# hyperplane-lab/RGBManip

Measured on AMD Instinct MI355X. Metric: adapose_poses_per_sec_batch256, higher is better.
Workload: dtype bf16

## Files before the change

### include/rgbm.h

```cpp
#ifndef RGBM_H_
#define RGBM_H_
#include <stddef.h>
#include <stdint.h>

#ifdef __cplusplus
extern "C" {
#endif

#define RGBM_VERSION 100
#define RGBM_F32 0
#define RGBM_BF16 1
#define RGBM_F16 2
#define RGBM_BF16X3 3

int rgbm_version(void);
const char* rgbm_last_error(void);

typedef struct rgbm_weight_desc {
  const char* name;
  const float* data;
  int ndim;
  const int64_t* shape;
} rgbm_weight_desc;

typedef struct rgbm_adapose rgbm_adapose_t;

typedef struct rgbm_adapose_out {
  float *view1_nocs, *view2_nocs;
  float *view1_depth, *view2_depth;
  float *view1_r, *view2_r;
  float *view1_t, *view2_t;
  float *view1_s, *view2_s;
} rgbm_adapose_out;

int rgbm_adapose_create(rgbm_adapose_t** h, int device, const rgbm_weight_desc* w, int n_w, int dtype, int norm_mode);
int rgbm_adapose_destroy(rgbm_adapose_t* h);
int rgbm_adapose_set_chunk(rgbm_adapose_t* h, int max_chunk_views);
int rgbm_adapose_set_option(rgbm_adapose_t* h, const char* key, int value);
int rgbm_adapose_workspace_bytes(rgbm_adapose_t* h, int B, size_t* bytes);
int rgbm_adapose_set_dropout(rgbm_adapose_t* h, float p, uint64_t seed);
int rgbm_adapose_dropout_masks(rgbm_adapose_t* h, int B, float* out_dev);
int rgbm_adapose_set_dropout_masks(rgbm_adapose_t* h, int B, const float* masks_dev);
int rgbm_adapose_forward(rgbm_adapose_t* h, int B, const float* img1, const float* img2, const int32_t* choose1,
                         const int32_t* choose2, const float* P1, const float* P2, const float* depths, void* workspace,
                         size_t workspace_bytes, const rgbm_adapose_out* out, void* stream);

int rgbm_adapose_postprocess(int B, int P, int img_size, const float* nocs1, const float* depth1, const float* r1,
                             const int32_t* choose1, const double* Kcrop, const double* E1, double* bbox_world, double* ts,
                             int32_t* valid, void* stream);
int rgbm_adapose_postprocess_scratch_bytes(int B, size_t* bytes);
int rgbm_adapose_postprocess_ws(int B, int P, int img_size, const float* nocs1, const float* depth1, const float* r1,
                                const int32_t* choose1, const double* Kcrop, const double* E1, double* bbox_world, double* ts,
                                int32_t* valid, void* scratch, size_t scratch_bytes, void* stream);

int rgbm_adapose_postprocess_ransac(int B, int P, int img_size, uint32_t seed, const float* nocs1, const float* depth1,
                                    const int32_t* choose1, const double* Kcrop, const double* E1, double* bbox_world, double* srt,
                                    int32_t* valid, void* stream);
int rgbm_adapose_postprocess_pnp(int B, int P, uint32_t seed, const float* nocs1, const float* pts2d1, const float* nocs2,
                                 const float* pts2d2, const double* K, const double* E1, const double* E2, double* bbox_out,
                                 double* srt_out, int32_t* info_out, int32_t* valid_out, void* stream);

int rgbm_prepare_inputs(const float* rgb_dev, const uint8_t* mask_dev, const double* K_dev, int N, int H, int W, int S, int P,
                        uint32_t seed, float* img_out, int32_t* choose_out, float* pts2d_out, double* Kcrop_out,
                        int32_t* window_out, int32_t* valid_out, uint8_t* scratch, void* stream);

int rgbm_prepare_inputs_indexed(const float* rgb_dev, const uint8_t* mask_dev, const double* K_dev, const int32_t* frame_map_dev,
                                int N, int H, int W, int S, int P, uint32_t seed, float* img_out, int32_t* choose_out,
                                float* pts2d_out, double* Kcrop_out, int32_t* window_out, int32_t* valid_out, uint8_t* scratch,
                                void* stream);
int rgbm_prepare_inputs_ex(const float* rgb_dev, const uint8_t* mask_dev, const double* K_dev, const int32_t* frame_map_dev,
                           int frame0, int N, int H, int W, int S, int P, uint32_t seed, float* img_out, int32_t* choose_out,
                           float* pts2d_out, double* Kcrop_out, int32_t* window_out, int32_t* valid_out, uint8_t* scratch,
                           void* stream);

int rgbm_projection(const double* Kcrop_dev, const double* E_dev, float* P_dev, int N, void* stream);
int rgbm_mask_extent(const uint8_t* mask_dev, int N, int H, int W, int32_t* ext_out, int32_t* count_out, void* stream);

int rgbm_lookat_quat(const double* dir_dev, int N, int batch_zero, double* quat_dev, void* stream);
int rgbm_control_action_to_pose(const float* action_dev, int lda, const double* pose_mid, const double* pose_min,
                                const double* pose_max, int N, double* pose_dev, void* stream);
typedef struct rgbm_control_reward_args {
  const float* action;
  const double* cam_pose;
  const double* target;
  const float* move_success;
  const double* bbox;
  const double* avail;
  const double* gt_bbox;
  const double* pred_bbox;
  const double* pose_cur;
  const double* pose_prev;
  const double* robot_pose;
  const double* success;
  double* reward;
  double* terms;
  double coef[14];
  double proper_pos[3];
  double precision2;
  int N, T, lda, pots, first;
  int pad_;
} rgbm_control_reward_args;
int rgbm_control_reward(const rgbm_control_reward_args* args, void* stream);
int rgbm_control_grasp_frame(const double* est_dev, int N, double* center_dev, double* direction_dev, void* stream);

typedef struct rgbm_synth_scene {
  const double* cam_pose;
  const double* robot_pose;
  const double* box;
  double fx, fy, cx, cy;
  int N, H, W, env0;
} rgbm_synth_scene;
int rgbm_synth_camera(const rgbm_synth_scene* scene, double* K_dev, double* E_dev, double* rays_dev, void* stream);
int rgbm_synth_render(const rgbm_synth_scene* scene, const double* rays_dev, float* color_dev, uint8_t* mask_dev, void* stream);

int rgbm_gae(int T, int N, const float* rewards, const uint8_t* dones, const float* values, const float* last_values,
             float gamma, float lam, float* returns, float* adv, double* sums, void* stream);
int rgbm_adv_normalise(int64_t n_local, float* adv, const double* sums, double count_total, void* stream);

typedef struct rgbm_policy_layout {
  int dims[5];
  int log_std;
  int w[2][4];
  int b[2][4];
  int total;
} rgbm_policy_layout;
int rgbm_policy_forward(const float* params, const rgbm_policy_layout* L, int n, int mode, const float* obs, const float* noise,
                        float* actions, float* logp, float* value, float* mu, void* stream);
int rgbm_ppo_partial_floats(const rgbm_policy_layout* L, int n, size_t* count);
int rgbm_ppo_minibatch_fwd_bwd(const float* params, const rgbm_policy_layout* L, int n, const float* obs, const float* actions,
                               const float* old_logp, const float* adv, const float* returns, const float* old_values,
                               const float* old_mu, const float* old_log_std, float clip, float vcoef, float ecoef,
                               float* partial_scratch, float* grads_flat, void* stream);
int rgbm_ppo_clip_adam(float* params, const float* grads_flat, float* exp_avg, float* exp_avg_sq, void* opt_state,
                       const rgbm_policy_layout* L, float inv_world, float max_norm, float desired_kl, float lr_min,
                       float lr_max, int adaptive, void* stream);

int rgbm_conv_nd(int dtype, const void* in_dev, int N, int D, int H, int W, int Cin, int Cin_pad, const float* w_host,
                 int Cout, int Cout_pad, int KD, int KH, int KW, int stride_d, int stride_hw, int pad_d, int pad_hw,
                 int dil_hw, int transposed, const float* bias_host, const float* bn_scale_host, const float* bn_shift_host,
                 const void* res_dev, int res_mode, int act, float slope, void* out_dev, void* stream);
int rgbm_bn_per_sample_scratch_bytes(int V, size_t* bytes);
int rgbm_bn_per_sample(int dtype, void* y_dev, const void* res_dev, const float* gamma_dev, const float* beta_dev, void* scratch_dev,
                       int V, int64_t nvox, int C, int relu, void* stream);
int rgbm_conv3d_tile(int layer, int dtype, const void* in_dev, int N, int D, int H, int W, const float* w_host,
                     const float* bn_scale_host, const float* bn_shift_host, const void* res_dev, void* out_dev, void* stream);
int rgbm_upsample_conv3x3(int dtype, const void* in_dev, int V, int h, int w, int Cin, const float* w_host, int Cout,
                          const float* bias_host, int act, float slope, void* z_scratch_dev, void* out_dev, void* stream);
int rgbm_upsample_conv3x3_final(int dtype, const void* in_dev, int V, int h, int w, const float* w3_host, const float* b3_host,
                                float slope, const float* wf_host, const float* bf_host, void* out_dev, int out_f32, void* stream);
int rgbm_stem(int dtype, const float* img1_dev, const float* img2_dev, const float* w_host, void* out_dev, int B, int S, void* stream);
int rgbm_maxpool3x3s2(int dtype, const void* in_dev, void* out_dev, int V, int H, int W, int C, void* stream);
int rgbm_resize_bilinear_ac(int dtype, const void* in_dev, void* out_dev, int V, int Hs, int Ws, int C, int Ho, int Wo,
                            void* stream);
int rgbm_adaptive_avgpool(int dtype, const void* in_dev, void* out_dev, int V, int H, int W, int C, int S, void* stream);
int rgbm_build_volume(int dtype, const void* feat_dev, const float* P_views_dev, const float* depths_dev, float* homog_scratch,
                      void* vol_dev, int V, int B, int D, int H, int W, void* stream);
int rgbm_conv0_sweep(const void* feat_dev, const float* P_views_dev, const float* depths_dev, float* homog_scratch,
                     const float* w_host, const float* bn_scale_host, const float* bn_shift_host, void* out_dev,
                     int V, int B, int D, int H, int W, void* stream);
int rgbm_conv0_sweep_dt(int dtype, const void* feat_dev, const float* P_views_dev, const float* depths_dev, float* homog_scratch,
                        const float* w_host, const float* bn_scale_host, const float* bn_shift_host, void* out_dev,
                        int V, int B, int D, int H, int W, void* stream);
int rgbm_conv0_sweep_f16feat(const void* feat_f16_dev, const float* P_views_dev, const float* depths_dev, float* homog_scratch,
                             const float* w_host, const float* bn_scale_host, const float* bn_shift_host, void* out_bf16_dev,
                             int V, int B, int D, int H, int W, void* stream);
int rgbm_adapose_forward_ex(rgbm_adapose_t* h, int B, const float* img1, const float* img2, const int32_t* choose1,
                            const int32_t* choose2, const float* P1, const float* P2, const float* depths, void* workspace,
                            size_t workspace_bytes, const rgbm_adapose_out* out, int stop_after, void* stream);
int rgbm_adapose_forward_graph(rgbm_adapose_t* h, int B, const float* img1, const float* img2, const int32_t* choose1,
                               const int32_t* choose2, const float* P1, const float* P2, const float* depths, void* workspace,
                               size_t workspace_bytes, const rgbm_adapose_out* out, void* stream, int32_t* n_nodes, int32_t* captured);
int rgbm_adapose_graph_clear(rgbm_adapose_t* h);
int rgbm_adapose_fetch(rgbm_adapose_t* h, int B, void* workspace, const char* name, float* out_dev, size_t capacity,
                       size_t* n_elems, void* stream);

#define RGBM_PROF_ROWS 42
int rgbm_debug_flags(int flags);
int rgbm_set_tuning(const char* key, long long value);
int rgbm_microbench_mfma_scratch_floats(int* n);
int rgbm_microbench_mfma(float* scratch, int iters, int random_operands, double* flops, void* stream);
int rgbm_microbench_copy(const void* src, void* dst, size_t bytes, void* stream);
int rgbm_prof_rows(void);
int rgbm_prof_start(void);
int rgbm_prof_stop(double* stats);
int rgbm_prof_select(int row);

#ifdef __cplusplus
}
#endif
#endif
```

### rgbmanip_amd/_lib.py

```python
from __future__ import annotations

import ctypes as C
import os

_HERE = os.path.dirname(os.path.abspath(__file__))
LIB_PATH = os.environ.get("RGBM_HIP_LIB") or os.path.join(_HERE, "librgbm_hip.so")

F32, BF16, F16, BF16X3 = 0, 1, 2, 3
ACT_NONE, ACT_RELU, ACT_PRELU, ACT_TANH = 0, 1, 2, 3
RES_NONE, RES_PRE_ACT, RES_POST_ACT = 0, 1, 2


PROF_ROWS = 42
PROF_KERNELS = [
    ("conv_igemm_glds_kernel<float, 16, 256>", "fp32"), ("conv_igemm_glds_kernel<float, 32, 256>", "fp32"),
    ("conv_igemm_glds_kernel<float, 64, 256>", "fp32"), ("conv_igemm_glds_kernel<float, 128, 128>", "fp32"),
    ("conv_igemm_glds_kernel<unsigned short, 16, 256>", "bf16"), ("conv_igemm_glds_kernel<unsigned short, 32, 256>", "bf16"),
    ("conv_igemm_glds_kernel<unsigned short, 64, 256>", "bf16"), ("conv_igemm_glds_kernel<unsigned short, 128, 128>", "bf16"),
    ("conv3d_tile_kernel<float, ...> (conv1..conv11)", "fp32"), ("conv3d_tile_kernel<unsigned short, ...> (conv1..conv11)", "bf16"),
    ("conv3d_tile_kernel<float, 32, 16, 4, 8, 8, 1, false, true> (conv0 + fused plane sweep)", "fp32"),
    ("conv3d_tile_kernel<unsigned short, 32, 16, 4, 8, 8, 1, false, true> (conv0 + fused plane sweep)", "bf16"),
    ("conv_igemm_ws_kernel<float, ...>", "fp32"), ("conv_igemm_ws_kernel<unsigned short, false, false> (128 channels x 256 pixels)", "bf16"),
    ("conv0_sweep_persistent_kernel<unsigned short> (conv0 + fused plane sweep of bf16 nets; sweep_f16 = 0 / fp16 nets: conv0_sweep_kernel)", "bf16"), ("conv_igemm_ws64_kernel", "bf16"),
    ("conv3d_tile_kernel<unsigned short, 32, 16, 6, 8, 8, 1, false, false> (conv0 on a materialised volume)", "bf16"),
    ("conv3d_tile_kernel<unsigned short, 8, 16, 2, 8, 8, 2, false, false> (conv1)", "bf16"),
    ("conv3d_tile_kernel<unsigned short, 16, 16, 4, 8, 8, 1, false, false> (conv2)", "bf16"),
    ("conv3d_tile_kernel<unsigned short, 16, 32, 2, 8, 8, 2, false, false> (conv3)", "bf16"),
    ("conv3d_tile_kernel<unsigned short, 32, 32, 2, 8, 8, 1, false, false> (conv4)", "bf16"),
    ("conv3d_tile_kernel<unsigned short, 32, 64, 1, 8, 8, 2, false, false> (conv5)", "bf16"),
    ("conv3d_tile_kernel<unsigned short, 64, 64, 1, 8, 8, 1, false, false> (conv6)", "bf16"),
    ("conv3d_tile_kernel<unsigned short, 64, 32, 1, 8, 8, 1, true, false> (conv7)", "bf16"),
    ("conv3d_tile_kernel<unsigned short, 32, 16, 2, 8, 8, 1, true, false> (conv9)", "bf16"),
    ("conv3d_tile_kernel<unsigned short, 16, 16, 4, 8, 8, 1, true, false> (conv11)", "bf16"),
] + [("conv_igemm_glds_kernel<bx3_t, ...> (all channel tiles)", "bf16x3"), ("conv3d_tile_kernel<bx3_t, ...> (conv1..conv11)", "bf16x3"),
     ("conv0 + fused plane sweep <bx3_t>", "bf16x3"), ("conv_igemm_ws_kernel<rgbm::bx3_t, false, false> (128 channels x 256 pixels)", "bf16x3"),
     ("unused (conv_igemm_w256_kernel of rounds 2-5)", "bf16"),
     ("conv_igemm_m32_kernel<unsigned short, 256, 256> (256 channels x 256 pixels, 32x32x16 MFMAs; gemm_kernel = 0: conv_igemm_ws_kernel<unsigned short, true, false>, 256 x 128)", "bf16"),
     ("unused (row-halo ws tile of rounds 2-5)", "bf16"),
     ("conv_igemm_m32_kernel<rgbm::bx3_t, 256, 256> (256 channels x 256 pixels, 32x32x16 MFMAs; gemm_kernel = 0: conv_igemm_ws_kernel<rgbm::bx3_t, true, false>, 256 x 128)", "bf16x3"),
     ("conv_igemm_ws_kernel<rgbm::bx3_t, false, false, true> (64 channels x 256 pixels, four multiply waves)", "bf16x3"),
     ("conv_igemm_ws_kernel<unsigned short, false, false, true> (64 channels x 256 pixels, four multiply waves)", "bf16"),
     ("conv_igemm_ws_kernel<float, false, false, true> (64 channels x 256 pixels, four multiply waves)", "fp32"),
     ("upconv_combine_kernel<16-bit> (PSPUpsample tap combination)", "bf16"), ("upconv_combine_kernel<4-byte> (PSPUpsample tap combination)", "bf16x3"),
     ("upconv_final_kernel (up_3 + final in one kernel; either storage width)", "bf16"),
     ("conv_igemm_m32_kernel<unsigned short, 128, 64 / 128 / 256> (128-pixel tiles: tail and small-batch launches of the 256-channel GEMM)", "bf16"),
     ("conv_igemm_m32_kernel<rgbm::bx3_t, 128, 64 / 128 / 256> (128-pixel tiles: tail and small-batch launches of the 256-channel GEMM)", "bf16x3")]
assert len(PROF_KERNELS) == PROF_ROWS


class RgbmError(RuntimeError):
    pass


class WeightDesc(C.Structure):
    _fields_ = [("name", C.c_char_p), ("data", C.c_void_p), ("ndim", C.c_int), ("shape", C.POINTER(C.c_int64))]


class PolicyLayout(C.Structure):
    _fields_ = [("dims", C.c_int * 5), ("log_std", C.c_int), ("w", (C.c_int * 4) * 2), ("b", (C.c_int * 4) * 2), ("total", C.c_int)]


class AdaposeOut(C.Structure):
    _fields_ = [(n, C.c_void_p) for n in ("view1_nocs", "view2_nocs", "view1_depth", "view2_depth", "view1_r", "view2_r",
                                           "view1_t", "view2_t", "view1_s", "view2_s")]


class ControlRewardArgs(C.Structure):
    _fields_ = [(n, C.c_void_p) for n in ("action", "cam_pose", "target", "move_success", "bbox", "avail", "gt_bbox", "pred_bbox",
                                           "pose_cur", "pose_prev", "robot_pose", "success", "reward", "terms")] + [
        ("coef", C.c_double * 14), ("proper_pos", C.c_double * 3), ("precision2", C.c_double),
        ("N", C.c_int), ("T", C.c_int), ("lda", C.c_int), ("pots", C.c_int), ("first", C.c_int), ("pad_", C.c_int)]


class SynthScene(C.Structure):
    _fields_ = [("cam_pose", C.c_void_p), ("robot_pose", C.c_void_p), ("box", C.c_void_p),
                ("fx", C.c_double), ("fy", C.c_double), ("cx", C.c_double), ("cy", C.c_double),
                ("N", C.c_int), ("H", C.c_int), ("W", C.c_int), ("env0", C.c_int)]


_vp, _i, _f, _d, _sz, _i64 = C.c_void_p, C.c_int, C.c_float, C.c_double, C.c_size_t, C.c_int64

SIGNATURES = {
    "rgbm_version": (_i, []),
    "rgbm_last_error": (C.c_char_p, []),
    "rgbm_adapose_create": (_i, [C.POINTER(_vp), _i, C.POINTER(WeightDesc), _i, _i, _i]),
    "rgbm_adapose_destroy": (_i, [_vp]),
    "rgbm_adapose_set_chunk": (_i, [_vp, _i]),
    "rgbm_adapose_set_option": (_i, [_vp, C.c_char_p, _i]),
    "rgbm_adapose_workspace_bytes": (_i, [_vp, _i, C.POINTER(_sz)]),
    "rgbm_adapose_set_dropout": (_i, [_vp, _f, C.c_uint64]),
    "rgbm_adapose_dropout_masks": (_i, [_vp, _i, _vp]),
    "rgbm_adapose_set_dropout_masks": (_i, [_vp, _i, _vp]),
    "rgbm_adapose_forward": (_i, [_vp, _i, _vp, _vp, _vp, _vp, _vp, _vp, _vp, _vp, _sz, C.POINTER(AdaposeOut), _vp]),
    "rgbm_adapose_forward_ex": (_i, [_vp, _i, _vp, _vp, _vp, _vp, _vp, _vp, _vp, _vp, _sz, C.POINTER(AdaposeOut), _i, _vp]),
    "rgbm_adapose_forward_graph": (_i, [_vp, _i, _vp, _vp, _vp, _vp, _vp, _vp, _vp, _vp, _sz, C.POINTER(AdaposeOut), _vp, C.POINTER(C.c_int32),
                                        C.POINTER(C.c_int32)]),
    "rgbm_adapose_graph_clear": (_i, [_vp]),
    "rgbm_adapose_fetch": (_i, [_vp, _i, _vp, C.c_char_p, _vp, _sz, C.POINTER(_sz), _vp]),
    "rgbm_adapose_postprocess": (_i, [_i, _i, _i, _vp, _vp, _vp, _vp, _vp, _vp, _vp, _vp, _vp, _vp]),
    "rgbm_adapose_postprocess_scratch_bytes": (_i, [_i, C.POINTER(_sz)]),
    "rgbm_adapose_postprocess_ws": (_i, [_i, _i, _i, _vp, _vp, _vp, _vp, _vp, _vp, _vp, _vp, _vp, _vp, _sz, _vp]),
    "rgbm_adapose_postprocess_ransac": (_i, [_i, _i, _i, C.c_uint32, _vp, _vp, _vp, _vp, _vp, _vp, _vp, _vp, _vp]),
    "rgbm_adapose_postprocess_pnp": (_i, [_i, _i, C.c_uint32, _vp, _vp, _vp, _vp, _vp, _vp, _vp, _vp, _vp, _vp, _vp, _vp]),
    "rgbm_gae": (_i, [_i, _i, _vp, _vp, _vp, _vp, _f, _f, _vp, _vp, _vp, _vp]),
    "rgbm_adv_normalise": (_i, [_i64, _vp, _vp, _d, _vp]),
    "rgbm_policy_forward": (_i, [_vp, _vp, _i, _i, _vp, _vp, _vp, _vp, _vp, _vp, _vp]),
    "rgbm_ppo_partial_floats": (_i, [_vp, _i, C.POINTER(_sz)]),
    "rgbm_ppo_minibatch_fwd_bwd": (_i, [_vp, _vp, _i, _vp, _vp, _vp, _vp, _vp, _vp, _vp, _vp, _f, _f, _f, _vp, _vp, _vp]),
    "rgbm_ppo_clip_adam": (_i, [_vp, _vp, _vp, _vp, _vp, _vp, _f, _f, _f, _f, _f, _i, _vp]),
    "rgbm_conv_nd": (_i, [_i, _vp, _i, _i, _i, _i, _i, _i, _vp, _i, _i, _i, _i, _i, _i, _i, _i, _i, _i, _i, _vp, _vp, _vp,
                          _vp, _i, _i, _f, _vp, _vp]),
    "rgbm_bn_per_sample_scratch_bytes": (_i, [_i, C.POINTER(_sz)]),
    "rgbm_bn_per_sample": (_i, [_i, _vp, _vp, _vp, _vp, _vp, _i, _i64, _i, _i, _vp]),
    "rgbm_conv3d_tile": (_i, [_i, _i, _vp, _i, _i, _i, _i, _vp, _vp, _vp, _vp, _vp, _vp]),
    "rgbm_upsample_conv3x3": (_i, [_i, _vp, _i, _i, _i, _i, _vp, _i, _vp, _i, _f, _vp, _vp, _vp]),
    "rgbm_upsample_conv3x3_final": (_i, [_i, _vp, _i, _i, _i, _vp, _vp, _f, _vp, _vp, _vp, _i, _vp]),
    "rgbm_stem": (_i, [_i, _vp, _vp, _vp, _vp, _i, _i, _vp]),
    "rgbm_maxpool3x3s2": (_i, [_i, _vp, _vp, _i, _i, _i, _i, _vp]),
    "rgbm_resize_bilinear_ac": (_i, [_i, _vp, _vp, _i, _i, _i, _i, _i, _i, _vp]),
    "rgbm_adaptive_avgpool": (_i, [_i, _vp, _vp, _i, _i, _i, _i, _i, _vp]),
    "rgbm_build_volume": (_i, [_i, _vp, _vp, _vp, _vp, _vp, _i, _i, _i, _i, _i, _vp]),
    "rgbm_conv0_sweep": (_i, [_vp, _vp, _vp, _vp, _vp, _vp, _vp, _vp, _i, _i, _i, _i, _i, _vp]),
    "rgbm_conv0_sweep_dt": (_i, [_i, _vp, _vp, _vp, _vp, _vp, _vp, _vp, _vp, _i, _i, _i, _i, _i, _vp]),
    "rgbm_conv0_sweep_f16feat": (_i, [_vp, _vp, _vp, _vp, _vp, _vp, _vp, _vp, _i, _i, _i, _i, _i, _vp]),
    "rgbm_prepare_inputs": (_i, [_vp, _vp, _vp, _i, _i, _i, _i, _i, C.c_uint32, _vp, _vp, _vp, _vp, _vp, _vp, _vp, _vp]),
    "rgbm_prepare_inputs_indexed": (_i, [_vp, _vp, _vp, _vp, _i, _i, _i, _i, _i, C.c_uint32, _vp, _vp, _vp, _vp, _vp, _vp, _vp, _vp]),
    "rgbm_prepare_inputs_ex": (_i, [_vp, _vp, _vp, _vp, _i, _i, _i, _i, _i, _i, C.c_uint32, _vp, _vp, _vp, _vp, _vp, _vp, _vp, _vp]),
    "rgbm_projection": (_i, [_vp, _vp, _vp, _i, _vp]),
    "rgbm_mask_extent": (_i, [_vp, _i, _i, _i, _vp, _vp, _vp]),
    "rgbm_lookat_quat": (_i, [_vp, _i, _i, _vp, _vp]),
    "rgbm_control_action_to_pose": (_i, [_vp, _i, C.POINTER(C.c_double), C.POINTER(C.c_double), C.POINTER(C.c_double), _i, _vp, _vp]),
    "rgbm_control_reward": (_i, [C.POINTER(ControlRewardArgs), _vp]),
    "rgbm_control_grasp_frame": (_i, [_vp, _i, _vp, _vp, _vp]),
    "rgbm_synth_camera": (_i, [C.POINTER(SynthScene), _vp, _vp, _vp, _vp]),
    "rgbm_synth_render": (_i, [C.POINTER(SynthScene), _vp, _vp, _vp, _vp]),
    "rgbm_debug_flags": (_i, [_i]),
    "rgbm_set_tuning": (_i, [C.c_char_p, _i64]),
    "rgbm_prof_rows": (_i, []),
    "rgbm_microbench_mfma_scratch_floats": (_i, [C.POINTER(C.c_int)]),
    "rgbm_microbench_mfma": (_i, [_vp, _i, _i, C.POINTER(C.c_double), _vp]),
    "rgbm_microbench_copy": (_i, [_vp, _vp, C.c_size_t, _vp]),
    "rgbm_prof_start": (_i, []),
    "rgbm_prof_select": (_i, [_i]),
    "rgbm_prof_stop": (_i, [C.POINTER(C.c_double)]),
}

_lib = None


def load():
    global _lib
    if _lib is not None:
        return _lib
    if not os.path.exists(LIB_PATH):
        raise RgbmError(f"{LIB_PATH} not found: build it with rgbmanip_amd/csrc/build.sh "
                        f"(or `python -c 'import __graft_entry__ as g; g.build()'`). There is no CPU fallback.")
    lib = C.CDLL(LIB_PATH)
    for name, (res, args) in SIGNATURES.items():
        fn = getattr(lib, name)
        fn.restype = res
        fn.argtypes = args
    if lib.rgbm_prof_rows() != PROF_ROWS:
        raise RgbmError(f"{LIB_PATH}: rgbm_prof_rows() = {lib.rgbm_prof_rows()}, this binding expects {PROF_ROWS} (stale build?)")
    _lib = lib
    return lib


def check(rc: int, what: str = ""):
    if rc != 0:
        msg = load().rgbm_last_error()
        raise RgbmError(f"{what} failed (code {rc}): {msg.decode() if msg else ''}")


def stream_ptr(stream=None):
    import torch
    s = stream if stream is not None else torch.cuda.current_stream()
    return C.c_void_p(s.cuda_stream)


def ptr(t):
    return C.c_void_p(t.data_ptr()) if t is not None else C.c_void_p(0)
```

### rgbmanip_amd/csrc/adapose.cpp

```cpp
#include "adapose.h"

#include <math.h>
#include <string.h>

namespace rgbm {

static const int kLayerPlanes[4] = {64, 128, 256, 512};
static const int kLayerBlocks[4] = {3, 4, 6, 3};
static const int kLayerStride[4] = {1, 2, 1, 1};
static const int kLayerDil[4] = {1, 1, 2, 4};
static const int kPspBins[4] = {1, 2, 3, 6};
static const int kPspSmallViews = 32;


static const HostTensor* find(const StateDict& sd, const std::string& name) {
  auto it = sd.find(name);
  return it == sd.end() ? nullptr : &it->second;
}

#define GET(var, name)                                               \
  const HostTensor* var = find(sd, name);                            \
  RGBM_REQUIRE(var != nullptr, std::string("missing weight ") + (name))

static int init_conv2d(ConvLayer& L, int dtype, const StateDict& sd, const std::string& wname, const char* bname, int Cin,
                       int Cout, int k, int stride, int pad, int dil, int act, float slope, int Cin_pad) {
  GET(w, wname);
  RGBM_REQUIRE(w->numel() == (long long)Cout * Cin * k * k, "weight shape " + wname);
  const float* b = nullptr;
  if (bname) { GET(bt, std::string(bname)); b = bt->data; }
  ConvGeom g;
  g.Cin = Cin; g.Cout = Cout; g.KH = g.KW = k; g.sh = g.sw = stride; g.ph = g.pw = pad; g.dilh = g.dilw = dil;
  g.act = act; g.slope = slope;
  return L.init(dtype, g, w->data, b, nullptr, nullptr, Cin_pad, Cout);
}

static int bn_fold(const StateDict& sd, const std::string& p, int C, std::vector<float>& scale, std::vector<float>& shift) {
  GET(gm, p + "weight"); GET(bt, p + "bias"); GET(mu, p + "running_mean"); GET(var, p + "running_var");
  RGBM_REQUIRE(gm->numel() == C && bt->numel() == C && mu->numel() == C && var->numel() == C, "bn shape " + p);
  scale.resize(C); shift.resize(C);
  for (int i = 0; i < C; ++i) {
    const float inv = 1.0f / sqrtf(var->data[i] + 1e-5f);
    scale[i] = gm->data[i] * inv;
    shift[i] = bt->data[i] - mu->data[i] * scale[i];
  }
  return 0;
}

static int init_conv3d_bn(ConvLayer& L, int dtype, const StateDict& sd, const std::string& p, int Cin, int Cout, int stride,
                          bool transposed) {
  GET(w, p + "conv.weight");
  RGBM_REQUIRE(w->numel() == (long long)Cout * Cin * 27, "weight shape " + p);
  std::vector<float> scale, shift;
  if (int rc = bn_fold(sd, p + "bn.", Cout, scale, shift)) return rc;
  ConvGeom g;
  g.Cin = Cin; g.Cout = Cout; g.KD = g.KH = g.KW = 3; g.sd = g.sh = g.sw = stride; g.pd = g.ph = g.pw = 1;
  g.transposed = transposed; g.act = ACT_RELU;
  return L.init(dtype, g, w->data, nullptr, scale.data(), shift.data(), Cin, Cout);
}

static int init_linear(ConvLayer& L, const StateDict& sd, const std::string& p, int Cin, int Cout, int act, int Cin_pad,
                       int Cout_pad, const float* w_override = nullptr, int ldtype = F32) {
  GET(w, p + ".weight"); GET(b, p + ".bias");
  ConvGeom g;
  g.Cin = Cin; g.Cout = Cout; g.act = act;
  return L.init(ldtype, g, w_override ? w_override : w->data, b->data, nullptr, nullptr, Cin_pad, Cout_pad);
}

int AdaPose::create(const StateDict& sd, int dtype_, int norm_mode_) {
  dtype = dtype_;
  norm_mode = norm_mode_;
  const int E = dtype_chunk(dtype);
  img_cpad = E;
  const std::string fe = "img_extractor.feats.";
  if (int rc = init_conv2d(conv1, dtype, sd, fe + "conv1.weight", nullptr, 3, 64, 7, 2, 3, 1, ACT_RELU, 0.f, img_cpad)) return rc;
  if (dtype != F32) {
    GET(w1, fe + "conv1.weight");
    RGBM_REQUIRE(w1->numel() == 64 * 3 * 7 * 7, "conv1 shape");
    std::vector<float> pk;
    stem_pack(w1->data, pk);
    if (int rc = upload_packed(pk, dtype, &stem_w)) return rc;
    stem = 1;
  }
  int inpl = 64, nb = 0;
  for (int li = 0; li < 4; ++li) {
    for (int b = 0; b < kLayerBlocks[li]; ++b) {
      Block& blk = blocks[nb++];
      const int planes = kLayerPlanes[li];
      const int cin = b == 0 ? inpl : planes;
      const int stride = b == 0 ? kLayerStride[li] : 1;
      const int dil = b == 0 ? 1 : kLayerDil[li];
      const std::string p = fe + "layer" + std::to_string(li + 1) + "." + std::to_string(b) + ".";
      if (int rc = init_conv2d(blk.c1, dtype, sd, p + "conv1.weight", nullptr, cin, planes, 3, stride, dil, dil, ACT_RELU, 0.f, cin)) return rc;
      if (int rc = init_conv2d(blk.c2, dtype, sd, p + "conv2.weight", nullptr, planes, planes, 3, 1, dil, dil, ACT_RELU, 0.f, planes)) return rc;
      blk.has_ds = find(sd, p + "downsample.0.weight") != nullptr;
      if (blk.has_ds)
        if (int rc = init_conv2d(blk.ds, dtype, sd, p + "downsample.0.weight", nullptr, cin, planes, 1, stride, 0, 1, ACT_NONE, 0.f, cin)) return rc;
      blk.stride = stride; blk.planes = planes;
    }
    inpl = kLayerPlanes[li];
  }
  n_blocks = nb;
  for (int i = 0; i < 4; ++i)
    if (int rc = init_conv2d(psp[i], dtype, sd, "img_extractor.psp.stages." + std::to_string(i) + ".1.weight", nullptr, 512, 128, 1, 1, 0, 1, ACT_RELU, 0.f, 512)) return rc;
  struct { ConvLayer* L; const char* nm; int cin, cout; } ups[3] = {{&up1, "up_1", 1024, 256}, {&up2, "up_2", 256, 64}, {&up3, "up_3", 64, 64}};
  for (auto& u : ups) {
    const std::string p = std::string("img_extractor.") + u.nm + ".conv.";
    GET(sl, p + "1.weight");
    const std::string bn = p + "0.bias";
    if (int rc = init_conv2d(*u.L, dtype, sd, p + "0.weight", bn.c_str(), u.cin, u.cout, 3, 1, 1, 1, ACT_PRELU, sl->data[0], u.cin)) return rc;
    UpConvLayer* uc = u.L == &up1 ? &up1c : u.L == &up2 ? &up2c : nullptr;
    if (uc) {
      GET(w, p + "0.weight"); GET(b, bn);
      if (int rc = uc->init(dtype, u.cin, u.cout, w->data, b->data, ACT_PRELU, sl->data[0])) return rc;
    }
  }
  if (int rc = init_conv2d(fin, dtype, sd, "img_extractor.final.weight", "img_extractor.final.bias", 64, 32, 1, 1, 0, 1, ACT_NONE, 0.f, 64)) return rc;
  if (dtype != F32) {
    GET(w3, "img_extractor.up_3.conv.0.weight"); GET(b3, "img_extractor.up_3.conv.0.bias"); GET(s3, "img_extractor.up_3.conv.1.weight");
    GET(wf, "img_extractor.final.weight"); GET(bfin, "img_extractor.final.bias");
    if (int rc = tail.init(dtype, w3->data, b3->data, s3->data[0], wf->data, bfin->data)) return rc;
  }


  const std::string cr = "cost_regularization.";
  const int crc[8] = {32, 8, 16, 16, 32, 32, 64, 64};
  const int crs[7] = {1, 2, 1, 2, 1, 2, 1};
  for (int i = 0; i < 7; ++i)
    if (int rc = init_conv3d_bn(c3d[i], dtype, sd, cr + "conv" + std::to_string(i) + ".", crc[i], crc[i + 1], crs[i], false)) return rc;
  if (int rc = init_conv3d_bn(dc[0], dtype, sd, cr + "conv7.", 64, 32, 2, true)) return rc;
  if (int rc = init_conv3d_bn(dc[1], dtype, sd, cr + "conv9.", 32, 16, 2, true)) return rc;
  if (int rc = init_conv3d_bn(dc[2], dtype, sd, cr + "conv11.", 16, 8, 2, true)) return rc;
  if (norm_mode == 1) {
    const char* nm[10] = {"conv0", "conv1", "conv2", "conv3", "conv4", "conv5", "conv6", "conv7", "conv9", "conv11"};
    for (int i = 0; i < 10; ++i) {
      const bool tr = i >= 7;
      const int cin = tr ? (i == 7 ? 64 : i == 8 ? 32 : 16) : crc[i], cout = tr ? cin / 2 : crc[i + 1];
      const std::string p = cr + nm[i] + ".";
      GET(w, p + "conv.weight"); GET(gm, p + "bn.weight"); GET(bt, p + "bn.bias");
      RGBM_REQUIRE(w->numel() == (long long)cout * cin * 27 && gm->numel() == cout && bt->numel() == cout, "weight shape " + p);
      ConvGeom g;
      g.Cin = cin; g.Cout = cout; g.KD = g.KH = g.KW = 3; g.sd = g.sh = g.sw = tr ? 2 : crs[i]; g.pd = g.ph = g.pw = 1;
      g.transposed = tr; g.act = ACT_NONE;
      ConvLayer& L = tr ? dc_raw[i - 7] : c3d_raw[i];
      if (int rc = L.init(dtype, g, w->data, nullptr, nullptr, nullptr, cin, cout)) return rc;
      if (upload_f32(gm->data, cout, &bn_gamma[i])) return -2;
      if (upload_f32(bt->data, cout, &bn_beta[i])) return -2;
    }
  }
  {
    const char* nm[10] = {"conv0", "conv1", "conv2", "conv3", "conv4", "conv5", "conv6", "conv7", "conv9", "conv11"};
    const int cin[10] = {32, 8, 16, 16, 32, 32, 64, 64, 32, 16};
    const int cout[10] = {8, 16, 16, 32, 32, 64, 64, 32, 16, 8};
    for (int i = 0; i < 10; ++i) {
      const std::string p = cr + nm[i] + ".";
      GET(w, p + "conv.weight");
      std::vector<float> scale, shift, packed;
      if (int rc = bn_fold(sd, p + "bn.", cout[i], scale, shift)) return rc;
      const int coutp = cout[i] < 16 ? 16 : cout[i];
      conv3d_tile_pack(w->data, scale.data(), cin[i], cout[i], coutp, i >= 7, dtype, packed);
      t3d[i].Cin = cin[i]; t3d[i].Cout = cout[i];
      if (upload_packed(packed, dtype, &t3d[i].w)) return -2;
      std::vector<float> bpad(coutp, 0.f);
      for (int o = 0; o < cout[i]; ++o) bpad[o] = shift[o];
      if (upload_f32(bpad.data(), bpad.size(), &t3d[i].bias)) return -2;
      if (i == 9 && dtype != F32) {
        std::vector<float> pt;
        prob_sparse_pack(w->data, scale.data(), pt);
        if (dtype == BF16X3) { if (conv0_sweep_x3_upload(pt, &w11_taps)) return -2; }
        else if (upload_packed(pt, dtype, &w11_taps)) return -2;
      }
      if (i == 9 && dtype == BF16X3) {
        std::vector<float> p16;
        conv3d_tile_pack(w->data, scale.data(), cin[i], cout[i], coutp, true, BF16, p16);
        if (conv0_sweep_x3_upload(p16, &w11_x3)) return -2;
      }
      if (i == 0 && dtype != F32) {
        conv0_sweep_pack(w->data, scale.data(), packed);
        if (dtype == BF16X3) { if (conv0_sweep_x3_upload(packed, &sweep_w)) return -2; }
        else if (upload_packed(packed, dtype, &sweep_w)) return -2;
        if (dtype == BF16 && weights_fit_f16(packed) && upload_packed(packed, F16, &sweep_w_f16)) return -2;
      }
    }
  }
  {
    GET(w, cr + "prob.weight");
    RGBM_REQUIRE(w->numel() == 8 * 27, "prob weight shape");
    std::vector<float> wp(27 * 8);
    for (int c = 0; c < 8; ++c) for (int t = 0; t < 27; ++t) wp[t * 8 + c] = w->data[c * 27 + t];
    if (upload_f32(wp.data(), wp.size(), &wprob)) return -2;
  }
  if (int rc = init_linear(inst, sd, "instance_color.0", 32, 64, ACT_RELU, 32, 64)) return rc;
  if (int rc = init_linear(nh[0], sd, "nocs_head.0", 64, 128, ACT_RELU, 64, 128)) return rc;
  if (int rc = init_linear(nh[1], sd, "nocs_head.2", 128, 64, ACT_RELU, 128, 64)) return rc;
  if (int rc = init_linear(nh[2], sd, "nocs_head.4", 64, 3, ACT_TANH, 64, 4)) return rc;
  if (int rc = init_linear(npm[0], sd, "nocs_pts_mlp.0", 3, 32, ACT_RELU, 4, 32)) return rc;
  if (int rc = init_linear(npm[1], sd, "nocs_pts_mlp.2", 32, 64, ACT_RELU, 32, 64)) return rc;
  {
    static const char* const names[6] = {"instance_color.0", "nocs_head.0", "nocs_head.2", "nocs_head.4", "nocs_pts_mlp.0", "nocs_pts_mlp.2"};
    static const int cin[6] = {32, 64, 128, 64, 3, 32}, cout[6] = {64, 128, 64, 3, 32, 64};
    const float* w[6]; const float* b[6];
    for (int l = 0; l < 6; ++l) {
      GET(wt, std::string(names[l]) + ".weight"); GET(bt, std::string(names[l]) + ".bias");
      RGBM_REQUIRE(wt->numel() == (long long)cin[l] * cout[l] && bt->numel() == cout[l], std::string("point MLP shape ") + names[l]);
      w[l] = wt->data; b[l] = bt->data;
    }
    std::vector<float> table((size_t)point_mlp_table_floats());
    point_mlp_pack(w, b, table.data());
    if (upload_f32(table.data(), table.size(), &pmlp_table)) return -2;
  }
  if (int rc = init_linear(pm1[0], sd, "pose_mlp1.0", 96, 128, ACT_RELU, 96, 128, nullptr, pose_dtype())) return rc;
  if (int rc = init_linear(pm1[1], sd, "pose_mlp1.2", 128, 128, ACT_RELU, 128, 128, nullptr, pose_dtype())) return rc;
  {
    GET(w, "pose_mlp2.0.weight"); GET(b, "pose_mlp2.0.bias");
    RGBM_REQUIRE(w->numel() == 256 * 256, "pose_mlp2.0 shape");
    std::vector<float> wl(256 * 128);
    for (int o = 0; o < 256; ++o) for (int i = 0; i < 128; ++i) wl[o * 128 + i] = w->data[o * 256 + i];
    if (int rc = init_linear(pm2[0], sd, "pose_mlp2.0", 128, 256, ACT_RELU, 128, 256, wl.data(), pose_dtype())) return rc;
    if (upload_f32(w->data, 256 * 256, &pm2_0_wfull)) return -2;
    if (upload_f32(b->data, 256, &pm2_0_bias)) return -2;
  }
  if (int rc = init_linear(pm2[1], sd, "pose_mlp2.2", 256, 256, ACT_RELU, 256, 256, nullptr, pose_dtype())) return rc;
  const char* hn[3] = {"rotation_estimator", "translation_estimator", "size_estimator"};
  const int hout[3] = {6, 3, 3};
  for (int h = 0; h < 3; ++h) {
    const int dims[4] = {256, 256, 128, hout[h]};
    for (int l = 0; l < 3; ++l) {
      GET(w, std::string(hn[h]) + "." + std::to_string(2 * l) + ".weight");
      GET(b, std::string(hn[h]) + "." + std::to_string(2 * l) + ".bias");
      RGBM_REQUIRE(w->numel() == (long long)dims[l] * dims[l + 1], "head weight shape");
      if (upload_f32(w->data, w->numel(), &head_w[h][l])) return -2;
      if (upload_f32(b->data, b->numel(), &head_b[h][l])) return -2;
    }
  }
  return 0;
}

void AdaPose::destroy() {
  conv1.destroy();
  if (stem_w) (void)hipFree(stem_w);
  stem_w = nullptr;
  for (int i = 0; i < n_blocks; ++i) { blocks[i].c1.destroy(); blocks[i].c2.destroy(); if (blocks[i].has_ds) blocks[i].ds.destroy(); }
  for (auto& l : psp) l.destroy();
  up1.destroy(); up2.destroy(); up3.destroy(); fin.destroy();
  up1c.destroy(); up2c.destroy(); tail.destroy();
  if (drop_masks) (void)hipFree(drop_masks);
  if (drop_state) (void)hipFree(drop_state);
  drop_masks = nullptr; drop_state = nullptr; drop_cap_views = 0; drop_p = 0.f; drop_explicit = 0; drop_last_B = 0;
  for (auto& l : c3d) l.destroy();
  for (auto& l : dc) l.destroy();
  for (auto& l : c3d_raw) l.destroy();
  for (auto& l : dc_raw) l.destroy();
  for (int i = 0; i < 10; ++i) { if (bn_gamma[i]) (void)hipFree(bn_gamma[i]); if (bn_beta[i]) (void)hipFree(bn_beta[i]); bn_gamma[i] = bn_beta[i] = nullptr; }
  inst.destroy();
  for (auto& l : nh) l.destroy();
  for (auto& l : npm) l.destroy();
  for (auto& l : pm1) l.destroy();
  for (auto& l : pm2) l.destroy();
  for (auto& t : t3d) { if (t.w) (void)hipFree(t.w); if (t.bias) (void)hipFree(t.bias); t.w = nullptr; t.bias = nullptr; }
  if (sweep_w) (void)hipFree(sweep_w);
  sweep_w = nullptr;
  if (sweep_w_f16) (void)hipFree(sweep_w_f16);
  sweep_w_f16 = nullptr;
  if (w11_x3) (void)hipFree(w11_x3);
  w11_x3 = nullptr;
  if (w11_taps) (void)hipFree(w11_taps);
  w11_taps = nullptr;
  if (wprob) (void)hipFree(wprob);
  if (pm2_0_wfull) (void)hipFree(pm2_0_wfull);
  if (pmlp_table) { (void)hipFree(pmlp_table); pmlp_table = nullptr; }
  if (pm2_0_bias) (void)hipFree(pm2_0_bias);
  for (int h = 0; h < 3; ++h) for (int l = 0; l < 3; ++l) { if (head_w[h][l]) (void)hipFree(head_w[h][l]); if (head_b[h][l]) (void)hipFree(head_b[h][l]); }
}

bool AdaPose::feat_f32_only() const {
  return dtype == BF16X3 && cost_impl == 3 && sweep_w != nullptr && norm_mode == 0 && !(g_debug_flags & 4096);
}

bool AdaPose::feat_f16() const {
  return dtype == BF16 && sweep_f16 != 0 && cost_impl == 3 && sweep_w_f16 != nullptr && norm_mode == 0 && !(g_debug_flags & 4096) && (upconv & 4) &&
         tail.ready() && tail.f16_ready();
}

bool AdaPose::sparse_active() const {
  const bool b16 = dtype_size(dtype) == 2;
  return sparse_dec != 0 && norm_mode == 0 && cost_impl == 3 && (b16 || (dtype == BF16X3 && w11_x3)) && sparse_tail && sweep_w != nullptr &&
         !(g_debug_flags & 4096);
}

int AdaPose::chunk_views(int V) const {
  const int cap = norm_mode == 1 && max_chunk > 32 ? 32 : max_chunk;
  return V < cap ? V : cap;
}

int AdaPose::plan(int B, Arena& A, Buffers& bf) const {
  const int V = 2 * B, P = n_pts, S = img;
  const size_t es = dtype_size(dtype);
  const size_t VP = (size_t)V * P;
  bf.Pviews = (float*)A.alloc((size_t)V * 16 * 4);
  bf.homog = (float*)A.alloc((size_t)V * 12 * 4);
  bf.choose = (int*)A.alloc(VP * 4);
  bf.masks = (unsigned char*)A.alloc((size_t)V * sparse_mask_bytes_per_view(img));
  bf.sweep_list = (int*)A.alloc((size_t)V * ((img + 11) / 12) * ((img + 15) / 16) * 4);
  bf.sweep_count = (int*)A.alloc((size_t)(V + 64) * 4);
  bf.feat = A.alloc((size_t)V * S * S * 32 * es);
  bf.featf = dtype == BF16X3 ? (float*)A.alloc((size_t)V * S * S * 32 * 4) : nullptr;
  bf.X0 = (float*)A.alloc(VP * 32 * 4);
  bf.X1 = (float*)A.alloc(VP * 64 * 4);
  bf.H128 = (float*)A.alloc(VP * 128 * 4);
  bf.H64 = (float*)A.alloc(VP * 64 * 4);
  bf.nocs4 = (float*)A.alloc(VP * 4 * 4);
  bf.N32 = (float*)A.alloc(VP * 32 * 4);
  bf.PF96 = (float*)A.alloc(VP * 96 * 4);
  bf.PF96h = pose_dtype() == F16 ? A.alloc(VP * 96 * 2) : nullptr;
  bf.prob = (float*)A.alloc(VP * n_depth * 4);
  bf.depth = (float*)A.alloc(VP * 4);
  bf.Q128a = (float*)A.alloc(VP * 128 * 4);
  bf.Q128b = (float*)A.alloc(VP * 128 * 4);
  bf.G256a = (float*)A.alloc(VP * 256 * 4);
  bf.G256b = (float*)A.alloc(VP * 256 * 4);
  bf.glob = (float*)A.alloc((size_t)V * 128 * 4);
  bf.vbias = (float*)A.alloc((size_t)V * 256 * 4);
  bf.pf2 = (float*)A.alloc((size_t)V * 256 * 4);
  bf.h1 = (float*)A.alloc((size_t)V * 256 * 4);
  bf.h2 = (float*)A.alloc((size_t)V * 128 * 4);
  bf.r6 = (float*)A.alloc((size_t)V * 8 * 4);
  bf.R = (float*)A.alloc((size_t)V * 9 * 4);
  bf.tv = (float*)A.alloc((size_t)V * 4 * 4);
  bf.sv = (float*)A.alloc((size_t)V * 4 * 4);
  const size_t m0 = A.mark();
  bf.imgpad = A.alloc((size_t)V * S * S * img_cpad * es);
  bf.c1 = A.alloc((size_t)V * (S / 2) * (S / 2) * 64 * es);
  const size_t lbuf = (size_t)V * ((size_t)(S / 4) * (S / 4) * 64 > (size_t)(S / 8) * (S / 8) * 512 ? (size_t)(S / 4) * (S / 4) * 64 : (size_t)(S / 8) * (S / 8) * 512) * es;
  for (int i = 0; i < 4; ++i) bf.lb[i] = A.alloc(lbuf);
  for (int i = 0; i < 4; ++i) {
    bf.pooled[i] = A.alloc((size_t)V * kPspBins[i] * kPspBins[i] * 512 * es);
    bf.stage[i] = A.alloc((size_t)V * kPspBins[i] * kPspBins[i] * 128 * es);
  }
  const size_t f8 = (size_t)(S / 8) * (S / 8), f4 = (size_t)(S / 4) * (S / 4), f2 = (size_t)(S / 2) * (S / 2), f1 = (size_t)S * S;
  bf.cat = A.alloc((size_t)V * f8 * 1024 * es);
  bf.ups = A.alloc((size_t)V * f4 * 1024 * es);
  bf.u1 = A.alloc((size_t)V * f4 * 256 * es);
  bf.u2 = A.alloc((size_t)V * f2 * 64 * es);
  bf.u3 = A.alloc((size_t)V * f1 * 64 * es);
  A.release(m0);
  const int Vc = chunk_views(V);
  const int D = n_depth;
  const size_t vox = (size_t)D * S * S;
  bf.vol = (cost_impl >= 2 && norm_mode == 0) ? nullptr : A.alloc((size_t)Vc * vox * 32 * es);
  bf.bn_scratch = norm_mode == 1 ? A.alloc(bn_scratch_bytes(Vc)) : nullptr;
  bf.c[0] = A.alloc((size_t)Vc * vox * 8 * es);
  bf.c[1] = A.alloc((size_t)Vc * (vox / 8) * 16 * es);
  bf.c[2] = A.alloc((size_t)Vc * (vox / 8) * 16 * es);
  bf.c[3] = A.alloc((size_t)Vc * (vox / 64) * 32 * es);
  bf.c[4] = A.alloc((size_t)Vc * (vox / 64) * 32 * es);
  bf.c[5] = A.alloc((size_t)Vc * (vox / 512) * 64 * es);
  bf.c[6] = A.alloc((size_t)Vc * (vox / 512) * 64 * es);
  bf.u7 = A.alloc((size_t)Vc * (vox / 64) * 32 * es);
  bf.u9 = A.alloc((size_t)Vc * (vox / 8) * 16 * es);
  bf.u11 = A.alloc((size_t)Vc * vox * 8 * es);
  A.release(m0);
  return 0;
}

size_t AdaPose::workspace_bytes(int B) const {
  Arena A(nullptr, 0);
  Buffers bf;
  plan(B, A, bf);
  return A.peak + 256;
}

int AdaPose::pspnet(const Buffers& bf, int V, const float* img1, const float* img2, hipStream_t s, const float* drop) const {
  const int S = img;
  int H = S / 2, W = S / 2;
  if (stem && stem_w) {
    if (int rc = launch_stem(dtype, img1, img2, stem_w, bf.lb[0], V / 2, V, S, s)) return rc;
  } else {
    const size_t es = dtype_size(dtype);
    const int B = V / 2;
    if (int rc = launch_nchw_to_nhwc_pad(dtype, img1, bf.imgpad, B, 3, S, S, img_cpad, s)) return rc;
    if (int rc = launch_nchw_to_nhwc_pad(dtype, img2, (char*)bf.imgpad + (size_t)B * S * S * img_cpad * es, B, 3, S, S, img_cpad, s)) return rc;
    if (int rc = conv1.run(bf.imgpad, bf.c1, V, 1, S, S, 64, nullptr, 0, nullptr, 0, s)) return rc;
    if (int rc = launch_maxpool3x3s2(dtype, bf.c1, bf.lb[0], V, H, W, 64, s)) return rc;
  }
  H = S / 4; W = S / 4;
  int xi = 0;
  for (int i = 0; i < n_blocks; ++i) {
    const Block& blk = blocks[i];
    void* x = bf.lb[xi];
    void* t = bf.lb[(xi + 1) & 3];
    void* r = bf.lb[(xi + 2) & 3];
    void* y = bf.lb[(xi + 3) & 3];
    int Do, Ho, Wo;
    blk.c1.out_dims(1, H, W, Do, Ho, Wo);
    if (int rc = blk.c1.run(x, t, V, 1, H, W, blk.planes, nullptr, 0, nullptr, 0, s)) return rc;
    const void* res = x;
    if (blk.has_ds) {
      if (int rc = blk.ds.run(x, r, V, 1, H, W, blk.planes, nullptr, 0, nullptr, 0, s)) return rc;
      res = r;
    }
    if (int rc = blk.c2.run(t, y, V, 1, Ho, Wo, blk.planes, res, RES_PRE_ACT, nullptr, 0, s)) return rc;
    H = Ho; W = Wo;
    xi = (xi + 3) & 3;
  }
  const void* f = bf.lb[xi];
  last_f_index = xi;
  RGBM_REQUIRE(H == S / 8 && W == S / 8, "feature stride");
  if (g_debug_flags & 1024) {
    if (int rc = launch_copy_channels(dtype, f, bf.cat, (long long)V * H * W, 512, 1024, 0, s)) return rc;
    {
      void* outs[4] = {bf.pooled[0], bf.pooled[1], bf.pooled[2], bf.pooled[3]};
      if (int rc = launch_adaptive_avgpool_multi(dtype, f, outs, kPspBins, 4, V, H, W, 512, s)) return rc;
    }
    for (int i = 0; i < 4; ++i) {
      const int Sb = kPspBins[i];
      if (int rc = psp[i].run(bf.pooled[i], bf.stage[i], V, 1, Sb, Sb, 128, nullptr, 0, nullptr, 0, s)) return rc;
      if (int rc = launch_resize_bilinear_ac(dtype, bf.stage[i], bf.cat, V, Sb, Sb, 128, H, W, 1024, 512 + 128 * i, s)) return rc;
    }
  } else {
    bool small = V <= kPspSmallViews;
    for (int i = 0; i < 4; ++i)
      small = small && psp[i].packs.size() == 1 && psp[i].packs[0].Kpad == 512 && psp[i].Cout_pad == 128 && psp[i].bias == nullptr;
    if (small) {
      const void* w[4] = {psp[0].packs[0].w, psp[1].packs[0].w, psp[2].packs[0].w, psp[3].packs[0].w};
      void* outs[4] = {bf.stage[0], bf.stage[1], bf.stage[2], bf.stage[3]};
      if (int rc = launch_psp_pool_conv(dtype, f, 512, w, outs, kPspBins, V, H, W, psp[0].g.act, psp[0].g.slope, s)) return rc;
    } else {
      void* outs[4] = {bf.pooled[0], bf.pooled[1], bf.pooled[2], bf.pooled[3]};
      if (int rc = launch_adaptive_avgpool_multi(dtype, f, outs, kPspBins, 4, V, H, W, 512, s)) return rc;
      for (int i = 0; i < 4; ++i)
        if (int rc = psp[i].run(bf.pooled[i], bf.stage[i], V, 1, kPspBins[i], kPspBins[i], 128, nullptr, 0, nullptr, 0, s)) return rc;
    }
    const void* stages[4] = {bf.stage[0], bf.stage[1], bf.stage[2], bf.stage[3]};
    if (int rc = launch_psp_resize_cat(dtype, f, stages, kPspBins, bf.cat, V, H, W, s)) return rc;
  }
  RGBM_REQUIRE(drop == nullptr || (upconv & 3) == 3, "dropout needs option upconv bits 0 and 1 (up_1 / up_2 through the tap combination)");
  if (upconv & 1) {
    if (int rc = up1c.run(bf.cat, bf.ups, bf.u1, V, H, W, 256, s, drop)) return rc;
  } else {
    if (int rc = launch_resize_bilinear_ac(dtype, bf.cat, bf.ups, V, H, W, 1024, 2 * H, 2 * W, 1024, 0, s)) return rc;
    if (int rc = up1.run(bf.ups, bf.u1, V, 1, 2 * H, 2 * W, 256, nullptr, 0, nullptr, 0, s)) return rc;
  }
  if (upconv & 2) {
    if (int rc = up2c.run(bf.u1, bf.ups, bf.u2, V, 2 * H, 2 * W, 64, s, drop ? drop + 256 : nullptr)) return rc;
  } else {
    if (int rc = launch_resize_bilinear_ac(dtype, bf.u1, bf.ups, V, 2 * H, 2 * W, 256, 4 * H, 4 * W, 256, 0, s)) return rc;
    if (int rc = up2.run(bf.ups, bf.u2, V, 1, 4 * H, 4 * W, 64, nullptr, 0, nullptr, 0, s)) return rc;
  }
  fin.out_plain_f32 = feat_f32_only();
  if ((upconv & 4) && tail.ready())
    return tail.run(bf.u2, fin.out_plain_f32 ? (void*)bf.featf : bf.feat, fin.out_plain_f32 ? 1 : feat_f16() ? 2 : 0, V, 4 * H, 4 * W, s);
  if (int rc = launch_resize_bilinear_ac(dtype, bf.u2, bf.ups, V, 4 * H, 4 * W, 64, 8 * H, 8 * W, 64, 0, s)) return rc;
  fin.out_plain_f32 = feat_f32_only();
  if (int rc = up3.run_then_1x1(fin, bf.ups, bf.u3, 64, fin.out_plain_f32 ? (void*)bf.featf : bf.feat, 32, V, 1, 8 * H, 8 * W, fuse_final != 0, nullptr, s)) return rc;
  return 0;
}

int AdaPose::cost_volume(const Buffers& bf, int V, int B, const float* depths, hipStream_t s) const {
  const int S = img, D = n_depth, P = n_pts;
  const int Vh = view2_heads ? V : B;
  const int Vc0 = chunk_views(V);
  const bool b16 = dtype_size(dtype) == 2;
  bool sweep_sparse = false;
  auto tile = [&](int layer, const void* in, void* out, const void* res, int Vc, int Di, int Hi, int Wi, int Do, int Ho,
                  int Wo, bool transposed, int v0, const unsigned char* tmask = nullptr) -> int {
    const int li = layer == 10 ? 0 : layer;
    Conv3dTileDesc d;
    memset(&d, 0, sizeof(d));
    d.in = in; d.wgt = t3d[li].w; d.out = out; d.bias = t3d[li].bias; d.res = res;
    d.N = Vc; d.Di = Di; d.Hi = Hi; d.Wi = Wi; d.Do = Do; d.Ho = Ho; d.Wo = Wo;
    d.Dq = transposed ? Di : Do; d.Hq = transposed ? Hi : Ho; d.Wq = transposed ? Wi : Wo;
    d.Cout = t3d[li].Cout; d.relu = 1;
    d.feat = bf.feat; d.homog = bf.homog; d.depths = depths; d.v0 = v0; d.V = V; d.B = B;
    d.out_classmajor = layer == 9 ? 1 : 0;
    d.tile_mask = tmask;
    d.tile_mask_stride = sparse_mask_bytes_per_view(S);
    if (layer == 10 && sweep_sparse) { d.tile_list = bf.sweep_list; d.tile_count = bf.sweep_count; }
    d.prof_variant = dtype == BF16X3 ? (layer == 10 ? 28 : 27) : layer == 10 ? 10 + (dtype != F32 ? 1 : 0) : (dtype != F32 ? 16 + layer : 8);
    d.algo_flops = 2.0 * Vc * (double)(transposed ? Di * Hi * Wi : Do * Ho * Wo) * t3d[li].Cout * 27.0 * t3d[li].Cin;
    d.algo_bytes = ((layer == 10 ? (double)Vc * Hi * Wi * t3d[li].Cin : (double)Vc * Di * Hi * Wi * t3d[li].Cin) +
                    (double)Vc * Do * Ho * Wo * t3d[li].Cout * (res ? 2 : 1)) * (double)dtype_size(dtype);
    if (layer == 10 && cost_impl == 3 && b16 && sweep_w && !(g_debug_flags & 4096)) {
      d.wgt = sweep_w;
      if (feat_f16()) { d.wgt = sweep_w_f16; d.feat_f16 = 1; }
      return launch_conv0_sweep(d, dtype, s);
    }
    if (layer == 10 && cost_impl == 3 && dtype == BF16X3 && sweep_w && !(g_debug_flags & 4096)) {
      d.wgt = sweep_w;
      d.feat = bf.featf;
      return launch_conv0_sweep_x3(d, s);
    }
    return launch_conv3d_tile(layer, dtype, d, s);
  };
  const bool sparse_ok = sparse_active();
  for (int v0 = 0; norm_mode == 0 && cost_impl >= 1 && v0 < Vh; v0 += Vc0) {
    const int Vc = Vh - v0 < Vc0 ? Vh - v0 : Vc0;
    const unsigned char* mk[10] = {nullptr, nullptr, nullptr, nullptr, nullptr, nullptr, nullptr, nullptr, nullptr, nullptr};
    sweep_sparse = false;
    if (sparse_ok) {
      int td, th, tw;
      for (int L : {1, 2, 3, 4, 5, 7, 8}) RGBM_REQUIRE(!conv3d_tile_dims(L, dtype, &td, &th, &tw) && th == 8 && tw == 8, "sparse cost regularisation: 8 x 8 tiles expected");
      if (int rc = launch_sparse_masks(bf.choose, v0, Vc, P, S, bf.masks, bf.sweep_list, bf.sweep_count, s)) return rc;
      for (int L : {7, 8}) mk[L] = bf.masks + sparse_mask_offset(S, L);
      if (sparse_dec >= 2) {
        for (int L : {1, 2, 3, 4, 5}) mk[L] = bf.masks + sparse_mask_offset(S, L);
        sweep_sparse = true;
      }
    }
    if (cost_impl == 1) {
      if (int rc = launch_build_volume(dtype, bf.feat, bf.homog, depths, bf.vol, v0, Vc, V, B, D, S, S, s)) return rc;
      if (int rc = tile(0, bf.vol, bf.c[0], nullptr, Vc, D, S, S, D, S, S, false, v0)) return rc;
    } else {
      if (int rc = tile(10, nullptr, bf.c[0], nullptr, Vc, D, S, S, D, S, S, false, v0)) return rc;
    }
    if (int rc = tile(1, bf.c[0], bf.c[1], nullptr, Vc, D, S, S, D / 2, S / 2, S / 2, false, v0, mk[1])) return rc;
    if (int rc = tile(2, bf.c[1], bf.c[2], nullptr, Vc, D / 2, S / 2, S / 2, D / 2, S / 2, S / 2, false, v0, mk[2])) return rc;
    if (int rc = tile(3, bf.c[2], bf.c[3], nullptr, Vc, D / 2, S / 2, S / 2, D / 4, S / 4, S / 4, false, v0, mk[3])) return rc;
    if (int rc = tile(4, bf.c[3], bf.c[4], nullptr, Vc, D / 4, S / 4, S / 4, D / 4, S / 4, S / 4, false, v0, mk[4])) return rc;
    if (int rc = tile(5, bf.c[4], bf.c[5], nullptr, Vc, D / 4, S / 4, S / 4, D / 8, S / 8, S / 8, false, v0, mk[5])) return rc;
    if (cost_impl == 3 && (b16 || dtype == BF16X3) && igemm_conv6) {
      if (int rc = c3d[6].run(bf.c[5], bf.c[6], Vc, D / 8, S / 8, S / 8, 64, nullptr, RES_NONE, nullptr, 0, s)) return rc;
    } else {
      if (int rc = tile(6, bf.c[5], bf.c[6], nullptr, Vc, D / 8, S / 8, S / 8, D / 8, S / 8, S / 8, false, v0)) return rc;
    }
    if (int rc = tile(7, bf.c[6], bf.u7, bf.c[4], Vc, D / 8, S / 8, S / 8, D / 4, S / 4, S / 4, true, v0, mk[7])) return rc;
    if (int rc = tile(8, bf.u7, bf.u9, bf.c[2], Vc, D / 4, S / 4, S / 4, D / 2, S / 2, S / 2, true, v0, mk[8])) return rc;
    if (cost_impl == 3 && (b16 || (dtype == BF16X3 && w11_x3)) && sparse_tail) {
      if (int rc = launch_prob_sparse(bf.u9, bf.c[0], dtype == BF16X3 ? w11_x3 : t3d[9].w, t3d[9].bias, wprob, bf.choose, depths, bf.prob,
                                      bf.depth, v0, Vc, B, P, D, S, S, dtype, s, w11_taps)) return rc;
      continue;
    }
    if (int rc = tile(9, bf.u9, bf.u11, bf.c[0], Vc, D / 2, S / 2, S / 2, D, S, S, true, v0)) return rc;
    if (int rc = launch_prob_softmax_depth(dtype, bf.u11, wprob, bf.choose, depths, bf.prob, bf.depth, v0, Vc, B, P, D, S, S, 1, s)) return rc;
  }
  for (int v0 = 0; norm_mode == 1 && v0 < Vh; v0 += Vc0) {
    const int Vc = Vh - v0 < Vc0 ? Vh - v0 : Vc0;
    if (int rc = launch_build_volume(dtype, bf.feat, bf.homog, depths, bf.vol, v0, Vc, V, B, D, S, S, s)) return rc;
    auto layer = [&](int i, const void* in, void* out, const void* res, int Di, int Hi, int Wi, int C) -> int {
      const ConvLayer& L = i >= 7 ? dc_raw[i - 7] : c3d_raw[i];
      int Do, Ho, Wo;
      L.out_dims(Di, Hi, Wi, Do, Ho, Wo);
      if (int rc = L.run(in, out, Vc, Di, Hi, Wi, C, nullptr, RES_NONE, nullptr, 0, s)) return rc;
      return launch_bn_per_sample(dtype, out, res, bn_gamma[i], bn_beta[i], bf.bn_scratch, Vc, (long long)Do * Ho * Wo, C, 1, s);
    };
    if (int rc = layer(0, bf.vol, bf.c[0], nullptr, D, S, S, 8)) return rc;
    if (int rc = layer(1, bf.c[0], bf.c[1], nullptr, D, S, S, 16)) return rc;
    if (int rc = layer(2, bf.c[1], bf.c[2], nullptr, D / 2, S / 2, S / 2, 16)) return rc;
    if (int rc = layer(3, bf.c[2], bf.c[3], nullptr, D / 2, S / 2, S / 2, 32)) return rc;
    if (int rc = layer(4, bf.c[3], bf.c[4], nullptr, D / 4, S / 4, S / 4, 32)) return rc;
    if (int rc = layer(5, bf.c[4], bf.c[5], nullptr, D / 4, S / 4, S / 4, 64)) return rc;
    if (int rc = layer(6, bf.c[5], bf.c[6], nullptr, D / 8, S / 8, S / 8, 64)) return rc;
    if (int rc = layer(7, bf.c[6], bf.u7, bf.c[4], D / 8, S / 8, S / 8, 32)) return rc;
    if (int rc = layer(8, bf.u7, bf.u9, bf.c[2], D / 4, S / 4, S / 4, 16)) return rc;
    if (int rc = layer(9, bf.u9, bf.u11, bf.c[0], D / 2, S / 2, S / 2, 8)) return rc;
    if (int rc = launch_prob_softmax_depth(dtype, bf.u11, wprob, bf.choose, depths, bf.prob, bf.depth, v0, Vc, B, P, D, S, S, 0, s)) return rc;
  }
  if (norm_mode == 1) return 0;
  for (int v0 = 0; cost_impl == 0 && v0 < Vh; v0 += Vc0) {
    const int Vc = Vh - v0 < Vc0 ? Vh - v0 : Vc0;
    if (int rc = launch_build_volume(dtype, bf.feat, bf.homog, depths, bf.vol, v0, Vc, V, B, D, S, S, s)) return rc;
    if (int rc = c3d[0].run(bf.vol, bf.c[0], Vc, D, S, S, 8, nullptr, 0, nullptr, 0, s)) return rc;
    if (int rc = c3d[1].run(bf.c[0], bf.c[1], Vc, D, S, S, 16, nullptr, 0, nullptr, 0, s)) return rc;
    if (int rc = c3d[2].run(bf.c[1], bf.c[2], Vc, D / 2, S / 2, S / 2, 16, nullptr, 0, nullptr, 0, s)) return rc;
    if (int rc = c3d[3].run(bf.c[2], bf.c[3], Vc, D / 2, S / 2, S / 2, 32, nullptr, 0, nullptr, 0, s)) return rc;
    if (int rc = c3d[4].run(bf.c[3], bf.c[4], Vc, D / 4, S / 4, S / 4, 32, nullptr, 0, nullptr, 0, s)) return rc;
    if (int rc = c3d[5].run(bf.c[4], bf.c[5], Vc, D / 4, S / 4, S / 4, 64, nullptr, 0, nullptr, 0, s)) return rc;
    if (int rc = c3d[6].run(bf.c[5], bf.c[6], Vc, D / 8, S / 8, S / 8, 64, nullptr, 0, nullptr, 0, s)) return rc;
    if (int rc = dc[0].run(bf.c[6], bf.u7, Vc, D / 8, S / 8, S / 8, 32, bf.c[4], RES_POST_ACT, nullptr, 0, s)) return rc;
    if (int rc = dc[1].run(bf.u7, bf.u9, Vc, D / 4, S / 4, S / 4, 16, bf.c[2], RES_POST_ACT, nullptr, 0, s)) return rc;
    if (int rc = dc[2].run(bf.u9, bf.u11, Vc, D / 2, S / 2, S / 2, 8, bf.c[0], RES_POST_ACT, nullptr, 0, s)) return rc;
    if (int rc = launch_prob_softmax_depth(dtype, bf.u11, wprob, bf.choose, depths, bf.prob, bf.depth, v0, Vc, B, P, D, S, S, 0, s)) return rc;
  }
  return 0;
}

int AdaPose::forward(int B, const float* img1, const float* img2, const int* choose1, const int* choose2, const float* P1,
                     const float* P2, const float* depths, void* workspace, size_t workspace_size, const Outputs& out,
                     hipStream_t s, int stop_after) const {
  RGBM_REQUIRE(B > 0, "batch");
  RGBM_REQUIRE(((uintptr_t)workspace & 255) == 0, "workspace must be 256-byte aligned");
  RGBM_REQUIRE(n_depth % 8 == 0 && img % 8 == 0, "depth/img must be multiples of 8");
  const size_t need = workspace_bytes(B);
  RGBM_REQUIRE(workspace_size >= need, "workspace too small: need " + std::to_string(need));
  Arena A(workspace, workspace_size);
  Buffers bf;
  plan(B, A, bf);
  const int V = 2 * B, P = n_pts, S = img, D = n_depth;
  const size_t VP = (size_t)V * P;

  if (int rc = launch_stage_in(P1, P2, choose1, choose2, bf.Pviews, bf.choose, B, P, s)) return rc;
  const float* drop = nullptr;
  if (drop_active()) {
    RGBM_REQUIRE(V <= drop_cap_views && drop_masks && (drop_explicit || drop_state), "dropout: mask buffer smaller than the batch");
    RGBM_REQUIRE((upconv & 3) == 3, "dropout needs option upconv bits 0 and 1 (up_1 / up_2 through the tap combination)");
    if (drop_explicit) {
      RGBM_REQUIRE(drop_explicit == B, "dropout: the masks set for the next forward are for batch " + std::to_string(drop_explicit));
      drop_explicit = 0;
    } else {
      if (int rc = launch_dropout_masks(drop_masks, drop_state, B, drop_p, drop_seed, drop_no_advance ? 0 : 1, s)) return rc;
    }
    drop = drop_masks;
    drop_last_B = B;
  }
  if (int rc = pspnet(bf, V, img1, img2, s, drop)) return rc;
  if (int rc = launch_homography(bf.Pviews, bf.homog, V, B, s)) return rc;
  const void* featg = bf.feat;
  int fdt = dtype;
  if (dtype == BF16X3) {
    if (!feat_f32_only())
      if (int rc = launch_bx3_to_f32(bf.feat, bf.featf, (long long)V * S * S * 32, s)) return rc;
    featg = bf.featf; fdt = F32;
  }
  if (feat_f16()) fdt = F16;
  if (stop_after == 1) return 0;

  const int Vh = view2_heads ? V : B;
  if (pmlp_table != nullptr && !(g_debug_flags & 2048) && ((long long)Vh * P) % 64 == 0) {
    PointMlpDesc pd{};
    pd.table = pmlp_table; pd.feat = featg; pd.choose = bf.choose; pd.nocs4 = bf.nocs4; pd.pf = bf.PF96 + 32; pd.ldpf = 96; pd.P = P; pd.HW = S * S;
    pd.N = (long long)Vh * P;
    if (int rc = launch_point_mlp(fdt, pd, s)) return rc;
  } else {
    if (int rc = launch_gather_points(fdt, featg, bf.choose, bf.X0, Vh, P, S * S, 32, s)) return rc;
    if (int rc = inst.run(bf.X0, bf.X1, Vh, 1, 1, P, 64, nullptr, 0, nullptr, 0, s)) return rc;
    if (int rc = nh[0].run(bf.X1, bf.H128, Vh, 1, 1, P, 128, nullptr, 0, nullptr, 0, s)) return rc;
    if (int rc = nh[1].run(bf.H128, bf.H64, Vh, 1, 1, P, 64, nullptr, 0, nullptr, 0, s)) return rc;
    if (int rc = nh[2].run(bf.H64, bf.nocs4, Vh, 1, 1, P, 4, nullptr, 0, nullptr, 0, s)) return rc;
    if (int rc = npm[0].run(bf.nocs4, bf.N32, Vh, 1, 1, P, 32, nullptr, 0, nullptr, 0, s)) return rc;
    if (int rc = npm[1].run(bf.N32, bf.PF96 + 32, Vh, 1, 1, P, 96, nullptr, 0, nullptr, 0, s)) return rc;
  }

  if (int rc = cost_volume(bf, V, B, depths, s)) return rc;
  if (stop_after == 2) return 0;

  if (int rc = launch_fuse_points(fdt, featg, bf.homog, depths, bf.choose, bf.prob, bf.PF96, V, B, P, D, S, S, 96, 0, s, Vh)) return rc;
  const int pdt = pose_dtype();
  const void* pf_in = bf.PF96;
  if (pdt == F16) {
    if (int rc = launch_f32_to_f16(bf.PF96, bf.PF96h, (long long)Vh * P * 96, s)) return rc;
    pf_in = bf.PF96h;
  } else if (pdt == BF16X3) {
    if (int rc = launch_f32_to_bx3(bf.PF96, bf.PF96, (long long)Vh * P * 96, s)) return rc;
  }
  if (int rc = pm1[0].run(pf_in, bf.Q128a, Vh, 1, 1, P, 128, nullptr, 0, nullptr, 0, s)) return rc;
  if (int rc = pm1[1].run(bf.Q128a, bf.Q128b, Vh, 1, 1, P, 128, nullptr, 0, nullptr, 0, s)) return rc;
  if (int rc = launch_mean_points_partial(pdt, bf.Q128b, (float*)bf.Q128a, Vh, P, 128, s)) return rc;
  if (int rc = launch_view_linear_mean((const float*)bf.Q128a, P, bf.glob, pm2_0_wfull, pm2_0_bias, bf.vbias, Vh, 128, 256, 256, 128, 0, s)) return rc;
  if (int rc = pm2[0].run(bf.Q128b, bf.G256a, Vh, 1, 1, P, 256, nullptr, 0, bf.vbias, 256, s)) return rc;
  if (int rc = pm2[1].run(bf.G256a, bf.G256b, Vh, 1, 1, P, 256, nullptr, 0, nullptr, 0, s)) return rc;
  if (int rc = launch_mean_points_partial(pdt, bf.G256b, (float*)bf.G256a, Vh, P, 256, s)) return rc;
  float* hout[3] = {bf.r6, bf.tv, bf.sv};
  const int hdim[3] = {6, 3, 3};
  if (int rc = launch_pose_heads_mean((const float*)bf.G256a, P, bf.pf2, bf.R, head_w, head_b, hout, hdim, Vh, s)) return rc;

  {
    float* const on[2] = {out.nocs1, out.nocs2};
    float* const od[2] = {out.depth1, out.depth2};
    float* const orr[2] = {out.r1, out.r2};
    float* const ot[2] = {out.t1, out.t2};
    float* const os[2] = {out.s1, out.s2};
    if (int rc = launch_stage_out(bf.nocs4, bf.depth, bf.R, bf.tv, bf.sv, on, od, orr, ot, os, B, P, view2_heads, s)) return rc;
  }
  (void)VP;
  return 0;
}

}
```

### rgbmanip_amd/csrc/adapose.h

```cpp
#pragma once
#include "kernels.h"
#include "layers.h"

namespace rgbm {

struct Arena {
  char* base; size_t off; size_t cap; size_t peak;
  explicit Arena(void* b, size_t c) : base((char*)b), off(0), cap(c), peak(0) {}
  void* alloc(size_t bytes) {
    off = align_up(off, 256);
    void* p = base ? base + off : nullptr;
    off += bytes;
    if (off > peak) peak = off;
    return p;
  }
  size_t mark() const { return off; }
  void release(size_t m) { off = m; }
};

struct AdaPose {
  int dtype = F32;
  int pose_dtype() const { return dtype == BF16 ? F16 : (dtype == BF16X3 && pose_x3) ? BF16X3 : F32; }
  int pose_x3 = 1;
  int img = 224, n_pts = 1024, n_depth = 24;
  int img_cpad = 4;
  int max_chunk = 512;

  struct Block { ConvLayer c1, c2, ds; bool has_ds = false; int stride = 1, planes = 0; };
  ConvLayer conv1;
  Block blocks[16];
  int n_blocks = 0;
  ConvLayer psp[4], up1, up2, up3, fin;
  UpConvLayer up1c, up2c;
  int sparse_dec = 2;
  void* stem_w = nullptr;
  int stem = 0;
  UpConvFinal tail;
  int upconv = 7;
  ConvLayer c3d[7], dc[3];
  int norm_mode = 0;
  ConvLayer c3d_raw[7], dc_raw[3];
  float* bn_gamma[10] = {nullptr};
  float* bn_beta[10] = {nullptr};
  struct Tile3d { void* w = nullptr; float* bias = nullptr; int Cin = 0, Cout = 0; };
  Tile3d t3d[10];
  int igemm_conv6 = 1;
  int fuse_final = 1;
  int view2_heads = 1;
  int sparse_tail = 1;
  int sweep_f16 = 1;
  void* w11_taps = nullptr;
  void* sweep_w_f16 = nullptr;
  void* sweep_w = nullptr;
  int cost_impl = 3;
  void* w11_x3 = nullptr;
  float* wprob = nullptr;
  ConvLayer inst, nh[3], npm[2], pm1[2], pm2[2];
  float* pm2_0_wfull = nullptr;
  float* pmlp_table = nullptr;
  float* pm2_0_bias = nullptr;
  float* head_w[3][3] = {{nullptr}};
  float* head_b[3][3] = {{nullptr}};

  float drop_p = 0.f;
  unsigned long long drop_seed = 0;
  float* drop_masks = nullptr;
  unsigned long long* drop_state = nullptr;
  int drop_cap_views = 0;
  mutable int drop_explicit = 0;
  mutable int drop_last_B = 0;
  int drop_no_advance = 0;
  bool drop_active() const { return drop_p > 0.f || drop_explicit > 0; }

  struct Buffers {
    float *Pviews, *homog; int* choose; void* feat;
    unsigned char* masks;
    int *sweep_list, *sweep_count;
    float* featf;
    float *X0, *X1, *H128, *H64, *nocs4, *N32, *PF96, *prob, *depth, *Q128a, *Q128b, *G256a, *G256b;
    void* PF96h;
    float *glob, *vbias, *pf2, *h1, *h2, *r6, *R, *tv, *sv;
    void *imgpad, *c1, *lb[4], *pooled[4], *stage[4], *cat, *ups, *u1, *u2, *u3;
    void *vol, *c[7], *u7, *u9, *u11;
    void* bn_scratch;
  };
  struct Outputs {
    float *nocs1, *nocs2;
    float *depth1, *depth2;
    float *r1, *r2;
    float *t1, *t2, *s1, *s2;
  };

  int create(const StateDict& sd, int dtype, int norm_mode = 0);
  void destroy();
  size_t workspace_bytes(int B) const;
  int forward(int B, const float* img1, const float* img2, const int* choose1, const int* choose2, const float* P1,
              const float* P2, const float* depths, void* workspace, size_t workspace_size, const Outputs& out,
              hipStream_t s, int stop_after = 0) const;
  mutable int last_f_index = 0;

  int plan(int B, Arena& A, Buffers& bf) const;
  int pspnet(const Buffers& bf, int V, const float* img1, const float* img2, hipStream_t s, const float* drop = nullptr) const;
  int cost_volume(const Buffers& bf, int V, int B, const float* depths, hipStream_t s) const;
  int chunk_views(int V) const;
  bool feat_f32_only() const;
  bool feat_f16() const;
  bool sparse_active() const;
};

const char* last_error_cstr();

}
```

### rgbmanip_amd/csrc/capi.cpp

```cpp
#include "../../include/rgbm.h"

#include <string.h>

#include <algorithm>
#include <string>
#include <vector>

#include "adapose.h"
#include "control.h"
#include "prof.h"

using namespace rgbm;

struct ForwardGraph {
  int B = 0;
  const void* in[7] = {nullptr};
  void* ws = nullptr;
  size_t ws_bytes = 0;
  rgbm_adapose_out out;
  int opt_version = 0;
  int tuning_version = 0;
  hipGraph_t graph = nullptr;
  hipGraphExec_t exec = nullptr;
  size_t nodes = 0;
  unsigned long long last_use = 0;
};

struct rgbm_adapose {
  AdaPose net;
  int device;
  int opt_version = 0;
  unsigned long long tick = 0;
  std::vector<ForwardGraph> graphs;
};
static const size_t kMaxGraphs = 8;

static int ensure_dropout_capacity(rgbm_adapose* h, int B) {
  AdaPose& n = h->net;
  if (2 * B <= n.drop_cap_views) return 0;
  const int views = std::max(2 * B, 2 * n.drop_cap_views);
  float* m = nullptr;
  RGBM_CHECK_HIP(hipMalloc(&m, (size_t)views * kDropoutPerView * sizeof(float)));
  if (n.drop_masks) {
    (void)hipDeviceSynchronize();
    (void)hipFree(n.drop_masks);
  }
  n.drop_masks = m;
  n.drop_cap_views = views;
  ++h->opt_version;
  return 0;
}

static void drop_graph(ForwardGraph& g) {
  if (g.exec) (void)hipGraphExecDestroy(g.exec);
  if (g.graph) (void)hipGraphDestroy(g.graph);
  g.exec = nullptr; g.graph = nullptr;
}


extern "C" {

int rgbm_version(void) { return RGBM_VERSION; }
const char* rgbm_last_error(void) { return last_error_cstr(); }

int rgbm_adapose_create(rgbm_adapose_t** h, int device, const rgbm_weight_desc* w, int n_w, int dtype, int norm_mode) {
  RGBM_REQUIRE(h != nullptr && w != nullptr && n_w > 0, "create arguments");
  RGBM_REQUIRE(dtype == RGBM_F32 || dtype == RGBM_BF16 || dtype == RGBM_F16 || dtype == RGBM_BF16X3, "dtype must be 0 (fp32), 1 (bf16), 2 (fp16) or 3 (bf16x3)");
  RGBM_REQUIRE(norm_mode == 0 || norm_mode == 1, "norm_mode: 0 = eval-mode (folded) BatchNorm3d, 1 = per-sample statistics");
  RGBM_CHECK_HIP(hipSetDevice(device));
  StateDict sd;
  for (int i = 0; i < n_w; ++i) {
    std::string name = w[i].name;
    if (name.rfind("module.", 0) == 0) name = name.substr(7);
    HostTensor t;
    t.data = w[i].data;
    for (int d = 0; d < w[i].ndim; ++d) t.shape.push_back(w[i].shape[d]);
    sd[name] = t;
  }
  rgbm_adapose* obj = new rgbm_adapose();
  obj->device = device;
  int rc = obj->net.create(sd, dtype, norm_mode);
  if (rc) { obj->net.destroy(); delete obj; return rc; }
  *h = obj;
  return 0;
}

int rgbm_adapose_destroy(rgbm_adapose_t* h) {
  if (!h) return 0;
  for (auto& g : h->graphs) drop_graph(g);
  h->net.destroy();
  delete h;
  return 0;
}

int rgbm_adapose_set_chunk(rgbm_adapose_t* h, int max_chunk_views) {
  RGBM_REQUIRE(h && max_chunk_views > 0, "set_chunk arguments");
  h->net.max_chunk = max_chunk_views;
  ++h->opt_version;
  return 0;
}

int rgbm_adapose_set_option(rgbm_adapose_t* h, const char* key, int value) {
  RGBM_REQUIRE(h && key, "set_option arguments");
  const std::string k = key;
  if (k == "max_chunk") { RGBM_REQUIRE(value > 0, "max_chunk"); h->net.max_chunk = value; }
  else if (k == "igemm_conv6") { RGBM_REQUIRE(value == 0 || value == 1, "igemm_conv6"); h->net.igemm_conv6 = value; }
  else if (k == "fuse_final") { RGBM_REQUIRE(value == 0 || value == 1, "fuse_final"); h->net.fuse_final = value; }
  else if (k == "sparse_tail") { RGBM_REQUIRE(value == 0 || value == 1, "sparse_tail"); h->net.sparse_tail = value; }
  else if (k == "upconv") { RGBM_REQUIRE(value >= 0 && value <= 7, "upconv"); h->net.upconv = value; }
  else if (k == "sparse_dec") { RGBM_REQUIRE(value >= 0 && value <= 2, "sparse_dec"); h->net.sparse_dec = value; }
  else if (k == "stem") { RGBM_REQUIRE(value == 0 || value == 1, "stem"); h->net.stem = value; }
  else if (k == "view2_heads") { RGBM_REQUIRE(value == 0 || value == 1, "view2_heads"); h->net.view2_heads = value; }
  else if (k == "sweep_f16") { RGBM_REQUIRE(value == 0 || value == 1, "sweep_f16"); h->net.sweep_f16 = value; }
  else if (k == "cost_impl") { RGBM_REQUIRE(value >= 0 && value <= 3, "cost_impl"); h->net.cost_impl = value; }
  else { set_error("unknown option " + k); return -1; }
  ++h->opt_version;
  return 0;
}

int rgbm_adapose_set_dropout(rgbm_adapose_t* h, float p, uint64_t seed) {
  RGBM_REQUIRE(h && (p == 0.f || (p > 0.f && p < 1.f)), "set_dropout: p must be 0 (off) or lie in (0, 1)");
  RGBM_CHECK_HIP(hipSetDevice(h->device));
  if (!h->net.drop_state) RGBM_CHECK_HIP(hipMalloc(&h->net.drop_state, 2 * sizeof(unsigned long long)));
  RGBM_CHECK_HIP(hipDeviceSynchronize());
  RGBM_CHECK_HIP(hipMemset(h->net.drop_state, 0, 2 * sizeof(unsigned long long)));
  RGBM_CHECK_HIP(hipDeviceSynchronize());
  h->net.drop_p = p;
  h->net.drop_seed = (unsigned long long)seed;
  ++h->opt_version;
  return 0;
}

int rgbm_adapose_dropout_masks(rgbm_adapose_t* h, int B, float* out_dev) {
  RGBM_REQUIRE(h && out_dev && B > 0, "dropout_masks arguments");
  RGBM_REQUIRE(h->net.drop_last_B == B && h->net.drop_masks, "dropout_masks: the last forward with dropout had batch " +
               std::to_string(h->net.drop_last_B) + ", not " + std::to_string(B));
  RGBM_CHECK_HIP(hipSetDevice(h->device));
  RGBM_CHECK_HIP(hipDeviceSynchronize());
  RGBM_CHECK_HIP(hipMemcpy(out_dev, h->net.drop_masks, (size_t)2 * B * kDropoutPerView * sizeof(float), hipMemcpyDeviceToDevice));
  return 0;
}

int rgbm_adapose_set_dropout_masks(rgbm_adapose_t* h, int B, const float* masks_dev) {
  RGBM_REQUIRE(h && masks_dev && B > 0, "set_dropout_masks arguments");
  RGBM_CHECK_HIP(hipSetDevice(h->device));
  if (int rc = ensure_dropout_capacity(h, B)) return rc;
  RGBM_CHECK_HIP(hipDeviceSynchronize());
  RGBM_CHECK_HIP(hipMemcpy(h->net.drop_masks, masks_dev, (size_t)2 * B * kDropoutPerView * sizeof(float), hipMemcpyDeviceToDevice));
  h->net.drop_explicit = B;
  return 0;
}

int rgbm_adapose_workspace_bytes(rgbm_adapose_t* h, int B, size_t* bytes) {
  RGBM_REQUIRE(h && bytes && B > 0, "workspace_bytes arguments");
  *bytes = h->net.workspace_bytes(B);
  return 0;
}

static AdaPose::Outputs to_out(const rgbm_adapose_out* o) {
  AdaPose::Outputs r;
  r.nocs1 = o->view1_nocs; r.nocs2 = o->view2_nocs; r.depth1 = o->view1_depth; r.depth2 = o->view2_depth;
  r.r1 = o->view1_r; r.r2 = o->view2_r; r.t1 = o->view1_t; r.t2 = o->view2_t; r.s1 = o->view1_s; r.s2 = o->view2_s;
  return r;
}

int rgbm_adapose_forward_ex(rgbm_adapose_t* h, int B, const float* img1, const float* img2, const int32_t* choose1,
                            const int32_t* choose2, const float* P1, const float* P2, const float* depths, void* workspace,
                            size_t workspace_bytes, const rgbm_adapose_out* out, int stop_after, void* stream) {
  RGBM_REQUIRE(h && img1 && img2 && choose1 && choose2 && P1 && P2 && depths && workspace && out, "forward arguments");
  if (h->net.drop_p > 0.f && B > 0)
    if (int rc = ensure_dropout_capacity(h, B)) return rc;
  return h->net.forward(B, img1, img2, choose1, choose2, P1, P2, depths, workspace, workspace_bytes, to_out(out),
                        (hipStream_t)stream, stop_after);
}

int rgbm_adapose_forward(rgbm_adapose_t* h, int B, const float* img1, const float* img2, const int32_t* choose1,
                         const int32_t* choose2, const float* P1, const float* P2, const float* depths, void* workspace,
                         size_t workspace_bytes, const rgbm_adapose_out* out, void* stream) {
  return rgbm_adapose_forward_ex(h, B, img1, img2, choose1, choose2, P1, P2, depths, workspace, workspace_bytes, out, 0, stream);
}

int rgbm_adapose_graph_clear(rgbm_adapose_t* h) {
  RGBM_REQUIRE(h, "graph_clear arguments");
  for (auto& g : h->graphs) drop_graph(g);
  h->graphs.clear();
  return 0;
}

int rgbm_adapose_forward_graph(rgbm_adapose_t* h, int B, const float* img1, const float* img2, const int32_t* choose1,
                               const int32_t* choose2, const float* P1, const float* P2, const float* depths, void* workspace,
                               size_t workspace_bytes, const rgbm_adapose_out* out, void* stream, int32_t* n_nodes, int32_t* captured) {
  RGBM_REQUIRE(h && img1 && img2 && choose1 && choose2 && P1 && P2 && depths && workspace && out, "forward_graph arguments");
  hipStream_t s = (hipStream_t)stream;
  if (n_nodes) *n_nodes = 0;
  if (captured) *captured = 0;
  if (h->net.drop_p > 0.f && B > 0)
    if (int rc = ensure_dropout_capacity(h, B)) return rc;
  if (prof_enabled() || h->net.drop_explicit) {
    if (captured) *captured = -1;
    return h->net.forward(B, img1, img2, choose1, choose2, P1, P2, depths, workspace, workspace_bytes, to_out(out), s, 0);
  }
  RGBM_REQUIRE(s != nullptr, "forward_graph: stream capture is not allowed on the default (null) stream; pass a created stream");
  const void* in[7] = {img1, img2, choose1, choose2, P1, P2, depths};
  ForwardGraph* hit = nullptr;
  for (size_t i = 0; i < h->graphs.size();) {
    ForwardGraph& g = h->graphs[i];
    if (g.opt_version != h->opt_version || g.tuning_version != g_tuning_version) {
      drop_graph(g);
      h->graphs.erase(h->graphs.begin() + i);
      continue;
    }
    if (g.B == B && !memcmp(g.in, in, sizeof(in)) && g.ws == workspace && g.ws_bytes == workspace_bytes &&
        !memcmp(&g.out, out, sizeof(*out))) hit = &g;
    ++i;
  }
  if (!hit) {
    h->net.drop_no_advance = 1;
    const int rw = h->net.forward(B, img1, img2, choose1, choose2, P1, P2, depths, workspace, workspace_bytes, to_out(out), s, 0);
    h->net.drop_no_advance = 0;
    if (rw) return rw;
    ForwardGraph g;
    g.B = B; memcpy(g.in, in, sizeof(in)); g.ws = workspace; g.ws_bytes = workspace_bytes; g.out = *out;
    g.opt_version = h->opt_version; g.tuning_version = g_tuning_version;
    RGBM_CHECK_HIP(hipStreamBeginCapture(s, hipStreamCaptureModeThreadLocal));
    const int rc = h->net.forward(B, img1, img2, choose1, choose2, P1, P2, depths, workspace, workspace_bytes, to_out(out), s, 0);
    const hipError_t ee = hipStreamEndCapture(s, &g.graph);
    if (rc) { if (g.graph) (void)hipGraphDestroy(g.graph); return rc; }
    if (ee != hipSuccess || !g.graph) { set_error(std::string("hipStreamEndCapture: ") + hipGetErrorString(ee)); return -2; }
    if (hipGraphGetNodes(g.graph, nullptr, &g.nodes) != hipSuccess) g.nodes = 0;
    const hipError_t ei = hipGraphInstantiate(&g.exec, g.graph, nullptr, nullptr, 0);
    if (ei != hipSuccess) { (void)hipGraphDestroy(g.graph); set_error(std::string("hipGraphInstantiate: ") + hipGetErrorString(ei)); return -2; }
    if (h->graphs.size() >= kMaxGraphs) {
      size_t lru = 0;
      for (size_t i = 1; i < h->graphs.size(); ++i) if (h->graphs[i].last_use < h->graphs[lru].last_use) lru = i;
      drop_graph(h->graphs[lru]);
      h->graphs.erase(h->graphs.begin() + lru);
    }
    h->graphs.push_back(g);
    hit = &h->graphs.back();
    if (captured) *captured = 1;
  }
  hit->last_use = ++h->tick;
  if (n_nodes) *n_nodes = (int32_t)hit->nodes;
  RGBM_CHECK_HIP(hipGraphLaunch(hit->exec, s));
  return 0;
}

int rgbm_adapose_fetch(rgbm_adapose_t* h, int B, void* workspace, const char* name, float* out_dev, size_t capacity,
                       size_t* n_elems, void* stream) {
  RGBM_REQUIRE(h && workspace && name && out_dev && n_elems, "fetch arguments");
  const AdaPose& n = h->net;
  Arena A(workspace, 0);
  AdaPose::Buffers bf;
  n.plan(B, A, bf);
  const size_t V = 2 * (size_t)B, S = n.img, P = n.n_pts, D = n.n_depth;
  const size_t Vc = n.chunk_views((int)V);
  const std::string nm = name;
  const void* src = nullptr; size_t cnt = 0; int dt = n.dtype;
  if (nm == "imgpad") { src = bf.imgpad; cnt = V * S * S * n.img_cpad; }
  else if (nm == "conv1") { src = bf.c1; cnt = V * (S / 2) * (S / 2) * 64; }
  else if (nm == "layer4") { src = bf.lb[n.last_f_index]; cnt = V * (S / 8) * (S / 8) * 512; }
  else if (nm == "cat") { src = bf.cat; cnt = V * (S / 8) * (S / 8) * 1024; }
  else if (nm == "u1") { src = bf.u1; cnt = V * (S / 4) * (S / 4) * 256; }
  else if (nm == "u2") { src = bf.u2; cnt = V * (S / 2) * (S / 2) * 64; }
  else if (nm == "u3") { src = bf.u3; cnt = V * S * S * 64; }
  else if (nm == "feat") { src = bf.feat; cnt = V * S * S * 32; if (n.feat_f32_only()) { src = bf.featf; dt = F32; } else if (n.feat_f16()) dt = F16; }
  else if (nm == "vol") { src = bf.vol; cnt = Vc * D * S * S * 32; }
  else if (nm == "c0") { src = bf.c[0]; cnt = Vc * D * S * S * 8; }
  else if (nm == "c2") { src = bf.c[2]; cnt = Vc * (D / 2) * (S / 2) * (S / 2) * 16; }
  else if (nm == "c4") { src = bf.c[4]; cnt = Vc * (D / 4) * (S / 4) * (S / 4) * 32; }
  else if (nm == "c6") { src = bf.c[6]; cnt = Vc * (D / 8) * (S / 8) * (S / 8) * 64; }
  else if (nm == "u7") { src = bf.u7; cnt = Vc * (D / 4) * (S / 4) * (S / 4) * 32; }
  else if (nm == "u9") { src = bf.u9; cnt = Vc * (D / 2) * (S / 2) * (S / 2) * 16; }
  else if (nm == "u11") { src = bf.u11; cnt = Vc * D * S * S * 8; }
  else if (nm == "homog") { src = bf.homog; cnt = V * 12; dt = F32; }
  else if (nm == "prob") { src = bf.prob; cnt = V * P * D; dt = F32; }
  else if (nm == "pf96") { src = bf.PF96; cnt = V * P * 96; dt = n.pose_dtype() == BF16X3 ? BF16X3 : F32; }
  else if (nm == "pf2") { src = bf.pf2; cnt = V * 256; dt = F32; }
  else if (nm == "r6") { src = bf.r6; cnt = V * 6; dt = F32; }
  RGBM_REQUIRE(src != nullptr, "unknown intermediate name: " + nm);
  const bool tap3d = nm == "c0" || nm == "c2" || nm == "c4" || nm == "c6" || nm == "u7" || nm == "u9";
  RGBM_REQUIRE(!(tap3d && n.sparse_active()), "tap '" + nm + "' needs a dense cost regularisation: set option sparse_dec = 0 before the forward "
               "(the default computes it only inside the chosen pixels' dependency cones)");
  *n_elems = cnt;
  RGBM_REQUIRE(cnt <= capacity, "fetch capacity too small");
  return launch_to_f32(dt, src, out_dev, (long long)cnt, (hipStream_t)stream);
}

int rgbm_adapose_postprocess(int B, int P, int img_size, const float* nocs1, const float* depth1, const float* r1,
                             const int32_t* choose1, const double* Kcrop, const double* E1, double* bbox_world, double* ts,
                             int32_t* valid, void* stream) {
  RGBM_REQUIRE(B > 0 && nocs1 && depth1 && r1 && choose1 && Kcrop && E1 && bbox_world && ts && valid, "postprocess arguments");
  return launch_postprocess(nocs1, depth1, r1, choose1, Kcrop, E1, bbox_world, ts, valid, B, P, img_size, (hipStream_t)stream);
}

int rgbm_adapose_postprocess_scratch_bytes(int B, size_t* bytes) {
  RGBM_REQUIRE(B > 0 && bytes, "postprocess_scratch_bytes arguments");
  *bytes = postprocess_slices(B) > 1 ? postprocess_scratch_bytes(B) : 0;
  return 0;
}

int rgbm_adapose_postprocess_ws(int B, int P, int img_size, const float* nocs1, const float* depth1, const float* r1,
                                const int32_t* choose1, const double* Kcrop, const double* E1, double* bbox_world, double* ts,
                                int32_t* valid, void* scratch, size_t scratch_bytes, void* stream) {
  RGBM_REQUIRE(B > 0 && nocs1 && depth1 && r1 && choose1 && Kcrop && E1 && bbox_world && ts && valid, "postprocess arguments");
  return launch_postprocess(nocs1, depth1, r1, choose1, Kcrop, E1, bbox_world, ts, valid, B, P, img_size, (hipStream_t)stream,
                            scratch, scratch_bytes);
}

int rgbm_adapose_postprocess_ransac(int B, int P, int img_size, uint32_t seed, const float* nocs1, const float* depth1,
                                    const int32_t* choose1, const double* Kcrop, const double* E1, double* bbox_world, double* srt,
                                    int32_t* valid, void* stream) {
  return launch_umeyama_ransac(nocs1, depth1, choose1, Kcrop, E1, bbox_world, srt, valid, B, P, img_size, seed, (hipStream_t)stream);
}

int rgbm_gae(int T, int N, const float* rewards, const uint8_t* dones, const float* values, const float* last_values,
             float gamma, float lam, float* returns, float* adv, double* sums, void* stream) {
  RGBM_REQUIRE(rewards && dones && values && last_values && returns && adv && sums, "gae arguments");
  return launch_gae(T, N, rewards, dones, values, last_values, gamma, lam, returns, adv, sums, (hipStream_t)stream);
}

int rgbm_adv_normalise(int64_t n_local, float* adv, const double* sums, double count_total, void* stream) {
  RGBM_REQUIRE(adv && sums && n_local > 0 && count_total > 1.0, "adv_normalise arguments");
  return launch_adv_normalise(n_local, adv, sums, count_total, (hipStream_t)stream);
}

int rgbm_conv_nd(int dtype, const void* in_dev, int N, int D, int H, int W, int Cin, int Cin_pad, const float* w_host,
                 int Cout, int Cout_pad, int KD, int KH, int KW, int stride_d, int stride_hw, int pad_d, int pad_hw,
                 int dil_hw, int transposed, const float* bias_host, const float* bn_scale_host, const float* bn_shift_host,
                 const void* res_dev, int res_mode, int act, float slope, void* out_dev, void* stream) {
  RGBM_REQUIRE(in_dev && w_host && out_dev, "conv arguments");
  ConvGeom g;
  g.Cin = Cin; g.Cout = Cout; g.KD = KD; g.KH = KH; g.KW = KW;
  g.sd = stride_d; g.sh = g.sw = stride_hw; g.pd = pad_d; g.ph = g.pw = pad_hw;
  g.dild = 1; g.dilh = g.dilw = dil_hw; g.transposed = transposed != 0; g.act = act; g.slope = slope;
  ConvLayer L;
  int rc = L.init(dtype, g, w_host, bias_host, bn_scale_host, bn_shift_host, Cin_pad, Cout_pad);
  if (!rc) rc = L.run(in_dev, out_dev, N, D, H, W, Cout_pad, res_dev, res_mode, nullptr, 0, (hipStream_t)stream);
  if (!rc) { hipError_t e = hipStreamSynchronize((hipStream_t)stream); if (e != hipSuccess) { set_error(hipGetErrorString(e)); rc = -2; } }
  L.destroy();
  return rc;
}

int rgbm_upsample_conv3x3(int dtype, const void* in_dev, int V, int h, int w, int Cin, const float* w_host, int Cout,
                          const float* bias_host, int act, float slope, void* z_scratch_dev, void* out_dev, void* stream) {
  RGBM_REQUIRE(in_dev && w_host && z_scratch_dev && out_dev, "upsample_conv3x3 arguments");
  UpConvLayer L;
  int rc = L.init(dtype, Cin, Cout, w_host, bias_host, act, slope);
  if (!rc) rc = L.run(in_dev, z_scratch_dev, out_dev, V, h, w, Cout, (hipStream_t)stream);
  if (!rc) { hipError_t e = hipStreamSynchronize((hipStream_t)stream); if (e != hipSuccess) { set_error(hipGetErrorString(e)); rc = -2; } }
  L.destroy();
  return rc;
}

int rgbm_upsample_conv3x3_final(int dtype, const void* in_dev, int V, int h, int w, const float* w3_host, const float* b3_host,
                                float slope, const float* wf_host, const float* bf_host, void* out_dev, int out_f32, void* stream) {
  RGBM_REQUIRE(in_dev && w3_host && b3_host && wf_host && bf_host && out_dev, "upsample_conv3x3_final arguments");
  UpConvFinal L;
  int rc = L.init(dtype, w3_host, b3_host, slope, wf_host, bf_host);
  if (!rc) rc = L.run(in_dev, out_dev, out_f32, V, h, w, (hipStream_t)stream);
  if (!rc) { hipError_t e = hipStreamSynchronize((hipStream_t)stream); if (e != hipSuccess) { set_error(hipGetErrorString(e)); rc = -2; } }
  L.destroy();
  return rc;
}

int rgbm_stem(int dtype, const float* img1_dev, const float* img2_dev, const float* w_host, void* out_dev, int B, int S, void* stream) {
  RGBM_REQUIRE(img1_dev && img2_dev && w_host && out_dev && B > 0, "stem arguments");
  std::vector<float> pk;
  stem_pack(w_host, pk);
  void* wd = nullptr;
  int rc = upload_packed(pk, dtype, &wd);
  if (!rc) rc = launch_stem(dtype, img1_dev, img2_dev, wd, out_dev, B, 2 * B, S, (hipStream_t)stream);
  if (!rc) { hipError_t e = hipStreamSynchronize((hipStream_t)stream); if (e != hipSuccess) { set_error(hipGetErrorString(e)); rc = -2; } }
  if (wd) (void)hipFree(wd);
  return rc;
}

int rgbm_bn_per_sample_scratch_bytes(int V, size_t* bytes) {
  RGBM_REQUIRE(V > 0 && bytes, "bn_per_sample_scratch_bytes arguments");
  *bytes = bn_scratch_bytes(V);
  return 0;
}
int rgbm_bn_per_sample(int dtype, void* y_dev, const void* res_dev, const float* gamma_dev, const float* beta_dev, void* scratch_dev,
                       int V, int64_t nvox, int C, int relu, void* stream) {
  RGBM_REQUIRE(y_dev && gamma_dev && beta_dev && scratch_dev, "bn_per_sample arguments");
  return launch_bn_per_sample(dtype, y_dev, res_dev, gamma_dev, beta_dev, scratch_dev, V, (long long)nvox, C, relu, (hipStream_t)stream);
}
int rgbm_maxpool3x3s2(int dtype, const void* in_dev, void* out_dev, int V, int H, int W, int C, void* stream) {
  return launch_maxpool3x3s2(dtype, in_dev, out_dev, V, H, W, C, (hipStream_t)stream);
}
int rgbm_resize_bilinear_ac(int dtype, const void* in_dev, void* out_dev, int V, int Hs, int Ws, int C, int Ho, int Wo,
                            void* stream) {
  return launch_resize_bilinear_ac(dtype, in_dev, out_dev, V, Hs, Ws, C, Ho, Wo, C, 0, (hipStream_t)stream);
}
int rgbm_adaptive_avgpool(int dtype, const void* in_dev, void* out_dev, int V, int H, int W, int C, int S, void* stream) {
  return launch_adaptive_avgpool(dtype, in_dev, out_dev, V, H, W, C, S, (hipStream_t)stream);
}
int rgbm_build_volume(int dtype, const void* feat_dev, const float* P_views_dev, const float* depths_dev, float* homog_scratch,
                      void* vol_dev, int V, int B, int D, int H, int W, void* stream) {
  if (int rc = launch_homography(P_views_dev, homog_scratch, V, B, (hipStream_t)stream)) return rc;
  return launch_build_volume(dtype, feat_dev, homog_scratch, depths_dev, vol_dev, 0, V, V, B, D, H, W, (hipStream_t)stream);
}

}

#include "prof.h"
extern "C" {
int rgbm_prof_rows(void) { return rgbm::kProfVariants; }
int rgbm_microbench_mfma_scratch_floats(int* n) {
  RGBM_REQUIRE(n, "microbench_mfma_scratch_floats arguments");
  return rgbm::microbench_mfma_scratch_floats(n);
}
int rgbm_microbench_mfma(float* scratch, int iters, int random_operands, double* flops, void* stream) {
  return rgbm::launch_microbench_mfma(scratch, iters, random_operands, flops, (hipStream_t)stream);
}
int rgbm_microbench_copy(const void* src, void* dst, size_t bytes, void* stream) {
  return rgbm::launch_microbench_copy(src, dst, bytes, (hipStream_t)stream);
}
int rgbm_prof_start(void) { return rgbm::prof_start(); }
int rgbm_prof_select(int row) {
  RGBM_REQUIRE(row >= -1 && row < rgbm::kProfVariants, "prof_select: row out of range");
  return rgbm::prof_select(row);
}
int rgbm_prof_stop(double* stats) {
  RGBM_REQUIRE(stats != nullptr, "prof_stop arguments");
  return rgbm::prof_stop(stats, rgbm::kProfVariants);
}
}

extern "C" int rgbm_conv3d_tile(int layer, int dtype, const void* in_dev, int N, int D, int H, int W, const float* w_host,
                                const float* bn_scale_host, const float* bn_shift_host, const void* res_dev, void* out_dev,
                                void* stream) {
  static const int cin[10] = {32, 8, 16, 16, 32, 32, 64, 64, 32, 16};
  static const int cout[10] = {8, 16, 16, 32, 32, 64, 64, 32, 16, 8};
  static const int stride[10] = {1, 2, 1, 2, 1, 2, 1, 1, 1, 1};
  RGBM_REQUIRE(layer >= 0 && layer < 10 && in_dev && w_host && bn_scale_host && bn_shift_host && out_dev, "conv3d_tile arguments");
  const bool tr = layer >= 7;
  const int coutp = cout[layer] < 16 ? 16 : cout[layer];
  std::vector<float> packed;
  conv3d_tile_pack(w_host, bn_scale_host, cin[layer], cout[layer], coutp, tr, dtype, packed);
  void* wdev = nullptr; float* bdev = nullptr;
  if (upload_packed(packed, dtype, &wdev)) return -2;
  std::vector<float> bpad(coutp, 0.f);
  for (int o = 0; o < cout[layer]; ++o) bpad[o] = bn_shift_host[o];
  if (upload_f32(bpad.data(), bpad.size(), &bdev)) return -2;
  Conv3dTileDesc d;
  memset(&d, 0, sizeof(d));
  d.in = in_dev; d.wgt = wdev; d.out = out_dev; d.bias = bdev; d.res = res_dev;
  d.N = N; d.Di = D; d.Hi = H; d.Wi = W;
  if (tr) { d.Do = 2 * D; d.Ho = 2 * H; d.Wo = 2 * W; d.Dq = D; d.Hq = H; d.Wq = W; }
  else {
    const int s = stride[layer];
    d.Do = (D + 2 - 3) / s + 1; d.Ho = (H + 2 - 3) / s + 1; d.Wo = (W + 2 - 3) / s + 1;
    d.Dq = d.Do; d.Hq = d.Ho; d.Wq = d.Wo;
  }
  d.Cout = cout[layer]; d.relu = 1; d.prof_variant = -1;
  int rc = launch_conv3d_tile(layer, dtype, d, (hipStream_t)stream);
  if (!rc) { hipError_t e = hipStreamSynchronize((hipStream_t)stream); if (e != hipSuccess) { set_error(hipGetErrorString(e)); rc = -2; } }
  (void)hipFree(wdev); (void)hipFree(bdev);
  return rc;
}

static int conv0_sweep_entry(int dtype, int feat_f16, const void* feat_dev, const float* P_views_dev, const float* depths_dev,
                             float* homog_scratch, const float* w_host, const float* bn_scale_host, const float* bn_shift_host,
                             void* out_dev, int V, int B, int D, int H, int W, void* stream) {
  RGBM_REQUIRE(feat_dev && P_views_dev && depths_dev && homog_scratch && w_host && bn_scale_host && bn_shift_host && out_dev,
               "conv0_sweep arguments");
  RGBM_REQUIRE(dtype == BF16 || dtype == F16 || dtype == BF16X3, "conv0_sweep: 16-bit storage types or bf16x3 (fp32 features in, split-pair c0 out)");
  if (int rc = launch_homography(P_views_dev, homog_scratch, V, B, (hipStream_t)stream)) return rc;
  std::vector<float> packed;
  conv0_sweep_pack(w_host, bn_scale_host, packed);
  void* wdev = nullptr; float* bdev = nullptr;
  if (dtype == BF16X3) { if (conv0_sweep_x3_upload(packed, &wdev)) return -2; }
  else if (upload_packed(packed, feat_f16 ? (int)F16 : dtype, &wdev)) return -2;
  std::vector<float> bpad(16, 0.f);
  for (int o = 0; o < 8; ++o) bpad[o] = bn_shift_host[o];
  if (upload_f32(bpad.data(), bpad.size(), &bdev)) return -2;
  Conv3dTileDesc d;
  memset(&d, 0, sizeof(d));
  d.wgt = wdev; d.out = out_dev; d.bias = bdev;
  d.N = V; d.Di = D; d.Hi = H; d.Wi = W; d.Do = D; d.Ho = H; d.Wo = W; d.Dq = D; d.Hq = H; d.Wq = W;
  d.Cout = 8; d.relu = 1; d.prof_variant = -1;
  d.feat = feat_dev; d.homog = homog_scratch; d.depths = depths_dev; d.v0 = 0; d.V = V; d.B = B;
  d.feat_f16 = feat_f16;
  int rc = dtype == BF16X3 ? launch_conv0_sweep_x3(d, (hipStream_t)stream) : launch_conv0_sweep(d, dtype, (hipStream_t)stream);
  if (!rc) { hipError_t e = hipStreamSynchronize((hipStream_t)stream); if (e != hipSuccess) { set_error(hipGetErrorString(e)); rc = -2; } }
  (void)hipFree(wdev); (void)hipFree(bdev);
  return rc;
}

extern "C" int rgbm_conv0_sweep_dt(int dtype, const void* feat_dev, const float* P_views_dev, const float* depths_dev,
                                   float* homog_scratch, const float* w_host, const float* bn_scale_host, const float* bn_shift_host,
                                   void* out_dev, int V, int B, int D, int H, int W, void* stream) {
  return conv0_sweep_entry(dtype, 0, feat_dev, P_views_dev, depths_dev, homog_scratch, w_host, bn_scale_host, bn_shift_host, out_dev, V, B, D,
                           H, W, stream);
}

extern "C" int rgbm_conv0_sweep_f16feat(const void* feat_f16_dev, const float* P_views_dev, const float* depths_dev,
                                        float* homog_scratch, const float* w_host, const float* bn_scale_host,
                                        const float* bn_shift_host, void* out_bf16_dev, int V, int B, int D, int H, int W, void* stream) {
  return conv0_sweep_entry(BF16, 1, feat_f16_dev, P_views_dev, depths_dev, homog_scratch, w_host, bn_scale_host, bn_shift_host, out_bf16_dev,
                           V, B, D, H, W, stream);
}

extern "C" int rgbm_conv0_sweep(const void* feat_dev, const float* P_views_dev, const float* depths_dev, float* homog_scratch,
                                const float* w_host, const float* bn_scale_host, const float* bn_shift_host, void* out_dev,
                                int V, int B, int D, int H, int W, void* stream) {
  return rgbm_conv0_sweep_dt(BF16, feat_dev, P_views_dev, depths_dev, homog_scratch, w_host, bn_scale_host, bn_shift_host, out_dev,
                             V, B, D, H, W, stream);
}

extern "C" int rgbm_prepare_inputs(const float* rgb_dev, const uint8_t* mask_dev, const double* K_dev, int N, int H, int W, int S,
                                   int P, uint32_t seed, float* img_out, int32_t* choose_out, float* pts2d_out, double* Kcrop_out,
                                   int32_t* window_out, int32_t* valid_out, uint8_t* scratch, void* stream) {
  return launch_prepare_inputs(rgb_dev, mask_dev, K_dev, nullptr, N, H, W, S, P, seed, img_out, choose_out, pts2d_out, Kcrop_out,
                               window_out, valid_out, scratch, (hipStream_t)stream);
}

extern "C" int rgbm_prepare_inputs_indexed(const float* rgb_dev, const uint8_t* mask_dev, const double* K_dev,
                                           const int32_t* frame_map_dev, int N, int H, int W, int S, int P, uint32_t seed,
                                           float* img_out, int32_t* choose_out, float* pts2d_out, double* Kcrop_out,
                                           int32_t* window_out, int32_t* valid_out, uint8_t* scratch, void* stream) {
  RGBM_REQUIRE(frame_map_dev, "prepare_inputs_indexed frame_map");
  return launch_prepare_inputs(rgb_dev, mask_dev, K_dev, frame_map_dev, N, H, W, S, P, seed, img_out, choose_out, pts2d_out,
                               Kcrop_out, window_out, valid_out, scratch, (hipStream_t)stream);
}

extern "C" int rgbm_prepare_inputs_ex(const float* rgb_dev, const uint8_t* mask_dev, const double* K_dev, const int32_t* frame_map_dev,
                                      int frame0, int N, int H, int W, int S, int P, uint32_t seed, float* img_out, int32_t* choose_out,
                                      float* pts2d_out, double* Kcrop_out, int32_t* window_out, int32_t* valid_out, uint8_t* scratch,
                                      void* stream) {
  RGBM_REQUIRE(frame0 >= 0, "prepare_inputs_ex frame0");
  return launch_prepare_inputs(rgb_dev, mask_dev, K_dev, frame_map_dev, N, H, W, S, P, seed, img_out, choose_out, pts2d_out,
                               Kcrop_out, window_out, valid_out, scratch, (hipStream_t)stream, frame0);
}

extern "C" int rgbm_adapose_postprocess_pnp(int B, int P, uint32_t seed, const float* nocs1, const float* pts2d1, const float* nocs2,
                                            const float* pts2d2, const double* K, const double* E1, const double* E2, double* bbox_out,
                                            double* srt_out, int32_t* info_out, int32_t* valid_out, void* stream) {
  return launch_pnp_ransac(nocs1, pts2d1, nocs2, pts2d2, K, E1, E2, bbox_out, srt_out, info_out, valid_out, B, P, seed, (hipStream_t)stream);
}

extern "C" int rgbm_projection(const double* Kcrop_dev, const double* E_dev, float* P_dev, int N, void* stream) {
  return launch_projection(Kcrop_dev, E_dev, P_dev, N, (hipStream_t)stream);
}

extern "C" int rgbm_mask_extent(const uint8_t* mask_dev, int N, int H, int W, int32_t* ext_out, int32_t* count_out, void* stream) {
  return launch_mask_extent(mask_dev, N, H, W, ext_out, count_out, (hipStream_t)stream);
}

static_assert(sizeof(rgbm_control_reward_args) == sizeof(rgbm::ControlRewardArgs), "control reward args ABI mismatch");
static_assert(sizeof(rgbm_synth_scene) == sizeof(rgbm::SynthScene), "synth scene ABI mismatch");
extern "C" int rgbm_lookat_quat(const double* dir_dev, int N, int batch_zero, double* quat_dev, void* stream) {
  return rgbm::launch_lookat_quat(dir_dev, quat_dev, N, batch_zero, (hipStream_t)stream);
}
extern "C" int rgbm_control_action_to_pose(const float* action_dev, int lda, const double* pose_mid, const double* pose_min,
                                           const double* pose_max, int N, double* pose_dev, void* stream) {
  return rgbm::launch_control_action(action_dev, lda, pose_mid, pose_min, pose_max, pose_dev, N, (hipStream_t)stream);
}
extern "C" int rgbm_control_reward(const rgbm_control_reward_args* args, void* stream) {
  RGBM_REQUIRE(args, "control_reward args");
  return rgbm::launch_control_reward(*reinterpret_cast<const rgbm::ControlRewardArgs*>(args), (hipStream_t)stream);
}
extern "C" int rgbm_control_grasp_frame(const double* est_dev, int N, double* center_dev, double* direction_dev, void* stream) {
  return rgbm::launch_control_grasp_frame(est_dev, center_dev, direction_dev, N, (hipStream_t)stream);
}
extern "C" int rgbm_synth_camera(const rgbm_synth_scene* scene, double* K_dev, double* E_dev, double* rays_dev, void* stream) {
  RGBM_REQUIRE(scene, "synth_camera scene");
  return rgbm::launch_synth_camera(*reinterpret_cast<const rgbm::SynthScene*>(scene), K_dev, E_dev, rays_dev, (hipStream_t)stream);
}
extern "C" int rgbm_synth_render(const rgbm_synth_scene* scene, const double* rays_dev, float* color_dev, uint8_t* mask_dev,
                                 void* stream) {
  RGBM_REQUIRE(scene, "synth_render scene");
  return rgbm::launch_synth_render(*reinterpret_cast<const rgbm::SynthScene*>(scene), rays_dev, color_dev, mask_dev,
                                   (hipStream_t)stream);
}

extern "C" int rgbm_debug_flags(int flags) { rgbm::g_debug_flags = flags; ++rgbm::g_tuning_version; return 0; }

extern "C" int rgbm_set_tuning(const char* key, long long value) {
  RGBM_REQUIRE(key != nullptr, "set_tuning arguments");
  const std::string k = key;
  if (k == "ws_min_rows") { RGBM_REQUIRE(value >= 0, "ws_min_rows"); rgbm::g_ws_min_rows = value; }
  else if (k == "gemm_kernel") { RGBM_REQUIRE(value >= 0 && value <= 2, "gemm_kernel"); rgbm::g_gemm_kernel = (int)value; }
  else { set_error("unknown tuning key " + k); return -1; }
  ++rgbm::g_tuning_version;
  return 0;
}

static_assert(sizeof(rgbm_policy_layout) == sizeof(rgbm::PolicyLayout), "policy layout ABI mismatch");
static_assert(sizeof(rgbm::PolicyOptState) == 40 || sizeof(rgbm::PolicyOptState) == 48, "opt state size");
extern "C" {
int rgbm_policy_forward(const float* params, const rgbm_policy_layout* L, int n, int mode, const float* obs, const float* noise,
                        float* actions, float* logp, float* value, float* mu, void* stream) {
  RGBM_REQUIRE(params && L && obs && mu, "policy_forward arguments");
  RGBM_REQUIRE(mode == 1 || (logp && value && actions), "policy_forward outputs");
  RGBM_REQUIRE(mode != 0 || noise, "policy_forward: act needs noise");
  return launch_policy_forward(params, *reinterpret_cast<const PolicyLayout*>(L), n, mode, obs, noise, actions, logp, value, mu,
                               (hipStream_t)stream);
}
int rgbm_ppo_partial_floats(const rgbm_policy_layout* L, int n, size_t* count) {
  RGBM_REQUIRE(L && count && n > 0, "ppo_partial_floats arguments");
  *count = (size_t)policy_partial_floats(*reinterpret_cast<const PolicyLayout*>(L), n);
  return 0;
}
int rgbm_ppo_minibatch_fwd_bwd(const float* params, const rgbm_policy_layout* L, int n, const float* obs, const float* actions,
                               const float* old_logp, const float* adv, const float* returns, const float* old_values,
                               const float* old_mu, const float* old_log_std, float clip, float vcoef, float ecoef,
                               float* partial_scratch, float* grads_flat, void* stream) {
  RGBM_REQUIRE(params && L && obs && actions && old_logp && adv && returns && old_values && old_mu && old_log_std &&
               partial_scratch && grads_flat, "ppo_minibatch arguments");
  return launch_ppo_minibatch(params, *reinterpret_cast<const PolicyLayout*>(L), n, obs, actions, old_logp, adv, returns,
                              old_values, old_mu, old_log_std, clip, vcoef, ecoef, partial_scratch, grads_flat, (hipStream_t)stream);
}
int rgbm_ppo_clip_adam(float* params, const float* grads_flat, float* exp_avg, float* exp_avg_sq, void* opt_state,
                       const rgbm_policy_layout* L, float inv_world, float max_norm, float desired_kl, float lr_min,
                       float lr_max, int adaptive, void* stream) {
  RGBM_REQUIRE(params && grads_flat && exp_avg && exp_avg_sq && opt_state && L, "ppo_clip_adam arguments");
  return launch_ppo_adam(params, grads_flat, exp_avg, exp_avg_sq, reinterpret_cast<PolicyOptState*>(opt_state), L->total,
                         inv_world, max_norm, desired_kl, lr_min, lr_max, adaptive, (hipStream_t)stream);
}
}
```

### rgbmanip_amd/csrc/conv3d_tile.hip

```cpp
#include <type_traits>
#include <utility>
#include "common.h"
#include "kernels.h"
#include "prof.h"

namespace rgbm {

template <typename T> struct Mma3;
template <> struct Mma3<unsigned short> {
  __device__ static __forceinline__ void run(const uint4& a, const uint4& b, f32x4& c) {
    c = __builtin_amdgcn_mfma_f32_16x16x32_bf16(__builtin_bit_cast(bf16x8, a), __builtin_bit_cast(bf16x8, b), c, 0, 0, 0);
  }
};
template <> struct Mma3<f16_t> {
  __device__ static __forceinline__ void run(const uint4& a, const uint4& b, f32x4& c) {
    c = __builtin_amdgcn_mfma_f32_16x16x32_f16(__builtin_bit_cast(f16x8, a), __builtin_bit_cast(f16x8, b), c, 0, 0, 0);
  }
};
template <> struct Mma3<float> {
  __device__ static __forceinline__ void run(const uint4& a, const uint4& b, f32x4& c) {
    c = __builtin_amdgcn_mfma_f32_16x16x4f32(__uint_as_float(a.x), __uint_as_float(b.x), c, 0, 0, 0);
    c = __builtin_amdgcn_mfma_f32_16x16x4f32(__uint_as_float(a.y), __uint_as_float(b.y), c, 0, 0, 0);
    c = __builtin_amdgcn_mfma_f32_16x16x4f32(__uint_as_float(a.z), __uint_as_float(b.z), c, 0, 0, 0);
    c = __builtin_amdgcn_mfma_f32_16x16x4f32(__uint_as_float(a.w), __uint_as_float(b.w), c, 0, 0, 0);
  }
};

template <> struct Mma3<bx3_t> {
  __device__ static __forceinline__ void run(const uint4& a, const uint4& b, f32x4& c) { c = mma_bx3_k16(a, b, c); }
};

template <typename T, int CIN, int COUTP, int TD, int TH, int TW, int STRIDE, bool TR, int WC = 1>
struct C3Cfg {
  static constexpr int E = 16 / sizeof(T);
  static constexpr int BPT = CIN * sizeof(T);
  static constexpr int VS = BPT <= 32 ? BPT : BPT + 16;
  static constexpr int CPV = BPT / 16;
  static constexpr int KE = TR ? 2 : 3;
  static constexpr int HD = (TD - 1) * STRIDE + KE, HH = (TH - 1) * STRIDE + KE, HW = (TW - 1) * STRIDE + KE;
  static constexpr int NVH = HD * HH * HW;
  static constexpr int LDS_BYTES = (NVH + 1) * VS;
  static constexpr int NV = TD * TH * TW;
  static constexpr int NF = NV / 64 * WC;
  static constexpr int FM = COUTP / 16 / WC;
  static_assert(4 % WC == 0 && (COUTP / 16) % WC == 0, "the channel tiles must split over WC waves");
  static constexpr int SPT = BPT >= 64 ? BPT / 64 : 1;
  static constexpr int TPS = BPT >= 64 ? 1 : 64 / BPT;
  static constexpr int GPT = 4 / TPS;
  static_assert(NV % 64 == 0, "tile must hold a multiple of 64 voxels");
  static_assert(BPT % 16 == 0, "voxel must be a multiple of 16 bytes");
  static constexpr int kd_of(int p) { return TR ? 1 + ((p >> 2) & 1) : 3; }
  static constexpr int kh_of(int p) { return TR ? 1 + ((p >> 1) & 1) : 3; }
  static constexpr int kw_of(int p) { return TR ? 1 + (p & 1) : 3; }
  static constexpr int taps_of(int p) { return kd_of(p) * kh_of(p) * kw_of(p); }
  static constexpr int steps_of(int p) { return (taps_of(p) + TPS - 1) / TPS * SPT; }
  static constexpr int step0_of(int p) { int s = 0; for (int q = 0; q < p; ++q) s += steps_of(q); return s; }
};

__device__ __forceinline__ void warp_ixy(const float* __restrict__ hm, float x, float y, float depth, int H, int W, float& ix,
                                         float& iy) {
  const float rx = hm[0] * x + hm[1] * y + hm[2];
  const float ry = hm[3] * x + hm[4] * y + hm[5];
  const float rz = hm[6] * x + hm[7] * y + hm[8];
  const float px = rx * depth + hm[9], py = ry * depth + hm[10], pz = rz * depth + hm[11];
  const float u = px / pz, vv = py / pz;
  const float gx = u / ((float)(W - 1) / 2.f) - 1.f;
  const float gy = vv / ((float)(H - 1) / 2.f) - 1.f;
  ix = ((gx + 1.f) * (float)W - 1.f) / 2.f;
  iy = ((gy + 1.f) * (float)H - 1.f) / 2.f;
}

int g_debug_flags = 0;
long long g_ws_min_rows = 0;
int g_tuning_version = 0;

template <int N> struct IC { static constexpr int value = N; };
template <int... I, typename F> __device__ __forceinline__ void static_for_impl(std::integer_sequence<int, I...>, F&& f) { (f(IC<I>{}), ...); }
template <int N, typename F> __device__ __forceinline__ void static_for(F&& f) { static_for_impl(std::make_integer_sequence<int, N>{}, f); }

template <typename T, int CIN, int COUTP, int TD, int TH, int TW, int STRIDE, bool TR, bool WARP, int WC = 1>
__global__ __launch_bounds__(256, 2) void conv3d_tile_kernel(const Conv3dTileDesc d) {
  using Cfg = C3Cfg<T, CIN, COUTP, TD, TH, TW, STRIDE, TR, WC>;
  constexpr int VS = Cfg::VS, CPV = Cfg::CPV, HH = Cfg::HH, HW = Cfg::HW, NVH = Cfg::NVH;
  constexpr int NF = Cfg::NF, FM = Cfg::FM, SPT = Cfg::SPT, TPS = Cfg::TPS, GPT = Cfg::GPT, E = Cfg::E;
  constexpr int ZERO_OFF = NVH * VS;
  extern __shared__ __attribute__((aligned(16))) unsigned char halo[];

  const int tid = threadIdx.x, lane = tid & 63, wave = tid >> 6;
  const int lr = lane & 15, lg = lane >> 4;

  const int nblk = gridDim.x, bq = nblk >> 3, br = nblk & 7, xcd = blockIdx.x & 7, bidx = blockIdx.x >> 3;
  int t = (xcd < br ? xcd * (bq + 1) : br * (bq + 1) + (xcd - br) * bq) + bidx;
  const int tw = t % d.ntw; t /= d.ntw;
  const int th = t % d.nth; t /= d.nth;
  const int td = t % d.ntd; t /= d.ntd;
  const int n = t;
  if (d.tile_mask && !d.tile_mask[(long long)n * (d.tile_mask_stride ? d.tile_mask_stride : d.nth * d.ntw) + th * d.ntw + tw]) return;
  const int q0d = td * TD, q0h = th * TH, q0w = tw * TW;
  const int i0d = TR ? q0d : q0d * STRIDE - 1, i0h = TR ? q0h : q0h * STRIDE - 1, i0w = TR ? q0w : q0w * STRIDE - 1;

  if (tid < VS / 16) reinterpret_cast<uint4*>(halo + ZERO_OFF)[tid] = make_uint4(0u, 0u, 0u, 0u);

  if constexpr (!WARP) {
    const T* __restrict__ in = reinterpret_cast<const T*>(d.in);
    constexpr int TOTAL = NVH * CPV;
    constexpr int ITERS = (TOTAL + 255) / 256;
    constexpr int BATCH = 8;
#pragma unroll 1
    for (int it0 = 0; it0 < ITERS; it0 += BATCH) {
      uint4 v[BATCH];
#pragma unroll
      for (int u = 0; u < BATCH; ++u) {
        const int idx = tid + (it0 + u) * 256;
        v[u] = make_uint4(0u, 0u, 0u, 0u);
        if (it0 + u < ITERS && idx < TOTAL) {
          const int vox = idx / CPV, chunk = idx - vox * CPV;
          const int hw = vox % HW, hh = (vox / HW) % HH, hd = vox / (HW * HH);
          const int gd = i0d + hd, gh = i0h + hh, gw = i0w + hw;
          if ((unsigned)gd < (unsigned)d.Di && (unsigned)gh < (unsigned)d.Hi && (unsigned)gw < (unsigned)d.Wi)
            v[u] = *reinterpret_cast<const uint4*>(in + ((((long long)n * d.Di + gd) * d.Hi + gh) * d.Wi + gw) * CIN + chunk * E);
        }
      }
#pragma unroll
      for (int u = 0; u < BATCH; ++u) {
        const int idx = tid + (it0 + u) * 256;
        if (it0 + u < ITERS && idx < TOTAL) {
          const int vox = idx / CPV, chunk = idx - vox * CPV;
          *reinterpret_cast<uint4*>(halo + vox * VS + chunk * 16) = v[u];
        }
      }
    }
  } else {
    const T* __restrict__ feat = reinterpret_cast<const T*>(d.feat);
    const int vv = d.v0 + n, partner = (vv + d.B) % d.V, bb = vv % d.B;
    const float* hm = d.homog + (long long)vv * 12;
    const T* refb = feat + (long long)vv * d.Hi * d.Wi * CIN;
    const T* srcb = feat + (long long)partner * d.Hi * d.Wi * CIN;
    constexpr int ITERS = (NVH + 255) / 256;
    constexpr int CG = CPV < 4 ? CPV : 4;
#pragma unroll 1
    for (int it = 0; it < ITERS; ++it) {
      const int vox = tid + it * 256;
      if (vox >= NVH) break;
      const int hw = vox % HW, hh = (vox / HW) % HH, hd = vox / (HW * HH);
      const int gd = i0d + hd, gh = i0h + hh, gw = i0w + hw;
      const bool inb = (unsigned)gd < (unsigned)d.Di && (unsigned)gh < (unsigned)d.Hi && (unsigned)gw < (unsigned)d.Wi;
      unsigned char* dst = halo + vox * VS;
      if (!inb) {
#pragma unroll
        for (int c = 0; c < CPV; ++c) *reinterpret_cast<uint4*>(dst + c * 16) = make_uint4(0u, 0u, 0u, 0u);
        continue;
      }
      float ix, iy;
      warp_ixy(hm, (float)gw, (float)gh, d.depths[bb * d.Di + gd], d.Hi, d.Wi, ix, iy);
      const bool fin = isfinite(ix) && isfinite(iy);
      ix = fin ? fminf(fmaxf(ix, -4.f), 1.0e6f) : 0.f;
      iy = fin ? fminf(fmaxf(iy, -4.f), 1.0e6f) : 0.f;
      const float fx = floorf(ix), fy = floorf(iy);
      const int x0 = (int)fx, y0 = (int)fy;
      const float tx = ix - fx, ty = iy - fy;
      const bool xin0 = (unsigned)x0 < (unsigned)d.Wi, xin1 = (unsigned)(x0 + 1) < (unsigned)d.Wi;
      const bool yin0 = (unsigned)y0 < (unsigned)d.Hi, yin1 = (unsigned)(y0 + 1) < (unsigned)d.Hi;
      const int xc0 = min(max(x0, 0), d.Wi - 1), xc1 = min(max(x0 + 1, 0), d.Wi - 1);
      const int yc0 = min(max(y0, 0), d.Hi - 1), yc1 = min(max(y0 + 1, 0), d.Hi - 1);
      const float w00 = (1.f - tx) * (1.f - ty), w01 = tx * (1.f - ty), w10 = (1.f - tx) * ty, w11 = tx * ty;
      const bool m00 = xin0 && yin0, m01 = xin1 && yin0, m10 = xin0 && yin1, m11 = xin1 && yin1;
      const T* p00 = srcb + ((long long)yc0 * d.Wi + xc0) * CIN;
      const T* p01 = srcb + ((long long)yc0 * d.Wi + xc1) * CIN;
      const T* p10 = srcb + ((long long)yc1 * d.Wi + xc0) * CIN;
      const T* p11 = srcb + ((long long)yc1 * d.Wi + xc1) * CIN;
      const T* pr = refb + ((long long)gh * d.Wi + gw) * CIN;
#pragma unroll
      for (int c0 = 0; c0 < CPV; c0 += CG) {
        uint4 r[CG], a[CG], b[CG], c[CG], e[CG];
#pragma unroll
        for (int k = 0; k < CG; ++k) {
          r[k] = *reinterpret_cast<const uint4*>(pr + (c0 + k) * E);
          a[k] = *reinterpret_cast<const uint4*>(p00 + (c0 + k) * E);
          b[k] = *reinterpret_cast<const uint4*>(p01 + (c0 + k) * E);
          c[k] = *reinterpret_cast<const uint4*>(p10 + (c0 + k) * E);
          e[k] = *reinterpret_cast<const uint4*>(p11 + (c0 + k) * E);
        }
#pragma unroll
        for (int k = 0; k < CG; ++k) {
          const uint4 z = make_uint4(0u, 0u, 0u, 0u);
          float fr[E], fa[E], fb[E], fc[E], fe[E], o[E];
          unpack_chunk(r[k], fr, T());
          unpack_chunk(m00 ? a[k] : z, fa, T());
          unpack_chunk(m01 ? b[k] : z, fb, T());
          unpack_chunk(m10 ? c[k] : z, fc, T());
          unpack_chunk(m11 ? e[k] : z, fe, T());
#pragma unroll
          for (int q = 0; q < E; ++q) {
            const float wsum = ((fa[q] * w00 + fb[q] * w01) + fc[q] * w10) + fe[q] * w11;
            o[q] = fin ? fr[q] + wsum : __builtin_nanf("");
          }
          *reinterpret_cast<uint4*>(dst + (c0 + k) * 16) = pack_chunk(o, T());
        }
      }
    }
  }
  __syncthreads();

  int base[NF];
  int qd_[NF], qh_[NF], qw_[NF];
#pragma unroll
  for (int f = 0; f < NF; ++f) {
    const int vt = ((wave / WC) * NF + f) * 16 + lr;
    const int w_ = vt % TW, h_ = (vt / TW) % TH, d_ = vt / (TW * TH);
    base[f] = ((d_ * STRIDE * HH + h_ * STRIDE) * HW + w_ * STRIDE) * VS + (TPS == 1 ? lg * 16 : 0);
    qd_[f] = q0d + d_; qh_[f] = q0h + h_; qw_[f] = q0w + w_;
  }

  const int co0 = (wave % WC) * FM * 16;
  const unsigned char* __restrict__ wg = reinterpret_cast<const unsigned char*>(d.wgt) + (long long)co0 * 64 + lr * 64 + lg * 16;
  T* __restrict__ out = reinterpret_cast<T*>(d.out);
  const T* __restrict__ res = reinterpret_cast<const T*>(d.res);

  float bv[FM][4];
#pragma unroll
  for (int a = 0; a < FM; ++a)
#pragma unroll
    for (int e = 0; e < 4; ++e) bv[a][e] = (co0 + a * 16 + lg * 4 < d.Cout) ? d.bias[co0 + a * 16 + lg * 4 + e] : 0.f;

  auto run_pass = [&](auto pc) {
    constexpr int PASS = decltype(pc)::value;
    constexpr int KH = Cfg::kh_of(PASS), KW = Cfg::kw_of(PASS);
    constexpr int NT = Cfg::taps_of(PASS), NS = Cfg::steps_of(PASS), S0 = Cfg::step0_of(PASS);
    f32x4 acc[FM][NF];
#pragma unroll
    for (int a = 0; a < FM; ++a)
#pragma unroll
      for (int f = 0; f < NF; ++f) acc[a][f] = f32x4{0.f, 0.f, 0.f, 0.f};
    auto step_off = [&](int s, int& so, bool& pad) {
      pad = false;
      if constexpr (TPS == 1) {
        const int tap = s / SPT;
        so = (((tap / (KH * KW)) * HH + (tap / KW) % KH) * HW + tap % KW) * VS + (s % SPT) * 64;
      } else {
        const int tap = s * TPS + lg / GPT;
        pad = tap >= NT;
        so = (((tap / (KH * KW)) * HH + (tap / KW) % KH) * HW + tap % KW) * VS + (lg % GPT) * 16;
      }
    };
    if constexpr (std::is_same<T, bx3_t>::value) {
      {
        constexpr int NP = (NS + 1) / 2;
        uint4 bq0[2][NF], bq1[2][NF], aq0[2][FM], aq1[2][FM];
        auto read_pair = [&](auto PI, uint4 (&d0)[NF], uint4 (&d1)[NF]) {
          constexpr int s = 2 * decltype(PI)::value;
          constexpr bool two = s + 1 < NS;
          int so0, so1 = 0;
          bool pad0, pad1 = false;
          step_off(s, so0, pad0);
          if constexpr (two) step_off(s + 1, so1, pad1);
          constexpr bool mp0 = (TPS > 1) && ((s + 1) * TPS > NT), mp1 = (TPS > 1) && ((s + 2) * TPS > NT);
#pragma unroll
          for (int f = 0; f < NF; ++f) {
            d0[f] = *reinterpret_cast<const uint4*>(halo + ((mp0 && pad0) ? ZERO_OFF : base[f] + so0));
            if constexpr (two) d1[f] = *reinterpret_cast<const uint4*>(halo + ((mp1 && pad1) ? ZERO_OFF : base[f] + so1));
          }
        };
        auto load_pair = [&](auto PI, uint4 (&d0)[FM], uint4 (&d1)[FM]) {
          constexpr int s = 2 * decltype(PI)::value;
#pragma unroll
          for (int a = 0; a < FM; ++a) {
            d0[a] = *reinterpret_cast<const uint4*>(wg + ((long long)(S0 + s) * COUTP + a * 16) * 64);
            if constexpr (s + 1 < NS) d1[a] = *reinterpret_cast<const uint4*>(wg + ((long long)(S0 + s + 1) * COUTP + a * 16) * 64);
          }
        };
        load_pair(IC<0>{}, aq0[0], aq1[0]);
        if constexpr (NP > 1) load_pair(IC<1>{}, aq0[1], aq1[1]);
        read_pair(IC<0>{}, bq0[0], bq1[0]);
        static_for<NP>([&](auto PI) {
          constexpr int pi = decltype(PI)::value;
          constexpr bool two = 2 * pi + 1 < NS;
          uint4 a0[FM], a1[FM];
#pragma unroll
          for (int a = 0; a < FM; ++a) {
            a0[a] = aq0[pi & 1][a];
            if constexpr (two) a1[a] = aq1[pi & 1][a];
          }
          if constexpr (pi + 2 < NP) load_pair(IC<pi + 2>{}, aq0[pi & 1], aq1[pi & 1]);
          if constexpr (pi + 1 < NP) read_pair(IC<pi + 1>{}, bq0[(pi + 1) & 1], bq1[(pi + 1) & 1]);
          __builtin_amdgcn_sched_barrier(0);
          if constexpr (two) {
            uint4 ah[FM], al[FM];
#pragma unroll
            for (int a = 0; a < FM; ++a) bx3_pair(a0[a], a1[a], ah[a], al[a]);
#pragma unroll
            for (int f = 0; f < NF; ++f) {
              uint4 bh, bl;
              bx3_pair(bq0[pi & 1][f], bq1[pi & 1][f], bh, bl);
#pragma unroll
              for (int a = 0; a < FM; ++a) {
                acc[a][f] = __builtin_amdgcn_mfma_f32_16x16x32_bf16(__builtin_bit_cast(bf16x8, al[a]), __builtin_bit_cast(bf16x8, bh), acc[a][f], 0, 0, 0);
                acc[a][f] = __builtin_amdgcn_mfma_f32_16x16x32_bf16(__builtin_bit_cast(bf16x8, ah[a]), __builtin_bit_cast(bf16x8, bl), acc[a][f], 0, 0, 0);
                acc[a][f] = __builtin_amdgcn_mfma_f32_16x16x32_bf16(__builtin_bit_cast(bf16x8, ah[a]), __builtin_bit_cast(bf16x8, bh), acc[a][f], 0, 0, 0);
              }
            }
          } else {
#pragma unroll
            for (int f = 0; f < NF; ++f)
#pragma unroll
              for (int a = 0; a < FM; ++a) Mma3<T>::run(a0[a], bq0[pi & 1][f], acc[a][f]);
          }
          __builtin_amdgcn_sched_barrier(0);
        });
      }
    } else {
    {
      uint4 bq[2][NF];
      auto read_b = [&](int s, uint4 (&dst)[NF]) {
        int so;
        bool pad;
        step_off(s, so, pad);
        const bool maybe_pad = (TPS > 1) && ((s + 1) * TPS > NT);
#pragma unroll
        for (int f = 0; f < NF; ++f) dst[f] = *reinterpret_cast<const uint4*>(halo + ((maybe_pad && pad) ? ZERO_OFF : base[f] + so));
      };
      constexpr int PDA = NS < 4 ? NS : 4;
      uint4 aq[PDA][FM];
      auto load_a = [&](int s, uint4 (&dst)[FM]) {
#pragma unroll
        for (int a = 0; a < FM; ++a) dst[a] = *reinterpret_cast<const uint4*>(wg + ((long long)(S0 + s) * COUTP + a * 16) * 64);
      };
#pragma unroll
      for (int p = 0; p < PDA; ++p) load_a(p, aq[p]);
      read_b(0, bq[0]);
#pragma unroll
      for (int s = 0; s < NS; ++s) {
        uint4 af[FM];
#pragma unroll
        for (int a = 0; a < FM; ++a) af[a] = aq[s % PDA][a];
        if (s + PDA < NS) load_a(s + PDA, aq[s % PDA]);
        if (s + 1 < NS) read_b(s + 1, bq[(s + 1) & 1]);
        __builtin_amdgcn_sched_barrier(0);
#pragma unroll
        for (int f = 0; f < NF; ++f)
#pragma unroll
          for (int a = 0; a < FM; ++a) Mma3<T>::run(af[a], bq[s & 1][f], acc[a][f]);
        __builtin_amdgcn_sched_barrier(0);
      }
    }
    }
    constexpr int pd = TR ? (PASS >> 2) & 1 : 0, ph = TR ? (PASS >> 1) & 1 : 0, pw = TR ? PASS & 1 : 0;
    constexpr int OS = TR ? 2 : 1;
    long long opix[NF];
    bool fok[NF];
    float rv[NF][FM][4];
#pragma unroll
    for (int f = 0; f < NF; ++f) {
      fok[f] = !(qd_[f] >= d.Dq || qh_[f] >= d.Hq || qw_[f] >= d.Wq);
      const long long rpix = (((long long)n * d.Do + (qd_[f] * OS + pd)) * d.Ho + (qh_[f] * OS + ph)) * d.Wo + (qw_[f] * OS + pw);
      opix[f] = (TR && d.out_classmajor) ? ((((long long)PASS * d.N + n) * d.Dq + qd_[f]) * d.Hq + qh_[f]) * d.Wq + qw_[f] : rpix;
#pragma unroll
      for (int a = 0; a < FM; ++a) {
        const int ch = co0 + a * 16 + lg * 4;
#pragma unroll
        for (int e = 0; e < 4; ++e) rv[f][a][e] = 0.f;
        if (res && fok[f] && ch < d.Cout) load4(res + rpix * d.Cout + ch, rv[f][a]);
      }
    }
#pragma unroll
    for (int f = 0; f < NF; ++f) {
      if (!fok[f]) continue;
#pragma unroll
      for (int a = 0; a < FM; ++a) {
        const int ch = co0 + a * 16 + lg * 4;
        if (ch >= d.Cout) continue;
        float v[4] = {acc[a][f][0], acc[a][f][1], acc[a][f][2], acc[a][f][3]};
#pragma unroll
        for (int e = 0; e < 4; ++e) {
          v[e] += bv[a][e];
          if (d.relu) v[e] = v[e] < 0.f ? 0.f : v[e];
          v[e] += rv[f][a][e];
        }
        store4(out + opix[f] * d.Cout + ch, v);
      }
    }
  };
  run_pass(IC<0>{});
  if constexpr (TR) {
    run_pass(IC<1>{}); run_pass(IC<2>{}); run_pass(IC<3>{});
    run_pass(IC<4>{}); run_pass(IC<5>{}); run_pass(IC<6>{}); run_pass(IC<7>{});
  }
}

static inline int c3_steps(int ntaps, int bpt) { return bpt >= 64 ? ntaps * (bpt / 64) : (ntaps + 64 / bpt - 1) / (64 / bpt); }

void conv3d_tile_pack(const float* w, const float* scale, int Cin, int Cout, int coutp, bool transposed, int dtype,
                      std::vector<float>& packed) {
  const int E = dtype_chunk(dtype);
  const int bpt = Cin * (int)dtype_size(dtype);
  const int spt = bpt >= 64 ? bpt / 64 : 1, tps = bpt >= 64 ? 1 : 64 / bpt;
  const int npass = transposed ? 8 : 1;
  int total = 0;
  for (int p = 0; p < npass; ++p) {
    const int nt = transposed ? (1 + ((p >> 2) & 1)) * (1 + ((p >> 1) & 1)) * (1 + (p & 1)) : 27;
    total += c3_steps(nt, bpt);
  }
  packed.assign((size_t)total * coutp * 4 * E, 0.f);
  int step0 = 0;
  for (int p = 0; p < npass; ++p) {
    const int pd = (p >> 2) & 1, ph = (p >> 1) & 1, pw = p & 1;
    const int KD = transposed ? 1 + pd : 3, KH = transposed ? 1 + ph : 3, KW = transposed ? 1 + pw : 3;
    const int nt = KD * KH * KW;
    const int ns = c3_steps(nt, bpt);
    for (int s = 0; s < ns; ++s)
      for (int g = 0; g < 4; ++g) {
        const int tap = spt > 1 ? s / spt : s * tps + g / (4 / tps);
        const int chunk = spt > 1 ? (s % spt) * 4 + g : g % (4 / tps);
        if (tap >= nt) continue;
        const int kd = tap / (KH * KW), kh = (tap / KW) % KH, kw = tap % KW;
        int widx;
        if (!transposed) widx = kd * 9 + kh * 3 + kw;
        else {
          auto kidx = [](int par, int delta) { return par == 0 ? 1 : (delta == 0 ? 2 : 0); };
          widx = kidx(pd, kd) * 9 + kidx(ph, kh) * 3 + kidx(pw, kw);
        }
        for (int o = 0; o < Cout; ++o)
          for (int e = 0; e < E; ++e) {
            const int c = chunk * E + e;
            if (c >= Cin) continue;
            const float val = transposed ? w[((long long)c * Cout + o) * 27 + widx] : w[((long long)o * Cin + c) * 27 + widx];
            packed[(((size_t)(step0 + s) * coutp + o) * 4 + g) * E + e] = val * (scale ? scale[o] : 1.f);
          }
      }
    step0 += ns;
  }
}

template <typename T, int CIN, int COUTP, int TD, int TH, int TW, int STRIDE, bool TR, bool WARP, int WC = 1>
static int launch_c3(Conv3dTileDesc d, hipStream_t s) {
  using Cfg = C3Cfg<T, CIN, COUTP, TD, TH, TW, STRIDE, TR, WC>;
  constexpr size_t LDS = Cfg::LDS_BYTES;
  static_assert(LDS <= 160 * 1024, "tile does not fit LDS");
  d.ntd = (d.Dq + TD - 1) / TD; d.nth = (d.Hq + TH - 1) / TH; d.ntw = (d.Wq + TW - 1) / TW;
  const long long nblk = (long long)d.N * d.ntd * d.nth * d.ntw;
  RGBM_REQUIRE(nblk > 0 && nblk < (1ll << 31), "conv3d grid out of range");
  auto kern = conv3d_tile_kernel<T, CIN, COUTP, TD, TH, TW, STRIDE, TR, WARP, WC>;
  if (int rc = ensure_dynamic_lds(reinterpret_cast<const void*>(kern), (int)LDS)) return rc;
  prof_begin_launch(s, d.prof_variant, d.algo_flops, d.algo_bytes);
  hipLaunchKernelGGL(kern, dim3((unsigned)nblk), dim3(256), LDS, s, d);
  prof_end_launch(s);
  RGBM_CHECK_HIP(hipGetLastError());
  return 0;
}

int conv3d_tile_dims(int layer, int dtype, int* TD, int* TH, int* TW) {
  const bool b16 = dtype == BF16 || dtype == F16;
#define C3_CASE(L, CIN, COUTP, TDB, THB, TWB, TDF, THF, TWF, STRIDE, TR, WARP, WCB, WCF) \
  case L: *TD = b16 ? TDB : TDF; *TH = b16 ? THB : THF; *TW = b16 ? TWB : TWF; return 0;
  switch (layer) {
#include "conv3d_tile_table.h"
    default: break;
  }
#undef C3_CASE
  return -1;
}

int launch_conv3d_tile(int layer, int dtype, const Conv3dTileDesc& d, hipStream_t s) {
#define C3_CASE(L, CIN, COUTP, TDB, THB, TWB, TDF, THF, TWF, STRIDE, TR, WARP, WCB, WCF)                           \
  case L:                                                                                                          \
    return dtype == BF16  ? launch_c3<unsigned short, CIN, COUTP, TDB, THB, TWB, STRIDE, TR, WARP, WCB>(d, s)      \
           : dtype == F16 ? launch_c3<f16_t, CIN, COUTP, TDB, THB, TWB, STRIDE, TR, WARP, WCB>(d, s)               \
           : dtype == BF16X3 ? launch_c3<bx3_t, CIN, COUTP, TDF, THF, TWF, STRIDE, TR, WARP, WCF>(d, s)            \
                          : launch_c3<float, CIN, COUTP, TDF, THF, TWF, STRIDE, TR, WARP, 1>(d, s);
  switch (layer) {
#include "conv3d_tile_table.h"
    default: break;
  }
#undef C3_CASE
  set_error("conv3d_tile: unknown layer id");
  return -1;
}

}
```

### rgbmanip_amd/csrc/kernels.h

```cpp
#pragma once
#include <vector>

#include "common.h"

namespace rgbm {

int launch_nchw_to_nhwc_pad(int dtype, const float* in, void* out, int V, int C, int H, int W, int Cp, hipStream_t s);
int launch_maxpool3x3s2(int dtype, const void* in, void* out, int V, int H, int W, int C, hipStream_t s);
int launch_resize_bilinear_ac(int dtype, const void* in, void* out, int V, int Hs, int Ws, int C, int Ho, int Wo, int ldo,
                              int ch_off, hipStream_t s);
int launch_copy_channels(int dtype, const void* in, void* out, long long npix, int C, int ldo, int ch_off, hipStream_t s);
int launch_adaptive_avgpool(int dtype, const void* in, void* out, int V, int H, int W, int C, int S, hipStream_t s);
int launch_adaptive_avgpool_multi(int dtype, const void* in, void* const* outs, const int* bins, int nb, int V, int H, int W, int C,
                                  hipStream_t s);
int launch_psp_pool_conv(int dtype, const void* in, int ldi, const void* const* w, void* const* outs, const int* bins, int V, int H, int W,
                         int act, float slope, hipStream_t s);
int launch_psp_resize_cat(int dtype, const void* f, const void* const* stages, const int* bins, void* out, int V, int Ho, int Wo, hipStream_t s);
int launch_homography(const float* P_views, float* out, int V, int B, hipStream_t s);
int launch_build_volume(int dtype, const void* feat, const float* homog, const float* depths, void* vol, int v0, int Vc, int V,
                        int B, int D, int H, int W, hipStream_t s);

int launch_upconv_combine(int dtype, const void* z, const float* bias, void* out, int V, int h, int w, int Co, int ldo, int act,
                          float slope, hipStream_t s, const float* drop = nullptr);
int launch_upconv_final(int dtype, const void* x, const void* wz, const float* bias, float slope, const void* wf, const float* biasf,
                        void* out, int out_f32, int V, int h, int w, hipStream_t s, const void* wf_f16 = nullptr);

constexpr int kDropoutPerView = 256 + 64;
unsigned dropout_threshold(float p);
float dropout_scale(float p);
int launch_dropout_masks(float* masks, unsigned long long* state, int B, float p, unsigned long long seed, int advance, hipStream_t s);

size_t bn_scratch_bytes(int V);
int launch_bn_per_sample(int dtype, void* y, const void* res, const float* gamma, const float* beta, void* scratch, int V,
                         long long nvox, int C, int relu, hipStream_t s);

int launch_to_f32(int dtype, const void* in, float* out, long long n, hipStream_t s);

int launch_gather_points(int dtype, const void* feat, const int* choose, float* out, int V, int P, int HW, int C, hipStream_t s);
int launch_prob_softmax_depth(int dtype, const void* u11, const float* wprob, const int* choose, const float* depths,
                              float* prob, float* depth_out, int v0, int Vc, int B, int P, int D, int H, int W, int classmajor,
                              hipStream_t s);
int launch_fuse_points(int dtype, const void* feat, const float* homog, const float* depths, const int* choose,
                       const float* prob, float* out, int V, int B, int P, int D, int H, int W, int ldo, int ch_off,
                       hipStream_t s, int Vn = -1);
int launch_mean_points(int dtype, const void* in, float* out, float* scratch, int V, int P, int C, hipStream_t s);
int launch_f32_to_f16(const float* in, void* out, long long n, hipStream_t s);
void stem_pack(const float* w, std::vector<float>& packed);
int launch_stem(int dtype, const float* img1, const float* img2, const void* wpk, void* out, int B, int V, int S, hipStream_t s);
int launch_f32_to_bx3(const float* in, void* out, long long n, hipStream_t s);
int launch_view_linear(const float* x, const float* W, const float* bias, float* out, int V, int I, int O, int ldw, int i0,
                       int relu, hipStream_t s);
struct PointMlpDesc {
  const float* table;
  const void* feat;
  const int* choose;
  float* nocs4;
  float* pf;
  int ldpf, P, HW;
  long long N;
};
int point_mlp_table_floats();
void point_mlp_pack(const float* const w[6], const float* const b[6], float* table);
int launch_point_mlp(int feat_dtype, const PointMlpDesc& d, hipStream_t s);
int launch_ortho6d(const float* r6, float* R, int V, hipStream_t s);
int launch_mean_points_partial(int dtype, const void* in, float* scratch, int V, int P, int C, hipStream_t s);
int launch_view_linear_mean(const float* partial, int P, float* mean_out, const float* W, const float* bias, float* out, int V, int I, int O,
                            int ldw, int i0, int relu, hipStream_t s);
int launch_pose_heads_mean(const float* partial, int P, float* mean_out, float* R, float* const w[3][3], float* const b[3][3],
                           float* const out[3], const int odim[3], int V, hipStream_t s);
int launch_pose_heads(const float* pf2, float* const w[3][3], float* const b[3][3], float* const out[3], const int odim[3], int V,
                      hipStream_t s);
int launch_stage_in(const float* P1, const float* P2, const int* c1, const int* c2, float* Pviews, int* choose, int B, int P, hipStream_t s);
int launch_stage_out(const float* nocs4, const float* depth, const float* R, const float* tv, const float* sv, float* const nocs[2],
                     float* const dep[2], float* const r[2], float* const t[2], float* const sz[2], int B, int P, int view2, hipStream_t s);
int launch_copy_cols(const float* in, float* out, long long rows, int ldi, int ldo, int n, hipStream_t s);

struct Conv3dTileDesc {
  const void* in; const void* wgt; void* out; const float* bias; const void* res;
  int N, Di, Hi, Wi;
  int Do, Ho, Wo;
  int Dq, Hq, Wq;
  int ntd, nth, ntw;
  int Cout, relu;
  const void* feat; const float* homog; const float* depths; int v0, V, B;
  int prof_variant; double algo_flops, algo_bytes;
  int out_classmajor;
  int feat_f16;
  const int* tile_list; const int* tile_count;
  int tile_mask_stride;
  const unsigned char* tile_mask;
};
extern int g_debug_flags;
extern long long g_ws_min_rows;
extern int g_tuning_version;
extern int g_gemm_kernel;
void conv3d_tile_pack(const float* w, const float* scale, int Cin, int Cout, int coutp, bool transposed, int dtype,
                      std::vector<float>& packed);
int launch_conv3d_tile(int layer, int dtype, const Conv3dTileDesc& d, hipStream_t s);
int sparse_mask_bytes_per_view(int S);
int sparse_mask_offset(int S, int layer);
int launch_sparse_masks(const int* choose, int v0, int Vc, int P, int S, unsigned char* masks, int* sweep_list, int* sweep_count,
                        hipStream_t s);
int conv3d_tile_dims(int layer, int dtype, int* TD, int* TH, int* TW);

void conv0_sweep_pack(const float* w, const float* scale, std::vector<float>& packed);
int launch_conv0_sweep(const Conv3dTileDesc& d, int dtype, hipStream_t s);

int conv0_sweep_x3_upload(const std::vector<float>& packed, void** dev);
int launch_conv0_sweep_x3(const Conv3dTileDesc& d, hipStream_t s);
int launch_bx3_to_f32(const void* in, float* out, long long n, hipStream_t s);

int launch_prob_sparse(const void* u9, const void* c0, const void* w11_packed, const float* bias11, const float* wprob,
                       const int* choose, const float* depths, float* prob, float* depth_out, int v0, int Vc, int B, int P,
                       int D, int H, int W, int dtype, hipStream_t s, const void* w11_taps = nullptr);
void prob_sparse_pack(const float* w, const float* scale, std::vector<float>& packed);

int launch_prepare_inputs(const float* rgb, const unsigned char* mask, const double* K, const int* frame_map, int N, int H, int W, int S, int P,
                          unsigned seed, float* img, int* choose, float* pts2d, double* Kcrop, int* window, int* valid,
                          unsigned char* small_scratch, hipStream_t s, int frame0 = 0);

int launch_umeyama_ransac(const float* nocs, const float* depth, const int* choose, const double* Kc, const double* E1,
                          double* bbox, double* srt, int* valid, int B, int P, int img, unsigned seed, hipStream_t s);

int launch_projection(const double* Kc, const double* E, float* P, int n, hipStream_t s);
int launch_pnp_ransac(const float* nocs1, const float* pts1, const float* nocs2, const float* pts2, const double* K, const double* E1,
                      const double* E2, double* bbox, double* srt, int* info, int* valid, int B, int P, unsigned seed, hipStream_t s);

int launch_mask_extent(const unsigned char* mask, int N, int H, int W, int* ext, int* count, hipStream_t s);

int launch_postprocess(const float* nocs, const float* depth, const float* rot, const int* choose, const double* Kc,
                       const double* E1, double* bbox, double* ts_out, int* valid, int B, int P, int img, hipStream_t s,
                       void* scratch = nullptr, size_t scratch_bytes = 0);
int launch_microbench_mfma(float* scratch, int iters, int random_operands, double* flops, hipStream_t s);
int microbench_mfma_scratch_floats(int* n);
int launch_microbench_copy(const void* src, void* dst, size_t bytes, hipStream_t s);
size_t postprocess_scratch_bytes(int B);
int postprocess_slices(int B);

int launch_gae(int T, int N, const float* rewards, const unsigned char* dones, const float* values, const float* last_values,
               float gamma, float lam, float* returns, float* adv, double* sums, hipStream_t s);
int launch_adv_normalise(long long n_local, float* adv, const double* sums, double count_total, hipStream_t s);

struct PolicyLayout { int dims[5]; int log_std; int w[2][4]; int b[2][4]; int total; };
struct PolicyOptState { int t; int n_updates; float lr; float last_kl; float last_norm; float pad_; double sum_surr; double sum_vloss; };
int launch_policy_forward(const float* params, const PolicyLayout& L, int n, int mode, const float* obs, const float* noise,
                          float* actions, float* logp, float* value, float* mu, hipStream_t s);
int policy_partial_floats(const PolicyLayout& L, int n);
int launch_ppo_minibatch(const float* params, const PolicyLayout& L, int n, const float* obs, const float* actions,
                         const float* old_logp, const float* adv, const float* returns, const float* old_values,
                         const float* old_mu, const float* old_sigma, float clip, float vcoef, float ecoef, float* partial,
                         float* grads, hipStream_t s);
int launch_ppo_adam(float* params, const float* grads, float* m, float* v, PolicyOptState* st, int total, float inv_world,
                    float max_norm, float desired_kl, float lr_min, float lr_max, int adaptive, hipStream_t s);

}
```

Measured before the change: 5835.

## Add persistent depth-column walk for 3D conv tiles with halo reuse and sparse column lists

Adds a persistent conv3d column kernel. Each workgroup walks a depth column of tiles for one (view, h, w) position, reusing the overlapping halo planes between consecutive depth tiles and prefetching the next tile while the current one computes. Weights can sit in LDS when they fit. Sparse tile masks are compacted into a column list by new count and list kernels. It is on by default for layers 1, 5 and 7 when there are enough columns, and it raises LDS use and adds two small launches per layer.

Measured after the change: 5889 (median of 6 runs). About the same (+0.9%).

```diff
diff --git a/include/rgbm.h b/include/rgbm.h
--- a/include/rgbm.h
+++ b/include/rgbm.h
@@ -144,6 +144,9 @@
                        int V, int64_t nvox, int C, int relu, void* stream);
 int rgbm_conv3d_tile(int layer, int dtype, const void* in_dev, int N, int D, int H, int W, const float* w_host,
                      const float* bn_scale_host, const float* bn_shift_host, const void* res_dev, void* out_dev, void* stream);
+int rgbm_conv3d_tile_ex(int layer, int dtype, const void* in_dev, int N, int D, int H, int W, const float* w_host,
+                        const float* bn_scale_host, const float* bn_shift_host, const void* res_dev, void* out_dev,
+                        const void* mask_dev, int mask_stride, int out_classmajor, int mode, int grid, void* stream);
 int rgbm_upsample_conv3x3(int dtype, const void* in_dev, int V, int h, int w, int Cin, const float* w_host, int Cout,
                           const float* bias_host, int act, float slope, void* z_scratch_dev, void* out_dev, void* stream);
 int rgbm_upsample_conv3x3_final(int dtype, const void* in_dev, int V, int h, int w, const float* w3_host, const float* b3_host,
diff --git a/rgbmanip_amd/_lib.py b/rgbmanip_amd/_lib.py
--- a/rgbmanip_amd/_lib.py
+++ b/rgbmanip_amd/_lib.py
@@ -113,6 +113,7 @@
     "rgbm_bn_per_sample_scratch_bytes": (_i, [_i, C.POINTER(_sz)]),
     "rgbm_bn_per_sample": (_i, [_i, _vp, _vp, _vp, _vp, _vp, _i, _i64, _i, _i, _vp]),
     "rgbm_conv3d_tile": (_i, [_i, _i, _vp, _i, _i, _i, _i, _vp, _vp, _vp, _vp, _vp, _vp]),
+    "rgbm_conv3d_tile_ex": (_i, [_i, _i, _vp, _i, _i, _i, _i, _vp, _vp, _vp, _vp, _vp, _vp, _i, _i, _i, _i, _vp]),
     "rgbm_upsample_conv3x3": (_i, [_i, _vp, _i, _i, _i, _i, _vp, _i, _vp, _i, _f, _vp, _vp, _vp]),
     "rgbm_upsample_conv3x3_final": (_i, [_i, _vp, _i, _i, _i, _vp, _vp, _f, _vp, _vp, _vp, _i, _vp]),
     "rgbm_stem": (_i, [_i, _vp, _vp, _vp, _vp, _i, _i, _vp]),
diff --git a/rgbmanip_amd/csrc/adapose.cpp b/rgbmanip_amd/csrc/adapose.cpp
--- a/rgbmanip_amd/csrc/adapose.cpp
+++ b/rgbmanip_amd/csrc/adapose.cpp
@@ -302,6 +302,7 @@
   bf.masks = (unsigned char*)A.alloc((size_t)V * sparse_mask_bytes_per_view(img));
   bf.sweep_list = (int*)A.alloc((size_t)V * ((img + 11) / 12) * ((img + 15) / 16) * 4);
   bf.sweep_count = (int*)A.alloc((size_t)(V + 64) * 4);
+  bf.col_scratch = (int*)A.alloc(((size_t)V * (1 + (size_t)((img / 2 + 7) / 8) * ((img / 2 + 7) / 8)) + 64) * 4);
   bf.feat = A.alloc((size_t)V * S * S * 32 * es);
   bf.featf = dtype == BF16X3 ? (float*)A.alloc((size_t)V * S * S * 32 * 4) : nullptr;
   bf.X0 = (float*)A.alloc(VP * 32 * 4);
@@ -474,6 +475,7 @@
     d.out_classmajor = layer == 9 ? 1 : 0;
     d.tile_mask = tmask;
     d.tile_mask_stride = sparse_mask_bytes_per_view(S);
+    d.col_scratch = bf.col_scratch;
     if (layer == 10 && sweep_sparse) { d.tile_list = bf.sweep_list; d.tile_count = bf.sweep_count; }
     d.prof_variant = dtype == BF16X3 ? (layer == 10 ? 28 : 27) : layer == 10 ? 10 + (dtype != F32 ? 1 : 0) : (dtype != F32 ? 16 + layer : 8);
     d.algo_flops = 2.0 * Vc * (double)(transposed ? Di * Hi * Wi : Do * Ho * Wo) * t3d[li].Cout * 27.0 * t3d[li].Cin;
diff --git a/rgbmanip_amd/csrc/adapose.h b/rgbmanip_amd/csrc/adapose.h
--- a/rgbmanip_amd/csrc/adapose.h
+++ b/rgbmanip_amd/csrc/adapose.h
@@ -76,6 +76,7 @@
     float *Pviews, *homog; int* choose; void* feat;
     unsigned char* masks;
     int *sweep_list, *sweep_count;
+    int* col_scratch;
     float* featf;
     float *X0, *X1, *H128, *H64, *nocs4, *N32, *PF96, *prob, *depth, *Q128a, *Q128b, *G256a, *G256b;
     void* PF96h;
diff --git a/rgbmanip_amd/csrc/capi.cpp b/rgbmanip_amd/csrc/capi.cpp
--- a/rgbmanip_amd/csrc/capi.cpp
+++ b/rgbmanip_amd/csrc/capi.cpp
@@ -428,9 +428,9 @@
 }
 }
 
-extern "C" int rgbm_conv3d_tile(int layer, int dtype, const void* in_dev, int N, int D, int H, int W, const float* w_host,
-                                const float* bn_scale_host, const float* bn_shift_host, const void* res_dev, void* out_dev,
-                                void* stream) {
+static int conv3d_tile_entry(int layer, int dtype, const void* in_dev, int N, int D, int H, int W, const float* w_host,
+                             const float* bn_scale_host, const float* bn_shift_host, const void* res_dev, void* out_dev,
+                             const unsigned char* mask_dev, int mask_stride, int out_classmajor, int mode, int grid, void* stream) {
   static const int cin[10] = {32, 8, 16, 16, 32, 32, 64, 64, 32, 16};
   static const int cout[10] = {8, 16, 16, 32, 32, 64, 64, 32, 16, 8};
   static const int stride[10] = {1, 2, 1, 2, 1, 2, 1, 1, 1, 1};
@@ -455,10 +455,36 @@
     d.Dq = d.Do; d.Hq = d.Ho; d.Wq = d.Wo;
   }
   d.Cout = cout[layer]; d.relu = 1; d.prof_variant = -1;
+  d.tile_mask = mask_dev; d.tile_mask_stride = mask_stride; d.out_classmajor = tr ? out_classmajor : 0;
+  d.col_mode = mode; d.col_grid = grid;
+  int* scratch = nullptr;
+  if (mask_dev) {
+    int td, th, tw;
+    RGBM_REQUIRE(!conv3d_tile_dims(layer, dtype, &td, &th, &tw), "conv3d_tile layer");
+    const size_t cols = (size_t)N * ((d.Hq + th - 1) / th) * ((d.Wq + tw - 1) / tw);
+    if (hipMalloc(&scratch, (1 + N + cols) * sizeof(int)) != hipSuccess) { (void)hipFree(wdev); (void)hipFree(bdev); set_error("hipMalloc"); return -2; }
+    d.col_scratch = scratch;
+  }
   int rc = launch_conv3d_tile(layer, dtype, d, (hipStream_t)stream);
   if (!rc) { hipError_t e = hipStreamSynchronize((hipStream_t)stream); if (e != hipSuccess) { set_error(hipGetErrorString(e)); rc = -2; } }
   (void)hipFree(wdev); (void)hipFree(bdev);
+  if (scratch) (void)hipFree(scratch);
   return rc;
+}
+
+extern "C" int rgbm_conv3d_tile(int layer, int dtype, const void* in_dev, int N, int D, int H, int W, const float* w_host,
+                                const float* bn_scale_host, const float* bn_shift_host, const void* res_dev, void* out_dev,
+                                void* stream) {
+  return conv3d_tile_entry(layer, dtype, in_dev, N, D, H, W, w_host, bn_scale_host, bn_shift_host, res_dev, out_dev, nullptr, 0, 0, 0, 0,
+                           stream);
+}
+
+extern "C" int rgbm_conv3d_tile_ex(int layer, int dtype, const void* in_dev, int N, int D, int H, int W, const float* w_host,
+                                   const float* bn_scale_host, const float* bn_shift_host, const void* res_dev, void* out_dev,
+                                   const void* mask_dev, int mask_stride, int out_classmajor, int mode, int grid, void* stream) {
+  RGBM_REQUIRE(mode >= 0 && mode <= 2 && grid >= 0 && mask_stride >= 0, "conv3d_tile_ex arguments");
+  return conv3d_tile_entry(layer, dtype, in_dev, N, D, H, W, w_host, bn_scale_host, bn_shift_host, res_dev, out_dev,
+                           static_cast<const unsigned char*>(mask_dev), mask_stride, out_classmajor, mode, grid, stream);
 }
 
 static int conv0_sweep_entry(int dtype, int feat_f16, const void* feat_dev, const float* P_views_dev, const float* depths_dev,
diff --git a/rgbmanip_amd/csrc/conv3d_tile.hip b/rgbmanip_amd/csrc/conv3d_tile.hip
--- a/rgbmanip_amd/csrc/conv3d_tile.hip
+++ b/rgbmanip_amd/csrc/conv3d_tile.hip
@@ -55,6 +55,10 @@
   static constexpr int taps_of(int p) { return kd_of(p) * kh_of(p) * kw_of(p); }
   static constexpr int steps_of(int p) { return (taps_of(p) + TPS - 1) / TPS * SPT; }
   static constexpr int step0_of(int p) { int s = 0; for (int q = 0; q < p; ++q) s += steps_of(q); return s; }
+  static constexpr int W_BYTES = step0_of(TR ? 8 : 1) * COUTP * 64;
+  static constexpr int ADV = TR ? TD : TD * STRIDE, OVL = HD - ADV;
+  static constexpr bool WL = W_BYTES <= 32 * 1024;
+  static constexpr int COL_LDS_BYTES = LDS_BYTES + (WL ? W_BYTES : 0);
 };
 
 __device__ __forceinline__ void warp_ixy(const float* __restrict__ hm, float x, float y, float depth, int H, int W, float& ix,
@@ -78,16 +82,228 @@
 template <int... I, typename F> __device__ __forceinline__ void static_for_impl(std::integer_sequence<int, I...>, F&& f) { (f(IC<I>{}), ...); }
 template <int N, typename F> __device__ __forceinline__ void static_for(F&& f) { static_for_impl(std::make_integer_sequence<int, N>{}, f); }
 
+template <int FM, int WC>
+__device__ __forceinline__ void c3_load_bias(const Conv3dTileDesc& d, float (&bv)[FM][4]) {
+  const int lane = threadIdx.x & 63, wave = threadIdx.x >> 6, lg = lane >> 4;
+  const int co0 = (wave % WC) * FM * 16;
+#pragma unroll
+  for (int a = 0; a < FM; ++a)
+#pragma unroll
+    for (int e = 0; e < 4; ++e) bv[a][e] = (co0 + a * 16 + lg * 4 < d.Cout) ? d.bias[co0 + a * 16 + lg * 4 + e] : 0.f;
+}
+
+template <typename T, int CIN, int COUTP, int TD, int TH, int TW, int STRIDE, bool TR, int WC, bool WL, int W_OFF, int HOOK_PASS, typename Hook>
+__device__ __forceinline__ void c3_tile_compute(const Conv3dTileDesc& d, const int n, const int q0d, const int q0h, const int q0w,
+                                                const float (&bv)[C3Cfg<T, CIN, COUTP, TD, TH, TW, STRIDE, TR, WC>::FM][4], Hook&& hook, const int zofs = 0) {
+  using Cfg = C3Cfg<T, CIN, COUTP, TD, TH, TW, STRIDE, TR, WC>;
+  constexpr int VS = Cfg::VS, HH = Cfg::HH, HW = Cfg::HW, NVH = Cfg::NVH;
+  constexpr int NF = Cfg::NF, FM = Cfg::FM, SPT = Cfg::SPT, TPS = Cfg::TPS, GPT = Cfg::GPT;
+  constexpr int ZERO_OFF = NVH * VS;
+  extern __shared__ __attribute__((aligned(16))) unsigned char halo[];
+  const int tid = threadIdx.x, lane = tid & 63, wave = tid >> 6;
+  const int lr = lane & 15, lg = lane >> 4;
+  (void)tid;
+
+  int base[NF];
+  int qd_[NF], qh_[NF], qw_[NF];
+#pragma unroll
+  for (int f = 0; f < NF; ++f) {
+    const int vt = ((wave / WC) * NF + f) * 16 + lr;
+    const int w_ = vt % TW, h_ = (vt / TW) % TH, d_ = vt / (TW * TH);
+    base[f] = ((d_ * STRIDE * HH + h_ * STRIDE) * HW + w_ * STRIDE) * VS + (TPS == 1 ? lg * 16 : 0) + zofs;
+    qd_[f] = q0d + d_; qh_[f] = q0h + h_; qw_[f] = q0w + w_;
+  }
+
+  const int co0 = (wave % WC) * FM * 16;
+  const unsigned char* __restrict__ wg = reinterpret_cast<const unsigned char*>(d.wgt) + (long long)co0 * 64 + lr * 64 + lg * 16 + zofs;
+  int wl[FM];
+#pragma unroll
+  for (int a = 0; a < FM; ++a) {
+    const int r = co0 + a * 16 + lr;
+    wl[a] = W_OFF + r * 64 + ((lg ^ ((r >> 2) & 3)) << 4) + zofs;
+  }
+  T* __restrict__ out = reinterpret_cast<T*>(d.out);
+  const T* __restrict__ res = reinterpret_cast<const T*>(d.res);
+
+  auto run_pass = [&](auto pc) {
+    constexpr int PASS = decltype(pc)::value;
+    constexpr int KH = Cfg::kh_of(PASS), KW = Cfg::kw_of(PASS);
+    constexpr int NT = Cfg::taps_of(PASS), NS = Cfg::steps_of(PASS), S0 = Cfg::step0_of(PASS);
+    f32x4 acc[FM][NF];
+#pragma unroll
+    for (int a = 0; a < FM; ++a)
+#pragma unroll
+      for (int f = 0; f < NF; ++f) acc[a][f] = f32x4{0.f, 0.f, 0.f, 0.f};
+    auto step_off = [&](int s, int& so, bool& pad) {
+      pad = false;
+      if constexpr (TPS == 1) {
+        const int tap = s / SPT;
+        so = (((tap / (KH * KW)) * HH + (tap / KW) % KH) * HW + tap % KW) * VS + (s % SPT) * 64;
+      } else {
+        const int tap = s * TPS + lg / GPT;
+        pad = tap >= NT;
+        so = (((tap / (KH * KW)) * HH + (tap / KW) % KH) * HW + tap % KW) * VS + (lg % GPT) * 16;
+      }
+    };
+    if constexpr (std::is_same<T, bx3_t>::value) {
+      {
+        constexpr int NP = (NS + 1) / 2;
+        uint4 bq0[2][NF], bq1[2][NF], aq0[2][FM], aq1[2][FM];
+        auto read_pair = [&](auto PI, uint4 (&d0)[NF], uint4 (&d1)[NF]) {
+          constexpr int s = 2 * decltype(PI)::value;
+          constexpr bool two = s + 1 < NS;
+          int so0, so1 = 0;
+          bool pad0, pad1 = false;
+          step_off(s, so0, pad0);
+          if constexpr (two) step_off(s + 1, so1, pad1);
+          constexpr bool mp0 = (TPS > 1) && ((s + 1) * TPS > NT), mp1 = (TPS > 1) && ((s + 2) * TPS > NT);
+#pragma unroll
+          for (int f = 0; f < NF; ++f) {
+            d0[f] = *reinterpret_cast<const uint4*>(halo + ((mp0 && pad0) ? ZERO_OFF : base[f] + so0));
+            if constexpr (two) d1[f] = *reinterpret_cast<const uint4*>(halo + ((mp1 && pad1) ? ZERO_OFF : base[f] + so1));
+          }
+        };
+        auto load_pair = [&](auto PI, uint4 (&d0)[FM], uint4 (&d1)[FM]) {
+          constexpr int s = 2 * decltype(PI)::value;
+#pragma unroll
+          for (int a = 0; a < FM; ++a) {
+            d0[a] = *reinterpret_cast<const uint4*>(wg + ((long long)(S0 + s) * COUTP + a * 16) * 64);
+            if constexpr (s + 1 < NS) d1[a] = *reinterpret_cast<const uint4*>(wg + ((long long)(S0 + s + 1) * COUTP + a * 16) * 64);
+          }
+        };
+        static_assert(!WL, "split pairs read their weights from L2");
+        load_pair(IC<0>{}, aq0[0], aq1[0]);
+        if constexpr (NP > 1) load_pair(IC<1>{}, aq0[1], aq1[1]);
+        read_pair(IC<0>{}, bq0[0], bq1[0]);
+        if constexpr (PASS == HOOK_PASS) hook();
+        static_for<NP>([&](auto PI) {
+          constexpr int pi = decltype(PI)::value;
+          constexpr bool two = 2 * pi + 1 < NS;
+          uint4 a0[FM], a1[FM];
+#pragma unroll
+          for (int a = 0; a < FM; ++a) {
+            a0[a] = aq0[pi & 1][a];
+            if constexpr (two) a1[a] = aq1[pi & 1][a];
+          }
+          if constexpr (pi + 2 < NP) load_pair(IC<pi + 2>{}, aq0[pi & 1], aq1[pi & 1]);
+          if constexpr (pi + 1 < NP) read_pair(IC<pi + 1>{}, bq0[(pi + 1) & 1], bq1[(pi + 1) & 1]);
+          __builtin_amdgcn_sched_barrier(0);
+          if constexpr (two) {
+            uint4 ah[FM], al[FM];
+#pragma unroll
+            for (int a = 0; a < FM; ++a) bx3_pair(a0[a], a1[a], ah[a], al[a]);
+#pragma unroll
+            for (int f = 0; f < NF; ++f) {
+              uint4 bh, bl;
+              bx3_pair(bq0[pi & 1][f], bq1[pi & 1][f], bh, bl);
+#pragma unroll
+              for (int a = 0; a < FM; ++a) {
+                acc[a][f] = __builtin_amdgcn_mfma_f32_16x16x32_bf16(__builtin_bit_cast(bf16x8, al[a]), __builtin_bit_cast(bf16x8, bh), acc[a][f], 0, 0, 0);
+                acc[a][f] = __builtin_amdgcn_mfma_f32_16x16x32_bf16(__builtin_bit_cast(bf16x8, ah[a]), __builtin_bit_cast(bf16x8, bl), acc[a][f], 0, 0, 0);
+                acc[a][f] = __builtin_amdgcn_mfma_f32_16x16x32_bf16(__builtin_bit_cast(bf16x8, ah[a]), __builtin_bit_cast(bf16x8, bh), acc[a][f], 0, 0, 0);
+              }
+            }
+          } else {
+#pragma unroll
+            for (int f = 0; f < NF; ++f)
+#pragma unroll
+              for (int a = 0; a < FM; ++a) Mma3<T>::run(a0[a], bq0[pi & 1][f], acc[a][f]);
+          }
+          __builtin_amdgcn_sched_barrier(0);
+        });
+      }
+    } else {
+    {
+      uint4 bq[2][NF];
+      auto read_b = [&](int s, uint4 (&dst)[NF]) {
+        int so;
+        bool pad;
+        step_off(s, so, pad);
+        const bool maybe_pad = (TPS > 1) && ((s + 1) * TPS > NT);
+#pragma unroll
+        for (int f = 0; f < NF; ++f) dst[f] = *reinterpret_cast<const uint4*>(halo + ((maybe_pad && pad) ? ZERO_OFF : base[f] + so));
+      };
+      constexpr int PDA = NS < 4 ? NS : 4;
+      uint4 aq[PDA][FM];
+      auto load_a = [&](int s, uint4 (&dst)[FM]) {
+#pragma unroll
+        for (int a = 0; a < FM; ++a) {
+          if constexpr (WL) dst[a] = *reinterpret_cast<const uint4*>(halo + wl[a] + (S0 + s) * COUTP * 64);
+          else dst[a] = *reinterpret_cast<const uint4*>(wg + ((long long)(S0 + s) * COUTP + a * 16) * 64);
+        }
+      };
+#pragma unroll
+      for (int p = 0; p < PDA; ++p) load_a(p, aq[p]);
+      read_b(0, bq[0]);
+      if constexpr (PASS == HOOK_PASS) hook();
+#pragma unroll
+      for (int s = 0; s < NS; ++s) {
+        uint4 af[FM];
+#pragma unroll
+        for (int a = 0; a < FM; ++a) af[a] = aq[s % PDA][a];
+        if (s + PDA < NS) load_a(s + PDA, aq[s % PDA]);
+        if (s + 1 < NS) read_b(s + 1, bq[(s + 1) & 1]);
+        __builtin_amdgcn_sched_barrier(0);
+#pragma unroll
+        for (int f = 0; f < NF; ++f)
+#pragma unroll
+          for (int a = 0; a < FM; ++a) Mma3<T>::run(af[a], bq[s & 1][f], acc[a][f]);
+        __builtin_amdgcn_sched_barrier(0);
+      }
+    }
+    }
+    constexpr int pd = TR ? (PASS >> 2) & 1 : 0, ph = TR ? (PASS >> 1) & 1 : 0, pw = TR ? PASS & 1 : 0;
+    constexpr int OS = TR ? 2 : 1;
+    long long opix[NF];
+    bool fok[NF];
+    float rv[NF][FM][4];
+#pragma unroll
+    for (int f = 0; f < NF; ++f) {
+      fok[f] = !(qd_[f] >= d.Dq || qh_[f] >= d.Hq || qw_[f] >= d.Wq);
+      const long long rpix = (((long long)n * d.Do + (qd_[f] * OS + pd)) * d.Ho + (qh_[f] * OS + ph)) * d.Wo + (qw_[f] * OS + pw);
+      opix[f] = (TR && d.out_classmajor) ? ((((long long)PASS * d.N + n) * d.Dq + qd_[f]) * d.Hq + qh_[f]) * d.Wq + qw_[f] : rpix;
+#pragma unroll
+      for (int a = 0; a < FM; ++a) {
+        const int ch = co0 + a * 16 + lg * 4;
+#pragma unroll
+        for (int e = 0; e < 4; ++e) rv[f][a][e] = 0.f;
+        if (res && fok[f] && ch < d.Cout) load4(res + rpix * d.Cout + ch, rv[f][a]);
+      }
+    }
+#pragma unroll
+    for (int f = 0; f < NF; ++f) {
+      if (!fok[f]) continue;
+#pragma unroll
+      for (int a = 0; a < FM; ++a) {
+        const int ch = co0 + a * 16 + lg * 4;
+        if (ch >= d.Cout) continue;
+        float v[4] = {acc[a][f][0], acc[a][f][1], acc[a][f][2], acc[a][f][3]};
+#pragma unroll
+        for (int e = 0; e < 4; ++e) {
+          v[e] += bv[a][e];
+          if (d.relu) v[e] = v[e] < 0.f ? 0.f : v[e];
+          v[e] += rv[f][a][e];
+        }
+        store4(out + opix[f] * d.Cout + ch, v);
+      }
+    }
+  };
+  run_pass(IC<0>{});
+  if constexpr (TR) {
+    run_pass(IC<1>{}); run_pass(IC<2>{}); run_pass(IC<3>{});
+    run_pass(IC<4>{}); run_pass(IC<5>{}); run_pass(IC<6>{}); run_pass(IC<7>{});
+  }
+}
+
 template <typename T, int CIN, int COUTP, int TD, int TH, int TW, int STRIDE, bool TR, bool WARP, int WC = 1>
 __global__ __launch_bounds__(256, 2) void conv3d_tile_kernel(const Conv3dTileDesc d) {
   using Cfg = C3Cfg<T, CIN, COUTP, TD, TH, TW, STRIDE, TR, WC>;
   constexpr int VS = Cfg::VS, CPV = Cfg::CPV, HH = Cfg::HH, HW = Cfg::HW, NVH = Cfg::NVH;
-  constexpr int NF = Cfg::NF, FM = Cfg::FM, SPT = Cfg::SPT, TPS = Cfg::TPS, GPT = Cfg::GPT, E = Cfg::E;
+  constexpr int FM = Cfg::FM, E = Cfg::E;
   constexpr int ZERO_OFF = NVH * VS;
   extern __shared__ __attribute__((aligned(16))) unsigned char halo[];
 
-  const int tid = threadIdx.x, lane = tid & 63, wave = tid >> 6;
-  const int lr = lane & 15, lg = lane >> 4;
+  const int tid = threadIdx.x;
 
   const int nblk = gridDim.x, bq = nblk >> 3, br = nblk & 7, xcd = blockIdx.x & 7, bidx = blockIdx.x >> 3;
   int t = (xcd < br ? xcd * (bq + 1) : br * (bq + 1) + (xcd - br) * bq) + bidx;
@@ -202,189 +418,163 @@
   }
   __syncthreads();
 
-  int base[NF];
-  int qd_[NF], qh_[NF], qw_[NF];
-#pragma unroll
-  for (int f = 0; f < NF; ++f) {
-    const int vt = ((wave / WC) * NF + f) * 16 + lr;
-    const int w_ = vt % TW, h_ = (vt / TW) % TH, d_ = vt / (TW * TH);
-    base[f] = ((d_ * STRIDE * HH + h_ * STRIDE) * HW + w_ * STRIDE) * VS + (TPS == 1 ? lg * 16 : 0);
-    qd_[f] = q0d + d_; qh_[f] = q0h + h_; qw_[f] = q0w + w_;
-  }
-
-  const int co0 = (wave % WC) * FM * 16;
-  const unsigned char* __restrict__ wg = reinterpret_cast<const unsigned char*>(d.wgt) + (long long)co0 * 64 + lr * 64 + lg * 16;
-  T* __restrict__ out = reinterpret_cast<T*>(d.out);
-  const T* __restrict__ res = reinterpret_cast<const T*>(d.res);
-
   float bv[FM][4];
-#pragma unroll
-  for (int a = 0; a < FM; ++a)
-#pragma unroll
-    for (int e = 0; e < 4; ++e) bv[a][e] = (co0 + a * 16 + lg * 4 < d.Cout) ? d.bias[co0 + a * 16 + lg * 4 + e] : 0.f;
-
-  auto run_pass = [&](auto pc) {
-    constexpr int PASS = decltype(pc)::value;
-    constexpr int KH = Cfg::kh_of(PASS), KW = Cfg::kw_of(PASS);
-    constexpr int NT = Cfg::taps_of(PASS), NS = Cfg::steps_of(PASS), S0 = Cfg::step0_of(PASS);
-    f32x4 acc[FM][NF];
-#pragma unroll
-    for (int a = 0; a < FM; ++a)
-#pragma unroll
-      for (int f = 0; f < NF; ++f) acc[a][f] = f32x4{0.f, 0.f, 0.f, 0.f};
-    auto step_off = [&](int s, int& so, bool& pad) {
-      pad = false;
-      if constexpr (TPS == 1) {
-        const int tap = s / SPT;
-        so = (((tap / (KH * KW)) * HH + (tap / KW) % KH) * HW + tap % KW) * VS + (s % SPT) * 64;
-      } else {
-        const int tap = s * TPS + lg / GPT;
-        pad = tap >= NT;
-        so = (((tap / (KH * KW)) * HH + (tap / KW) % KH) * HW + tap % KW) * VS + (lg % GPT) * 16;
-      }
-    };
-    if constexpr (std::is_same<T, bx3_t>::value) {
-      {
-        constexpr int NP = (NS + 1) / 2;
-        uint4 bq0[2][NF], bq1[2][NF], aq0[2][FM], aq1[2][FM];
-        auto read_pair = [&](auto PI, uint4 (&d0)[NF], uint4 (&d1)[NF]) {
-          constexpr int s = 2 * decltype(PI)::value;
-          constexpr bool two = s + 1 < NS;
-          int so0, so1 = 0;
-          bool pad0, pad1 = false;
-          step_off(s, so0, pad0);
-          if constexpr (two) step_off(s + 1, so1, pad1);
-          constexpr bool mp0 = (TPS > 1) && ((s + 1) * TPS > NT), mp1 = (TPS > 1) && ((s + 2) * TPS > NT);
-#pragma unroll
-          for (int f = 0; f < NF; ++f) {
-            d0[f] = *reinterpret_cast<const uint4*>(halo + ((mp0 && pad0) ? ZERO_OFF : base[f] + so0));
-            if constexpr (two) d1[f] = *reinterpret_cast<const uint4*>(halo + ((mp1 && pad1) ? ZERO_OFF : base[f] + so1));
-          }
-        };
-        auto load_pair = [&](auto PI, uint4 (&d0)[FM], uint4 (&d1)[FM]) {
-          constexpr int s = 2 * decltype(PI)::value;
-#pragma unroll
-          for (int a = 0; a < FM; ++a) {
-            d0[a] = *reinterpret_cast<const uint4*>(wg + ((long long)(S0 + s) * COUTP + a * 16) * 64);
-            if constexpr (s + 1 < NS) d1[a] = *reinterpret_cast<const uint4*>(wg + ((long long)(S0 + s + 1) * COUTP + a * 16) * 64);
-          }
-        };
-        load_pair(IC<0>{}, aq0[0], aq1[0]);
-        if constexpr (NP > 1) load_pair(IC<1>{}, aq0[1], aq1[1]);
-        read_pair(IC<0>{}, bq0[0], bq1[0]);
-        static_for<NP>([&](auto PI) {
-          constexpr int pi = decltype(PI)::value;
-          constexpr bool two = 2 * pi + 1 < NS;
-          uint4 a0[FM], a1[FM];
-#pragma unroll
-          for (int a = 0; a < FM; ++a) {
-            a0[a] = aq0[pi & 1][a];
-            if constexpr (two) a1[a] = aq1[pi & 1][a];
-          }
-          if constexpr (pi + 2 < NP) load_pair(IC<pi + 2>{}, aq0[pi & 1], aq1[pi & 1]);
-          if constexpr (pi + 1 < NP) read_pair(IC<pi + 1>{}, bq0[(pi + 1) & 1], bq1[(pi + 1) & 1]);
-          __builtin_amdgcn_sched_barrier(0);
-          if constexpr (two) {
-            uint4 ah[FM], al[FM];
-#pragma unroll
-            for (int a = 0; a < FM; ++a) bx3_pair(a0[a], a1[a], ah[a], al[a]);
-#pragma unroll
-            for (int f = 0; f < NF; ++f) {
-              uint4 bh, bl;
-              bx3_pair(bq0[pi & 1][f], bq1[pi & 1][f], bh, bl);
-#pragma unroll
-              for (int a = 0; a < FM; ++a) {
-                acc[a][f] = __builtin_amdgcn_mfma_f32_16x16x32_bf16(__builtin_bit_cast(bf16x8, al[a]), __builtin_bit_cast(bf16x8, bh), acc[a][f], 0, 0, 0);
-                acc[a][f] = __builtin_amdgcn_mfma_f32_16x16x32_bf16(__builtin_bit_cast(bf16x8, ah[a]), __builtin_bit_cast(bf16x8, bl), acc[a][f], 0, 0, 0);
-                acc[a][f] = __builtin_amdgcn_mfma_f32_16x16x32_bf16(__builtin_bit_cast(bf16x8, ah[a]), __builtin_bit_cast(bf16x8, bh), acc[a][f], 0, 0, 0);
-              }
-            }
-          } else {
-#pragma unroll
-            for (int f = 0; f < NF; ++f)
-#pragma unroll
-              for (int a = 0; a < FM; ++a) Mma3<T>::run(a0[a], bq0[pi & 1][f], acc[a][f]);
-          }
-          __builtin_amdgcn_sched_barrier(0);
-        });
-      }
-    } else {
+  c3_load_bias<FM, WC>(d, bv);
+  c3_tile_compute<T, CIN, COUTP, TD, TH, TW, STRIDE, TR, WC, false, 0, 0>(d, n, q0d, q0h, q0w, bv, [] {});
+}
+
+template <typename T, int CIN, int COUTP, int TD, int TH, int TW, int STRIDE, bool TR, int WC, int WPC>
+__global__ __launch_bounds__(256, WPC) void conv3d_col_kernel(const Conv3dTileDesc d) {
+  using Cfg = C3Cfg<T, CIN, COUTP, TD, TH, TW, STRIDE, TR, WC>;
+  constexpr int VS = Cfg::VS, CPV = Cfg::CPV, HH = Cfg::HH, HW = Cfg::HW, HD = Cfg::HD, NVH = Cfg::NVH, FM = Cfg::FM, E = Cfg::E;
+  constexpr int ADV = Cfg::ADV, OVL = Cfg::OVL;
+  constexpr int PLV = HH * HW, PLC = PLV * CPV;
+  constexpr int NU = (HD * PLC + 255) / 256, NO = (OVL * PLC + 255) / 256;
+  constexpr int W_OFF = (NVH + 1) * VS;
+  static_assert(OVL >= 1 && OVL <= ADV, "the shared planes must not overlap the new ones' sources");
+  static_assert(sizeof(T) == 2, "16-bit storage only");
+  extern __shared__ __attribute__((aligned(16))) unsigned char halo[];
+  const int tid = threadIdx.x;
+
+  const long long cnt = d.col_count ? (long long)*d.col_count : (long long)d.N * d.nth * d.ntw;
+  const int G = gridDim.x, gq = G >> 3, gr = G & 7, xcd = blockIdx.x & 7, j = blockIdx.x >> 3;
+  const int nx = gq + (xcd < gr ? 1 : 0);
+  const int r0 = xcd < gr ? xcd * (gq + 1) : gr * (gq + 1) + (xcd - gr) * gq;
+  const long long hi = cnt * (r0 + nx) / G;
+  long long it = cnt * r0 / G + j;
+  if (it >= hi) return;
+  auto col_of = [&](long long i, int& n, int& th, int& tw) {
+    const int c = d.col_list ? d.col_list[i] : (int)i;
+    tw = c % d.ntw; th = (c / d.ntw) % d.nth; n = c / (d.ntw * d.nth);
+  };
+
+  if (tid < VS / 16) reinterpret_cast<uint4*>(halo + NVH * VS)[tid] = make_uint4(0u, 0u, 0u, 0u);
+  if constexpr (Cfg::WL) {
+    constexpr int WCH = Cfg::W_BYTES / 16;
+    const uint4* __restrict__ wsrc = reinterpret_cast<const uint4*>(d.wgt);
+    for (int k = tid; k < WCH; k += 256) {
+      const int g = k & 3, r = (k >> 2) % COUTP, step = k / (4 * COUTP);
+      *reinterpret_cast<uint4*>(halo + W_OFF + step * COUTP * 64 + r * 64 + ((g ^ ((r >> 2) & 3)) << 4)) = wsrc[k];
+    }
+  }
+  float bv[FM][4];
+  c3_load_bias<FM, WC>(d, bv);
+
+  const T* __restrict__ in = reinterpret_cast<const T*>(d.in);
+  uint4 pf[NU];
+  int z = 0;
+  auto prefetch = [&](int n, int th, int tw, int td, bool start) {
+    const int q0d = td * TD, q0h = th * TH, q0w = tw * TW;
+    const int i0d = TR ? q0d : q0d * STRIDE - 1, i0h = TR ? q0h : q0h * STRIDE - 1, i0w = TR ? q0w : q0w * STRIDE - 1;
+    const int gp0 = start ? i0d : i0d + OVL, nch = (start ? HD : ADV) * PLC;
+#pragma unroll
+    for (int u = 0; u < NU; ++u) {
+      const int idx = tid + z + u * 256;
+      pf[u] = make_uint4(0u, 0u, 0u, 0u);
+      if (idx < nch) {
+        const int pl = idx / PLC, rem = idx - pl * PLC, vox = rem / CPV, chunk = rem - vox * CPV;
+        const int gd = gp0 + pl, gh = i0h + vox / HW, gw = i0w + vox % HW;
+        if ((unsigned)gd < (unsigned)d.Di && (unsigned)gh < (unsigned)d.Hi && (unsigned)gw < (unsigned)d.Wi)
+          pf[u] = *reinterpret_cast<const uint4*>(in + ((((long long)n * d.Di + gd) * d.Hi + gh) * d.Wi + gw) * CIN + chunk * E);
+      }
+    }
+  };
+
+  int n, th, tw, td = 0;
+  bool start = true;
+  col_of(it, n, th, tw);
+  prefetch(n, th, tw, 0, true);
+#pragma unroll 1
+  while (true) {
+    asm volatile("v_mov_b32 %0, 0" : "=v"(z));
+    const int tz = tid + z;
+    __syncthreads();
+    if (!start) {
+      uint4 ov[NO];
+#pragma unroll
+      for (int u = 0; u < NO; ++u) {
+        const int idx = tz + u * 256;
+        ov[u] = make_uint4(0u, 0u, 0u, 0u);
+        if (idx < OVL * PLC) ov[u] = *reinterpret_cast<const uint4*>(halo + (ADV * PLV + idx / CPV) * VS + (idx % CPV) * 16);
+      }
+      __syncthreads();
+#pragma unroll
+      for (int u = 0; u < NO; ++u) {
+        const int idx = tz + u * 256;
+        if (idx < OVL * PLC) *reinterpret_cast<uint4*>(halo + (idx / CPV) * VS + (idx % CPV) * 16) = ov[u];
+      }
+    }
     {
-      uint4 bq[2][NF];
-      auto read_b = [&](int s, uint4 (&dst)[NF]) {
-        int so;
-        bool pad;
-        step_off(s, so, pad);
-        const bool maybe_pad = (TPS > 1) && ((s + 1) * TPS > NT);
-#pragma unroll
-        for (int f = 0; f < NF; ++f) dst[f] = *reinterpret_cast<const uint4*>(halo + ((maybe_pad && pad) ? ZERO_OFF : base[f] + so));
-      };
-      constexpr int PDA = NS < 4 ? NS : 4;
-      uint4 aq[PDA][FM];
-      auto load_a = [&](int s, uint4 (&dst)[FM]) {
-#pragma unroll
-        for (int a = 0; a < FM; ++a) dst[a] = *reinterpret_cast<const uint4*>(wg + ((long long)(S0 + s) * COUTP + a * 16) * 64);
-      };
-#pragma unroll
-      for (int p = 0; p < PDA; ++p) load_a(p, aq[p]);
-      read_b(0, bq[0]);
-#pragma unroll
-      for (int s = 0; s < NS; ++s) {
-        uint4 af[FM];
-#pragma unroll
-        for (int a = 0; a < FM; ++a) af[a] = aq[s % PDA][a];
-        if (s + PDA < NS) load_a(s + PDA, aq[s % PDA]);
-        if (s + 1 < NS) read_b(s + 1, bq[(s + 1) & 1]);
-        __builtin_amdgcn_sched_barrier(0);
-#pragma unroll
-        for (int f = 0; f < NF; ++f)
-#pragma unroll
-          for (int a = 0; a < FM; ++a) Mma3<T>::run(af[a], bq[s & 1][f], acc[a][f]);
-        __builtin_amdgcn_sched_barrier(0);
-      }
-    }
-    }
-    constexpr int pd = TR ? (PASS >> 2) & 1 : 0, ph = TR ? (PASS >> 1) & 1 : 0, pw = TR ? PASS & 1 : 0;
-    constexpr int OS = TR ? 2 : 1;
-    long long opix[NF];
-    bool fok[NF];
-    float rv[NF][FM][4];
-#pragma unroll
-    for (int f = 0; f < NF; ++f) {
-      fok[f] = !(qd_[f] >= d.Dq || qh_[f] >= d.Hq || qw_[f] >= d.Wq);
-      const long long rpix = (((long long)n * d.Do + (qd_[f] * OS + pd)) * d.Ho + (qh_[f] * OS + ph)) * d.Wo + (qw_[f] * OS + pw);
-      opix[f] = (TR && d.out_classmajor) ? ((((long long)PASS * d.N + n) * d.Dq + qd_[f]) * d.Hq + qh_[f]) * d.Wq + qw_[f] : rpix;
-#pragma unroll
-      for (int a = 0; a < FM; ++a) {
-        const int ch = co0 + a * 16 + lg * 4;
-#pragma unroll
-        for (int e = 0; e < 4; ++e) rv[f][a][e] = 0.f;
-        if (res && fok[f] && ch < d.Cout) load4(res + rpix * d.Cout + ch, rv[f][a]);
-      }
-    }
-#pragma unroll
-    for (int f = 0; f < NF; ++f) {
-      if (!fok[f]) continue;
-#pragma unroll
-      for (int a = 0; a < FM; ++a) {
-        const int ch = co0 + a * 16 + lg * 4;
-        if (ch >= d.Cout) continue;
-        float v[4] = {acc[a][f][0], acc[a][f][1], acc[a][f][2], acc[a][f][3]};
-#pragma unroll
-        for (int e = 0; e < 4; ++e) {
-          v[e] += bv[a][e];
-          if (d.relu) v[e] = v[e] < 0.f ? 0.f : v[e];
-          v[e] += rv[f][a][e];
-        }
-        store4(out + opix[f] * d.Cout + ch, v);
-      }
-    }
-  };
-  run_pass(IC<0>{});
-  if constexpr (TR) {
-    run_pass(IC<1>{}); run_pass(IC<2>{}); run_pass(IC<3>{});
-    run_pass(IC<4>{}); run_pass(IC<5>{}); run_pass(IC<6>{}); run_pass(IC<7>{});
-  }
+      const int v0 = start ? 0 : OVL * PLV, nch = (start ? HD : ADV) * PLC;
+#pragma unroll
+      for (int u = 0; u < NU; ++u) {
+        const int idx = tz + u * 256;
+        if (idx < nch) *reinterpret_cast<uint4*>(halo + (v0 + idx / CPV) * VS + (idx % CPV) * 16) = pf[u];
+      }
+    }
+    __syncthreads();
+    int nn = n, nh = th, nw = tw, nd = td + 1;
+    bool nstart = false, more = true;
+    if (nd >= d.ntd) {
+      it += nx;
+      more = it < hi;
+      if (more) { col_of(it, nn, nh, nw); nd = 0; nstart = true; }
+    }
+    c3_tile_compute<T, CIN, COUTP, TD, TH, TW, STRIDE, TR, WC, Cfg::WL, W_OFF, TR ? 7 : 0>(
+        d, n, td * TD, th * TH, tw * TW, bv, [&] { if (more) prefetch(nn, nh, nw, nd, nstart); }, z);
+    if (!more) break;
+    n = nn; th = nh; tw = nw; td = nd; start = nstart;
+  }
+}
+
+__global__ __launch_bounds__(256) void c3_col_count_kernel(const unsigned char* __restrict__ mask, int stride, int per_view,
+                                                           int* __restrict__ scratch) {
+  __shared__ int part[256];
+  const int v = blockIdx.x, tid = threadIdx.x;
+  const unsigned char* m = mask + (long long)v * stride;
+  int c = 0;
+  for (int i = tid; i < per_view; i += 256) c += m[i] ? 1 : 0;
+  part[tid] = c;
+  __syncthreads();
+  for (int off = 128; off > 0; off >>= 1) {
+    if (tid < off) part[tid] += part[tid + off];
+    __syncthreads();
+  }
+  if (tid == 0) scratch[1 + v] = part[0];
+}
+
+__global__ __launch_bounds__(256) void c3_col_list_kernel(const unsigned char* __restrict__ mask, int stride, int per_view, int N,
+                                                          int* __restrict__ scratch) {
+  __shared__ int part[256];
+  const int v = blockIdx.x, tid = threadIdx.x;
+  int* list = scratch + 1 + N;
+  int c = 0;
+  for (int u = tid; u < v; u += 256) c += scratch[1 + u];
+  part[tid] = c;
+  __syncthreads();
+  for (int off = 128; off > 0; off >>= 1) {
+    if (tid < off) part[tid] += part[tid + off];
+    __syncthreads();
+  }
+  int base = part[0];
+  __syncthreads();
+  const unsigned char* m = mask + (long long)v * stride;
+  for (int seg = 0; seg < per_view; seg += 256) {
+    const int i = seg + tid;
+    const int f = i < per_view && m[i] ? 1 : 0;
+    part[tid] = f;
+    __syncthreads();
+    for (int off = 1; off < 256; off <<= 1) {
+      const int t = tid >= off ? part[tid - off] : 0;
+      __syncthreads();
+      part[tid] += t;
+      __syncthreads();
+    }
+    if (f) list[base + part[tid] - 1] = v * per_view + i;
+    base += part[255];
+    __syncthreads();
+  }
+  if (v == N - 1 && tid == 0) scratch[0] = base;
 }
 
 static inline int c3_steps(int ntaps, int bpt) { return bpt >= 64 ? ntaps * (bpt / 64) : (ntaps + 64 / bpt - 1) / (64 / bpt); }
@@ -431,7 +621,34 @@
   }
 }
 
-template <typename T, int CIN, int COUTP, int TD, int TH, int TW, int STRIDE, bool TR, bool WARP, int WC = 1>
+static constexpr int kC3OneTileFlag = 1 << 19;
+
+template <typename T, int CIN, int COUTP, int TD, int TH, int TW, int STRIDE, bool TR, int WC, int WPC>
+static int launch_c3_col(Conv3dTileDesc d, long long ncols, int n_cu, hipStream_t s) {
+  using Cfg = C3Cfg<T, CIN, COUTP, TD, TH, TW, STRIDE, TR, WC>;
+  constexpr size_t LDS = Cfg::COL_LDS_BYTES;
+  static_assert(LDS <= 160 * 1024, "column walk does not fit LDS");
+  auto kern = conv3d_col_kernel<T, CIN, COUTP, TD, TH, TW, STRIDE, TR, WC, WPC>;
+  d.ntd = (d.Dq + TD - 1) / TD;
+  if (int rc = ensure_dynamic_lds(reinterpret_cast<const void*>(kern), (int)LDS)) return rc;
+  long long grid = d.col_grid > 0 ? d.col_grid : (long long)WPC * n_cu;
+  if (grid > ncols) grid = ncols;
+  d.col_list = nullptr; d.col_count = nullptr;
+  prof_begin_launch(s, d.prof_variant, d.algo_flops, d.algo_bytes);
+  if (d.tile_mask) {
+    const int per_view = d.nth * d.ntw, stride = d.tile_mask_stride ? d.tile_mask_stride : per_view;
+    hipLaunchKernelGGL(c3_col_count_kernel, dim3((unsigned)d.N), dim3(256), 0, s, d.tile_mask, stride, per_view, d.col_scratch);
+    hipLaunchKernelGGL(c3_col_list_kernel, dim3((unsigned)d.N), dim3(256), 0, s, d.tile_mask, stride, per_view, d.N, d.col_scratch);
+    d.col_count = d.col_scratch;
+    d.col_list = d.col_scratch + 1 + d.N;
+  }
+  hipLaunchKernelGGL(kern, dim3((unsigned)grid), dim3(256), LDS, s, d);
+  prof_end_launch(s);
+  RGBM_CHECK_HIP(hipGetLastError());
+  return 0;
+}
+
+template <typename T, int CIN, int COUTP, int TD, int TH, int TW, int STRIDE, bool TR, bool WARP, int WC = 1, int COL = 0, int TDC = TD, bool COL_DEF = false>
 static int launch_c3(Conv3dTileDesc d, hipStream_t s) {
   using Cfg = C3Cfg<T, CIN, COUTP, TD, TH, TW, STRIDE, TR, WC>;
   constexpr size_t LDS = Cfg::LDS_BYTES;
@@ -439,6 +656,16 @@
   d.ntd = (d.Dq + TD - 1) / TD; d.nth = (d.Hq + TH - 1) / TH; d.ntw = (d.Wq + TW - 1) / TW;
   const long long nblk = (long long)d.N * d.ntd * d.nth * d.ntw;
   RGBM_REQUIRE(nblk > 0 && nblk < (1ll << 31), "conv3d grid out of range");
+  if constexpr (COL > 0 && !WARP && sizeof(T) == 2) {
+    static_assert(COL * C3Cfg<T, CIN, COUTP, TDC, TH, TW, STRIDE, TR, WC>::COL_LDS_BYTES <= 160 * 1024, "column walk: COL workgroups per CU do not fit LDS");
+    if (d.col_mode != 1 && !(g_debug_flags & kC3OneTileFlag) && (!d.tile_mask || d.col_scratch)) {
+      const long long ncols = (long long)d.N * d.nth * d.ntw;
+      int n_cu = 0;
+      if (int rc = persistent_grid_cus(&n_cu)) return rc;
+      if (d.col_mode == 2 || (COL_DEF && ncols >= 4ll * COL * n_cu)) return launch_c3_col<T, CIN, COUTP, TDC, TH, TW, STRIDE, TR, WC, COL>(d, ncols, n_cu, s);
+    }
+  }
+  RGBM_REQUIRE(d.col_mode != 2, "conv3d_tile: this layer / storage type has no column walk");
   auto kern = conv3d_tile_kernel<T, CIN, COUTP, TD, TH, TW, STRIDE, TR, WARP, WC>;
   if (int rc = ensure_dynamic_lds(reinterpret_cast<const void*>(kern), (int)LDS)) return rc;
   prof_begin_launch(s, d.prof_variant, d.algo_flops, d.algo_bytes);
@@ -460,11 +687,14 @@
   return -1;
 }
 
+#define C3_COL(L) ((L) == 1 ? 3 : (L) == 8 ? 3 : ((L) >= 2 && (L) <= 5) || (L) == 7 ? 2 : 0)
+#define C3_COL_TD(L, TDB) ((L) == 1 ? 4 : (TDB))
+#define C3_COL_DEF(L) ((L) == 1 || (L) == 5 || (L) == 7)
 int launch_conv3d_tile(int layer, int dtype, const Conv3dTileDesc& d, hipStream_t s) {
 #define C3_CASE(L, CIN, COUTP, TDB, THB, TWB, TDF, THF, TWF, STRIDE, TR, WARP, WCB, WCF)                           \
   case L:                                                                                                          \
-    return dtype == BF16  ? launch_c3<unsigned short, CIN, COUTP, TDB, THB, TWB, STRIDE, TR, WARP, WCB>(d, s)      \
-           : dtype == F16 ? launch_c3<f16_t, CIN, COUTP, TDB, THB, TWB, STRIDE, TR, WARP, WCB>(d, s)               \
+    return dtype == BF16  ? launch_c3<unsigned short, CIN, COUTP, TDB, THB, TWB, STRIDE, TR, WARP, WCB, C3_COL(L), C3_COL_TD(L, TDB), C3_COL_DEF(L)>(d, s) \
+           : dtype == F16 ? launch_c3<f16_t, CIN, COUTP, TDB, THB, TWB, STRIDE, TR, WARP, WCB, C3_COL(L), C3_COL_TD(L, TDB), C3_COL_DEF(L)>(d, s)  \
            : dtype == BF16X3 ? launch_c3<bx3_t, CIN, COUTP, TDF, THF, TWF, STRIDE, TR, WARP, WCF>(d, s)            \
                           : launch_c3<float, CIN, COUTP, TDF, THF, TWF, STRIDE, TR, WARP, 1>(d, s);
   switch (layer) {
@@ -475,5 +705,8 @@
   set_error("conv3d_tile: unknown layer id");
   return -1;
 }
-
-}
+#undef C3_COL
+#undef C3_COL_TD
+#undef C3_COL_DEF
+
+}
diff --git a/rgbmanip_amd/csrc/kernels.h b/rgbmanip_amd/csrc/kernels.h
--- a/rgbmanip_amd/csrc/kernels.h
+++ b/rgbmanip_amd/csrc/kernels.h
@@ -89,6 +89,10 @@
   const int* tile_list; const int* tile_count;
   int tile_mask_stride;
   const unsigned char* tile_mask;
+  int* col_scratch;
+  int col_mode;
+  int col_grid;
+  const int* col_list; const int* col_count;
 };
 extern int g_debug_flags;
 extern long long g_ws_min_rows;
```
